# EspressoSystems/cap

Hardware: AMD Instinct MI355X
Metric: transfer-note proofs/sec (2-in/2-out) (higher is better)
Workload: dtype u32 limbs (254-bit Montgomery integers; 9 x 29-bit lazy limbs in the hot kernels)

## Files before the change

cap_amd/csrc/check_kernels.hpp:

```cpp
#pragma once
#include <hip/hip_runtime.h>

#include "gatecheck29.hpp"
#include "plonk_kernels.hpp"

namespace cap {
namespace pk {

constexpr unsigned long long kCopyKeyBase = 1ull << 40;
constexpr unsigned long long kNoFault = ~0ull;

struct CheckKey {
  const fe* sel;
  const uint32_t* perm;
  uint32_t num_inputs;
  uint32_t pad;
};
struct CheckOut {
  unsigned long long first;
  unsigned long long gates, copies;
};

__device__ __forceinline__ void check_report(unsigned long long key, unsigned long long* first,
                                             unsigned long long* count) {
  __shared__ unsigned long long s_min[kThreads / 64];
  __shared__ uint32_t s_cnt[kThreads / 64];
  const uint32_t cnt = (uint32_t)__popcll(__ballot(key != kNoFault));
  uint32_t lo = (uint32_t)key, hi = (uint32_t)(key >> 32);
#pragma unroll
  for (int d = 32; d >= 1; d >>= 1) {
    const uint32_t olo = __shfl_xor(lo, d), ohi = __shfl_xor(hi, d);
    const unsigned long long o = ((unsigned long long)ohi << 32) | olo, m = ((unsigned long long)hi << 32) | lo;
    if (o < m) {
      lo = olo;
      hi = ohi;
    }
  }
  const uint32_t wave = threadIdx.x >> 6;
  if ((threadIdx.x & 63) == 0) {
    s_min[wave] = ((unsigned long long)hi << 32) | lo;
    s_cnt[wave] = cnt;
  }
  __syncthreads();
  if (threadIdx.x == 0) {
    unsigned long long m = s_min[0];
    uint32_t c = s_cnt[0];
#pragma unroll
    for (int k = 1; k < kThreads / 64; k++) {
      m = s_min[k] < m ? s_min[k] : m;
      c += s_cnt[k];
    }
    if (c) {
      atomicMin(first, m);
      atomicAdd(count, (unsigned long long)c);
    }
  }
}

__global__ __launch_bounds__(kThreads) void k_check_gates(const fe* __restrict__ wires ,
                                                          const fe* __restrict__ pub ,
                                                          size_t pub_stride, const CheckKey* __restrict__ keys, size_t n,
                                                          CheckOut* __restrict__ out) {
  using C = wc29::Check<>;
  using F = C::F;
  const size_t j = (size_t)blockIdx.x * blockDim.x + threadIdx.x;
  const uint32_t p = blockIdx.y;
  unsigned long long key = kNoFault;
  if (j < n) {
    const CheckKey k = keys[p];
    fl w[NW];
#pragma unroll
    for (int i = 0; i < NW; i++) w[i] = F::from_ext(wires[((size_t)p * NW + i) * n + j]);
    const fl pi = j < k.num_inputs ? F::from_ext(pub[(size_t)p * pub_stride + j]) : F::zero();
    const fe* sel = k.sel + j;
    if (!C::gate_holds([&](int s) { return F::load(sel[(size_t)s * n]); }, w, pi)) key = j;
  }
  check_report(key, &out[p].first, &out[p].gates);
}

__global__ __launch_bounds__(kThreads) void k_check_copies(const fe* __restrict__ wires ,
                                                           const CheckKey* __restrict__ keys, size_t n,
                                                           CheckOut* __restrict__ out) {
  using C = wc29::Check<>;
  const size_t cells = (size_t)NW * n;
  const size_t c = (size_t)blockIdx.x * blockDim.x + threadIdx.x;
  const uint32_t p = blockIdx.y;
  unsigned long long key = kNoFault;
  if (c < cells) {
    const uint32_t to = keys[p].perm[c];
    if (to != c && to < cells) {
      const fe* w = wires + (size_t)p * cells;
      if (!C::same_value(w[c], w[to])) key = kCopyKeyBase + c;
    }
  }
  check_report(key, &out[p].first, &out[p].copies);
}

__global__ void k_check_targets(const CheckKey* __restrict__ keys, const CheckOut* __restrict__ out, uint32_t P,
                                size_t cells, uint32_t* __restrict__ to) {
  const uint32_t p = blockIdx.x * blockDim.x + threadIdx.x;
  if (p >= P) return;
  const unsigned long long first = out[p].first;
  uint32_t t = 0;
  if (first != kNoFault && first >= kCopyKeyBase && first - kCopyKeyBase < cells) t = keys[p].perm[first - kCopyKeyBase];
  to[p] = t;
}

__global__ __launch_bounds__(kThreads) void k_perm_index(const fe* __restrict__ sig_eval ,
                                                         wc29::PermConsts pc, size_t cells, uint32_t* __restrict__ perm,
                                                         uint32_t* __restrict__ bad) {
  using C = wc29::Check<>;
  const size_t c = (size_t)blockIdx.x * blockDim.x + threadIdx.x;
  if (c >= cells) return;
  const uint32_t idx = C::perm_index(C::F::from_ext(sig_eval[c]), pc);
  perm[c] = idx;
  if (idx == wc29::kNoIndex) atomicOr(bad, 1u);
}

}
}
```

cap_amd/csrc/ntt.hip:

```cpp
#include "ntt.hpp"
#include "field29.hpp"
#include "launch.hpp"

#include <stdlib.h>

#include <vector>

namespace cap {

namespace {

constexpr int kThreads = 256;
#ifndef CAP_NTT_IO_BATCH
#define CAP_NTT_IO_BATCH 2
#endif
constexpr int kIoBatch = CAP_NTT_IO_BATCH;
#ifdef CAP_NTT_WAVES4
#define CAP_NTT_ATTR __attribute__((amdgpu_waves_per_eu(4, 4)))
#else
#define CAP_NTT_ATTR
#endif
constexpr uint32_t kMaxTileLogDefault = 10;
uint32_t max_tile_log() {
  static uint32_t v = [] {
    const char* e = getenv("CAPGPU_NTT_TILE_LOG");
    int x = e ? atoi(e) : (int)kMaxTileLogDefault;
    return (uint32_t)(x >= 8 && x <= 11 ? x : (int)kMaxTileLogDefault);
  }();
  return v;
}

uint32_t tile_log_for(uint32_t log_n, uint32_t count) {
  static const bool adapt = [] {
    const char* e = getenv("CAPGPU_NTT_TILE_ADAPT");
    return !e || atoi(e) != 0;
  }();
  uint32_t tl = max_tile_log();
  if (!adapt) return tl;
  while (tl > 8 && (((uint64_t)count << log_n) >> tl) < 256) tl--;
  return tl;
}

struct PassParams {
  const fe* in;
  fe* out;
  size_t in_outer, in_inner, in_len;
  uint32_t in_group;
  uint32_t in_es;
  size_t in_inner2;
  uint32_t in_group2;
  size_t out_outer, out_inner;
  uint32_t out_group;
  size_t out_inner2;
  uint32_t out_group2;
  size_t pre_inner;
  const fl* tw_small;
  const fe* tw_full;
  const fe* pre_scale;
  const fe* post_scale;
  fe post_scalar;
  uint32_t use_post_scalar;
  uint32_t tw_scaled;
  uint32_t lazy_out;
  uint32_t log_n;
  uint32_t log_len;
  uint32_t log_c;
  uint32_t log_m;
  uint32_t log_n1, log_n2;
  uint32_t* tile_counter;
  uint32_t tiles_x, tiles_y;
};

__device__ __forceinline__ bool next_tile(const PassParams& p, uint32_t round, uint32_t& bx, uint32_t& by) {
  if (!p.tile_counter) {
    bx = blockIdx.x;
    by = blockIdx.y;
    return round == 0;
  }
  __shared__ uint32_t tile_s;
  __syncthreads();
  if (threadIdx.x == 0) tile_s = atomicAdd(p.tile_counter, 1u);
  __syncthreads();
  const uint32_t t = tile_s;
  if (t >= p.tiles_x * p.tiles_y) return false;
  bx = t % p.tiles_x;
  by = t / p.tiles_x;
  return true;
}

__device__ __forceinline__ uint32_t bitrev32(uint32_t x, uint32_t bits) { return __brev(x) >> (32 - bits); }

__device__ __forceinline__ uint32_t fl_any(const fl& a) {
  uint32_t o = 0;
#pragma unroll
  for (int k = 0; k < 9; k++) o |= a.v[k];
  return o;
}
#ifndef CAP_NTT_NO_SHOUP
constexpr int kTwStride = 2;
#define NTT_TW_MUL(x, idx) Fr29::mul_shoup((x), tw_small[2 * (idx)], tw_small[2 * (idx) + 1])
#define NTT_SUB(u, t) Fr29::sub8p((u), (t))
#define NTT_SUB_LAZY(u, t) Fr29::sub8p_lazy((u), (t))
#define NTT_SUB_FROM_LAZY(u, t) Fr29::sub8p((u), (t))
#else
constexpr int kTwStride = 1;
#define NTT_TW_MUL(x, idx) Fr29::mul((x), tw_small[(idx)])
#define NTT_SUB(u, t) Fr29::sub2p((u), (t))
#define NTT_SUB_LAZY(u, t) Fr29::sub2p_lazy((u), (t))
#define NTT_SUB_FROM_LAZY(u, t) Fr29::sub2p((u), (t))
#endif
__device__ __forceinline__ void lds_ntt(fl* sh, const fl* __restrict__ tw_small, uint32_t log_len, uint32_t log_c) {
  const uint32_t half_tile = 1u << (log_len + log_c - 1);
  const uint32_t cmask = (1u << log_c) - 1;
  const uint32_t s0 = log_len & 1;
  if (s0) {
    for (uint32_t b = threadIdx.x; b < half_tile; b += kThreads) {
      const uint32_t c = b & cmask, bb = b >> log_c;
      const uint32_t i0 = ((bb << 1) << log_c) + c, i1 = i0 + (1u << log_c);
      const fl u = sh[i0], v = sh[i1];
      if (fl_any(v) == 0) {
        sh[i1] = u;
        continue;
      }
      const fl t = Fr29::weak_reduce(v);
      sh[i0] = Fr29::normalize(Fr29::add(u, t));
      sh[i1] = Fr29::sub2p(u, t);
    }
    __syncthreads();
  }
  const uint32_t quarter_tile = half_tile >> 1;
  for (uint32_t s = s0; s + 1 < log_len; s += 2) {
    const uint32_t h = 1u << s;
    const uint32_t step = h << log_c;
    for (uint32_t g = threadIdx.x; g < quarter_tile; g += kThreads) {
      const uint32_t c = g & cmask;
      const uint32_t gg = g >> log_c;
      const uint32_t pos = gg & (h - 1);
      const uint32_t j = ((gg >> s) << (s + 2)) + pos;
      const uint32_t i0 = (j << log_c) + c, i1 = i0 + step, i2 = i1 + step, i3 = i2 + step;
      fl a = sh[i0], b = sh[i1], cc = sh[i2], d = sh[i3];
      fl a1, b1, c1, d1, t;
      if (s == 0) {
        if (fl_any(b)) {
          t = Fr29::weak_reduce(b);
          a1 = Fr29::add(a, t);
          b1 = Fr29::sub2p_lazy(a, t);
        } else {
          a1 = a;
          b1 = a;
        }
        if (fl_any(d)) {
          t = Fr29::weak_reduce(d);
          c1 = Fr29::normalize(Fr29::add(cc, t));
          d1 = Fr29::sub2p(cc, t);
        } else {
          c1 = cc;
          d1 = cc;
        }
        t = Fr29::weak_reduce(c1);
      } else {
        const uint32_t i_w1 = pos << (log_len - 1 - s);
        t = NTT_TW_MUL(b, i_w1);
        a1 = Fr29::add(a, t);
        b1 = NTT_SUB_LAZY(a, t);
        t = NTT_TW_MUL(d, i_w1);
        c1 = Fr29::add(cc, t);
        d1 = NTT_SUB(cc, t);
        t = NTT_TW_MUL(c1, pos << (log_len - 2 - s));
      }
      sh[i0] = Fr29::normalize(Fr29::add(a1, t));
      sh[i2] = NTT_SUB(a1, t);
      t = NTT_TW_MUL(d1, (pos + h) << (log_len - 2 - s));
      sh[i1] = Fr29::normalize(Fr29::add(b1, t));
      sh[i3] = NTT_SUB_FROM_LAZY(b1, t);
    }
    __syncthreads();
  }
}

__device__ __forceinline__ void col_tile(const PassParams& p, fl* sh, const uint32_t bx, const uint32_t by) {
  {
  const uint32_t log_s = p.log_m - p.log_len;
  const uint32_t tiles_per_seg_log = log_s - p.log_c;
  const uint32_t t = bx;
  const size_t seg = t >> tiles_per_seg_log;
  const uint32_t col0 = (t & ((1u << tiles_per_seg_log) - 1)) << p.log_c;
  const uint32_t q2 = by / p.in_group;
  const fe* in = p.in + (size_t)(q2 / p.in_group2) * p.in_outer + (size_t)(q2 % p.in_group2) * p.in_inner2 +
                 (size_t)(by % p.in_group) * p.in_inner;
  const uint32_t o2 = by / p.out_group;
  fe* out = p.out + (size_t)(o2 / p.out_group2) * p.out_outer + (size_t)(o2 % p.out_group2) * p.out_inner2 +
            (size_t)(by % p.out_group) * p.out_inner;
  const size_t base = (seg << p.log_m) + col0;
  const uint32_t tile = 1u << (p.log_len + p.log_c);
  const uint32_t cmask = (1u << p.log_c) - 1;
  for (uint32_t e0 = threadIdx.x; e0 < tile; e0 += kIoBatch * kThreads) {
    fe raw[kIoBatch], pre[kIoBatch];
    uint32_t any[kIoBatch];
    size_t sgs[kIoBatch];
#pragma unroll
    for (int u = 0; u < kIoBatch; u++) {
      const uint32_t e = e0 + u * kThreads;
      const uint32_t c = e & cmask, j = e >> p.log_c;
      const size_t g = base + ((size_t)j << log_s) + c;
      const size_t sg = p.in_es == 1 ? g : g * p.in_es + (size_t)(by % p.in_group) * p.in_inner;
      sgs[u] = sg;
      any[u] = 0;
      if (e < tile && sg < p.in_len) {
        raw[u] = p.in_es == 1 ? in[g] : in[g * p.in_es];
        any[u] = 1;
      } else {
#pragma unroll
        for (int k = 0; k < 8; k++) raw[u].v[k] = 0;
      }
    }
    if (p.pre_scale) {
#pragma unroll
      for (int u = 0; u < kIoBatch; u++)
        if (any[u]) pre[u] = p.pre_scale[sgs[u] + (size_t)(by % p.in_group) * p.pre_inner];
    }
#pragma unroll
    for (int u = 0; u < kIoBatch; u++) {
      const uint32_t e = e0 + u * kThreads;
      if (e >= tile) break;
      const uint32_t c = e & cmask, j = e >> p.log_c;
      uint32_t nz = 0;
#pragma unroll
      for (int k = 0; k < 8; k++) nz |= raw[u].v[k];
      fl v = Fr29::load(raw[u]);
      if (p.pre_scale && any[u] && nz) v = Fr29::mul(v, Fr29::load(pre[u]));
      sh[(bitrev32(j, p.log_len) << p.log_c) + c] = v;
    }
  }
  __syncthreads();
  lds_ntt(sh, p.tw_small, p.log_len, p.log_c);
  const uint32_t tw_shift = p.log_n - p.log_m;
  for (uint32_t e0 = threadIdx.x; e0 < tile; e0 += kIoBatch * kThreads) {
    fe tw[kIoBatch];
    size_t exs[kIoBatch];
#pragma unroll
    for (int u = 0; u < kIoBatch; u++) {
      const uint32_t e = e0 + u * kThreads;
      const uint32_t c = e & cmask, k = e >> p.log_c;
      exs[u] = e < tile ? ((size_t)(col0 + c) * k) << tw_shift : 0;
      if (exs[u] || p.tw_scaled) tw[u] = p.tw_full[exs[u]];
    }
#pragma unroll
    for (int u = 0; u < kIoBatch; u++) {
      const uint32_t e = e0 + u * kThreads;
      if (e >= tile) break;
      const uint32_t c = e & cmask, k = e >> p.log_c;
      fl v = sh[e];
      v = (exs[u] || p.tw_scaled) ? Fr29::mul(v, Fr29::load(tw[u])) : Fr29::weak_reduce(v);
      out[base + ((size_t)k << log_s) + c] = Fr29::pack(v);
    }
  }
  }
}
template <bool PERSIST>
__global__ __launch_bounds__(kThreads) CAP_NTT_ATTR void ntt_col_pass(PassParams p) {
  extern __shared__ __align__(16) unsigned char smem[];
  fl* sh = reinterpret_cast<fl*>(smem);
  if constexpr (!PERSIST) {
    col_tile(p, sh, blockIdx.x, blockIdx.y);
  } else {
    uint32_t bx, by;
    for (uint32_t round = 0; next_tile(p, round, bx, by); round++) col_tile(p, sh, bx, by);
  }
}

__device__ __forceinline__ void row_tile(const PassParams& p, fl* sh, const uint32_t bx, const uint32_t by) {
  {
  const uint32_t t = bx;
  const uint32_t k2 = t & ((1u << p.log_n2) - 1);
  const uint32_t r0 = (t >> p.log_n2) << p.log_c;
  const uint32_t q2 = by / p.in_group;
  const fe* in = p.in + (size_t)(q2 / p.in_group2) * p.in_outer + (size_t)(q2 % p.in_group2) * p.in_inner2 +
                 (size_t)(by % p.in_group) * p.in_inner;
  const uint32_t o2 = by / p.out_group;
  fe* out = p.out + (size_t)(o2 / p.out_group2) * p.out_outer + (size_t)(o2 % p.out_group2) * p.out_inner2 +
            (size_t)(by % p.out_group) * p.out_inner;
  const uint32_t tile = 1u << (p.log_len + p.log_c);
  const uint32_t lmask = (1u << p.log_len) - 1;
  const uint32_t cmask = (1u << p.log_c) - 1;
  for (uint32_t e0 = threadIdx.x; e0 < tile; e0 += kIoBatch * kThreads) {
    fe raw[kIoBatch], pre[kIoBatch];
    uint32_t any[kIoBatch];
    size_t sgs[kIoBatch];
#pragma unroll
    for (int u = 0; u < kIoBatch; u++) {
      const uint32_t e = e0 + u * kThreads;
      const uint32_t j = e & lmask, c = e >> p.log_len;
      const size_t g = ((((size_t)(r0 + c) << p.log_n2) + k2) << p.log_len) + j;
      const size_t sg = p.in_es == 1 ? g : g * p.in_es + (size_t)(by % p.in_group) * p.in_inner;
      sgs[u] = sg;
      any[u] = 0;
      if (e < tile && sg < p.in_len) {
        raw[u] = p.in_es == 1 ? in[g] : in[g * p.in_es];
        any[u] = 1;
      } else {
#pragma unroll
        for (int k = 0; k < 8; k++) raw[u].v[k] = 0;
      }
    }
    if (p.pre_scale) {
#pragma unroll
      for (int u = 0; u < kIoBatch; u++)
        if (any[u]) pre[u] = p.pre_scale[sgs[u] + (size_t)(by % p.in_group) * p.pre_inner];
    }
#pragma unroll
    for (int u = 0; u < kIoBatch; u++) {
      const uint32_t e = e0 + u * kThreads;
      if (e >= tile) break;
      const uint32_t j = e & lmask, c = e >> p.log_len;
      uint32_t nz = 0;
#pragma unroll
      for (int k = 0; k < 8; k++) nz |= raw[u].v[k];
      fl v = Fr29::load(raw[u]);
      if (p.pre_scale && any[u] && nz) v = Fr29::mul(v, Fr29::load(pre[u]));
      sh[(bitrev32(j, p.log_len) << p.log_c) + c] = v;
    }
  }
  __syncthreads();
  lds_ntt(sh, p.tw_small, p.log_len, p.log_c);
  for (uint32_t e = threadIdx.x; e < tile; e += kThreads) {
    uint32_t c = e & cmask, k = e >> p.log_c;
    fl v = sh[e];
    size_t g = (size_t)(r0 + c) + ((size_t)k2 << p.log_n1) + ((size_t)k << (p.log_n1 + p.log_n2));
    if (p.post_scale) v = Fr29::mul(v, Fr29::load(p.post_scale[g]));
    else if (p.use_post_scalar) v = Fr29::mul(v, Fr29::load(p.post_scalar));
    out[g] = p.lazy_out ? Fr29::store(v) : Fr29::pack(Fr29::canonical(v));
  }
  }
}
template <bool PERSIST>
__global__ __launch_bounds__(kThreads) CAP_NTT_ATTR void ntt_row_pass(PassParams p) {
  extern __shared__ __align__(16) unsigned char smem[];
  fl* sh = reinterpret_cast<fl*>(smem);
  if constexpr (!PERSIST) {
    row_tile(p, sh, blockIdx.x, blockIdx.y);
  } else {
    uint32_t bx, by;
    for (uint32_t round = 0; next_tile(p, round, bx, by); round++) row_tile(p, sh, bx, by);
  }
}

__global__ void table_unpack(fl* __restrict__ out, const fe* __restrict__ in, size_t n) {
  size_t e = (size_t)blockIdx.x * blockDim.x + threadIdx.x;
  if (e >= n) return;
  if constexpr (kTwStride == 1) {
    out[e] = Fr29::load(in[e]);
  } else {
    const fl t = Fr29::load(in[e]);
    out[2 * e] = Fr29::load(Fr29::from_mont(t));
    out[2 * e + 1] = Fr29::shoup_quotient(t);
  }
}

__global__ void table_to_internal(fe* __restrict__ out, const fe* __restrict__ in, size_t n) {
  size_t e = (size_t)blockIdx.x * blockDim.x + threadIdx.x;
  if (e >= n) return;
  out[e] = Fr29::pack(Fr29::canonical(Fr29::from_ext(in[e])));
}

__global__ void powers_table(fe* out, size_t n, const fe* __restrict__ pw, fe scale, int has_scale) {
  size_t e = (size_t)blockIdx.x * blockDim.x + threadIdx.x;
  if (e >= n) return;
  fe r = has_scale ? scale : Fr::one();
  bool started = has_scale;
  for (int b = 0; (e >> b) != 0; b++) {
    if ((e >> b) & 1) {
      r = started ? Fr::mul(r, pw[b]) : pw[b];
      started = true;
    }
  }
  out[e] = r;
}

__global__ __launch_bounds__(kThreads) void ntt3_combine(const fe* __restrict__ y, fe* __restrict__ out, size_t out_outer,
                                                         size_t out_inner, uint32_t out_group, size_t m_len,
                                                         const fe* __restrict__ tw, fe w3, const fe* __restrict__ post,
                                                         const fe* __restrict__ add) {
  using F = Fr29;
  const size_t k = (size_t)blockIdx.x * blockDim.x + threadIdx.x;
  if (k >= m_len) return;
  const uint32_t q = blockIdx.y;
  const fe* yq = y + (size_t)q * 3 * m_len;
  fe* o = out + (size_t)(q / out_group) * out_outer + (size_t)(q % out_group) * out_inner;
  const fl y0 = F::load(yq[k]);
  const fl t1 = F::mul(F::load(yq[m_len + k]), F::load(tw[k]));
  const fl t2 = F::mul(F::load(yq[2 * m_len + k]), F::load(tw[2 * k]));
  const fl d = F::mul(F::sub(t1, t2), F::load(w3));
  fl x0 = F::normalize(F::add(F::add(y0, t1), t2));
  fl x1 = F::normalize(F::add(F::sub(y0, t2), d));
  fl x2 = F::sub(F::sub(y0, t1), d);
  if (post) {
    const size_t half = m_len >> 1;
    const fl a = add ? F::load(add[(size_t)q * half + (k & (half - 1))]) : F::zero();
    auto finish = [&](const fl& x, const fe& ps) {
      fl v = F::mul(x, F::load(ps));
      if (add) v = F::add_norm(v, a);
      return F::pack(F::canonical(v));
    };
    o[k] = finish(x0, post[k]);
    o[m_len + k] = finish(x1, post[m_len + k]);
    o[2 * m_len + k] = finish(x2, post[2 * m_len + k]);
  } else {
    o[k] = F::store(x0);
    o[m_len + k] = F::store(x1);
    o[2 * m_len + k] = F::store(x2);
  }
}

fe host_root_of_unity(uint32_t log_n) {
  fe w;
  const uint32_t root28[8] = {0x725b19f0u, 0x9bd61b6eu, 0x41112ed4u, 0x402d111eu,
                              0x8ef62abcu, 0x00e0a7ebu, 0xa58a7e85u, 0x2a3c09f0u};
  for (int i = 0; i < 8; i++) w.v[i] = root28[i];
  w = Fr::to_mont(w);
  for (uint32_t i = log_n; i < 28; i++) w = Fr::sqr(w);
  return w;
}

fe host_from_u64(uint64_t v) {
  fe t = Fr::zero();
  t.v[0] = (uint32_t)v;
  t.v[1] = (uint32_t)(v >> 32);
  return Fr::to_mont(t);
}

int build_powers(fe* d_out, size_t n, fe base, const fe* scale, hipStream_t stream) {
  std::vector<fe> pw(40);
  fe x = base;
  for (int b = 0; b < 40; b++) {
    pw[b] = x;
    x = Fr::sqr(x);
  }
  fe* d_pw = nullptr;
  hipError_t e = hipMalloc(&d_pw, sizeof(fe) * pw.size());
  if (e != hipSuccess) return (int)e;
  e = hipMemcpyAsync(d_pw, pw.data(), sizeof(fe) * pw.size(), hipMemcpyHostToDevice, stream);
  if (e != hipSuccess) return (int)e;
  fe sc = scale ? *scale : Fr::one();
  size_t blocks = (n + 255) / 256;
  launch("powers_table", powers_table, dim3((unsigned)blocks), dim3(256), 0, stream, d_out, n, d_pw, sc, scale ? 1 : 0);
  e = hipStreamSynchronize(stream);
  hipFree(d_pw);
  return (int)e;
}

}

fe ntt_root_of_unity(uint32_t log_n) { return host_root_of_unity(log_n); }

int ntt_build_small_tables(NttSmallTables* t, hipStream_t stream) {
  if (!t->pass_counters) {
    hipError_t ec = hipMalloc(&t->pass_counters, sizeof(uint32_t) * kNttPassCounters);
    if (ec != hipSuccess) return (int)ec;
  }
  for (int s = 1; s <= kMaxLogTile; s++) {
    size_t n = (size_t)1 << (s - 1);
    hipError_t e = hipMalloc(&t->fwd[s], sizeof(fe) * n);
    if (e != hipSuccess) return (int)e;
    e = hipMalloc(&t->inv[s], sizeof(fe) * n);
    if (e != hipSuccess) return (int)e;
    fe w = host_root_of_unity(s);
    int rc = build_powers(t->fwd[s], n, w, nullptr, stream);
    if (rc) return rc;
    rc = build_powers(t->inv[s], n, Fr::inv(w), nullptr, stream);
    if (rc) return rc;
    launch("table_to_internal", table_to_internal, dim3((unsigned)((n + 255) / 256)), dim3(256), 0, stream, t->fwd[s],
           (const fe*)t->fwd[s], n);
    launch("table_to_internal", table_to_internal, dim3((unsigned)((n + 255) / 256)), dim3(256), 0, stream, t->inv[s],
           (const fe*)t->inv[s], n);
    for (int d = 0; d < 2; d++) {
      uint32_t** dst = d ? &t->inv_u[s] : &t->fwd_u[s];
      e = hipMalloc(dst, sizeof(fl) * n * kTwStride);
      if (e != hipSuccess) return (int)e;
      launch("table_unpack", table_unpack, dim3((unsigned)((n + 255) / 256)), dim3(256), 0, stream,
             reinterpret_cast<fl*>(*dst), (const fe*)(d ? t->inv[s] : t->fwd[s]), n);
    }
    hipError_t es = hipStreamSynchronize(stream);
    if (es != hipSuccess) return (int)es;
  }
  return 0;
}

void ntt_free_small_tables(NttSmallTables* t) {
  if (t->pass_counters) hipFree(t->pass_counters);
  t->pass_counters = nullptr;
  for (int s = 0; s <= kMaxLogTile; s++) {
    if (t->fwd[s]) hipFree(t->fwd[s]);
    if (t->inv[s]) hipFree(t->inv[s]);
    if (t->fwd_u[s]) hipFree(t->fwd_u[s]);
    if (t->inv_u[s]) hipFree(t->inv_u[s]);
    t->fwd[s] = t->inv[s] = nullptr;
    t->fwd_u[s] = t->inv_u[s] = nullptr;
  }
}

int ntt_build_domain(NttDomain* d, uint32_t log_n, hipStream_t stream) {
  d->log_n = log_n;
  size_t n = (size_t)1 << log_n;
  hipError_t e;
  if ((e = hipMalloc(&d->tw_fwd, sizeof(fe) * n)) != hipSuccess) return (int)e;
  if ((e = hipMalloc(&d->tw_inv, sizeof(fe) * n)) != hipSuccess) return (int)e;
  if ((e = hipMalloc(&d->coset_fwd, sizeof(fe) * n)) != hipSuccess) return (int)e;
  if ((e = hipMalloc(&d->coset_inv, sizeof(fe) * n)) != hipSuccess) return (int)e;
  fe w = host_root_of_unity(log_n);
  fe g = host_from_u64(5);
  d->n_inv = Fr::inv(host_from_u64((uint64_t)n));
  int rc;
  if ((rc = build_powers(d->tw_fwd, n, w, nullptr, stream))) return rc;
  if ((rc = build_powers(d->tw_inv, n, Fr::inv(w), nullptr, stream))) return rc;
  if ((rc = build_powers(d->coset_fwd, n, g, nullptr, stream))) return rc;
  if ((rc = build_powers(d->coset_inv, n, Fr::inv(g), &d->n_inv, stream))) return rc;
  fe* src[4] = {d->tw_fwd, d->tw_inv, d->coset_fwd, d->coset_inv};
  fe** dst[4] = {&d->tw29_fwd, &d->tw29_inv, &d->coset29_fwd, &d->coset29_inv};
#ifndef CAP_NTT_NO_INV_FOLD
  if ((e = hipMalloc(&d->tw29_inv_n, sizeof(fe) * n)) != hipSuccess) return (int)e;
  if ((rc = build_powers(d->tw29_inv_n, n, Fr::inv(w), &d->n_inv, stream))) return rc;
  launch("table_to_internal", table_to_internal, dim3((unsigned)((n + 255) / 256)), dim3(256), 0, stream, d->tw29_inv_n,
         (const fe*)d->tw29_inv_n, n);
#endif
  for (int k = 0; k < 4; k++) {
    if ((e = hipMalloc(dst[k], sizeof(fe) * n)) != hipSuccess) return (int)e;
    launch("table_to_internal", table_to_internal, dim3((unsigned)((n + 255) / 256)), dim3(256), 0, stream, *dst[k],
           (const fe*)src[k], n);
  }
  d->n_inv29 = Fr29::pack(Fr29::canonical(Fr29::from_ext(d->n_inv)));
  if ((e = hipStreamSynchronize(stream)) != hipSuccess) return (int)e;
  hipFree(d->tw_inv);
  hipFree(d->coset_fwd);
  hipFree(d->coset_inv);
  d->tw_inv = d->coset_fwd = d->coset_inv = nullptr;
  return 0;
}

void ntt_free_domain(NttDomain* d) {
  if (d->tw_fwd) hipFree(d->tw_fwd);
  if (d->tw_inv) hipFree(d->tw_inv);
  if (d->coset_fwd) hipFree(d->coset_fwd);
  if (d->coset_inv) hipFree(d->coset_inv);
  for (fe* t : {d->tw29_fwd, d->tw29_inv, d->tw29_inv_n, d->coset29_fwd, d->coset29_inv})
    if (t) hipFree(t);
  d->tw_fwd = d->tw_inv = d->coset_fwd = d->coset_inv = nullptr;
  d->tw29_fwd = d->tw29_inv = d->tw29_inv_n = d->coset29_fwd = d->coset29_inv = nullptr;
}

void ntt_table_to_internal(fe* out, const fe* in, size_t n, hipStream_t stream) {
  if (n == 0) return;
  launch("table_to_internal", table_to_internal, dim3((unsigned)((n + 255) / 256)), dim3(256), 0, stream, out, in, n);
}

namespace {
unsigned ntt_persistent() {
  static const unsigned v = [] {
    const char* e = getenv("CAPGPU_NTT_PERSISTENT");
    const long x = e ? atol(e) : 0;
    return (unsigned)(x >= 1 && x <= 16 ? x : 0);
  }();
  return v;
}
template <class K>
void launch_pass(const char* name, K kernel, K kernel_persistent, PassParams& p, const NttSmallTables& small, size_t tiles,
                 uint32_t count, size_t lds, bool persistent, hipStream_t stream) {
  p.tile_counter = nullptr;
  p.tiles_x = (uint32_t)tiles;
  p.tiles_y = count;
  if (persistent) {
    uint32_t* ctr = small.pass_counters ? small.pass_counters + (small.next_counter++ % kNttPassCounters) : nullptr;
    const hipError_t e = ctr ? hipMemsetAsync(ctr, 0, sizeof(uint32_t), stream) : hipErrorInvalidValue;
    if (e != hipSuccess) {
      (void)hipGetLastError();
      LaunchError& le = launch_error();
      if (le.code == hipSuccess) {
        le.code = e;
        le.kernel = name;
      }
      return;
    }
    p.tile_counter = ctr;
    launch(name, kernel_persistent, dim3(256u * ntt_persistent()), dim3(kThreads), lds, stream, p);
    return;
  }
  launch(name, kernel, dim3((unsigned)tiles, count), dim3(kThreads), lds, stream, p);
}
}

int ntt_plan(uint32_t log_n, uint32_t count, NttPlan* out) {
  NttPlan pl{};
  if (log_n == 0 || count == 0) {
    *out = pl;
    return 0;
  }
  pl.tile_log = tile_log_for(log_n, count);
  uint32_t lg[3] = {0, 0, 0};
  if (log_n <= 10) {
    pl.passes = 1;
    lg[2] = log_n;
  } else if (log_n <= 20) {
    pl.passes = 2;
    lg[0] = (log_n + 1) / 2;
    lg[2] = log_n / 2;
  } else {
    pl.passes = 3;
    lg[0] = (log_n + 2) / 3;
    lg[1] = (log_n - lg[0] + 1) / 2;
    lg[2] = log_n - lg[0] - lg[1];
  }
  if (lg[0] > 10 || lg[1] > 10 || lg[2] > 10) return (int)hipErrorInvalidValue;
  const unsigned per_cu = ntt_persistent();
  auto finish = [&](uint32_t i, uint32_t log_len, uint32_t log_c) {
    pl.digits[i] = log_len;
    pl.log_c[i] = log_c;
    pl.tiles[i] = (uint64_t)1 << (log_n - log_len - log_c);
    const uint64_t total = pl.tiles[i] * count;
    pl.persistent[i] = per_cu && total > 4ull * 256 * per_cu && total < (1ull << 32);
  };
  uint32_t log_m = log_n;
  for (uint32_t d = 0; d + 1 < pl.passes; d++) {
    const uint32_t log_len = lg[d];
    const uint32_t log_s = log_m - log_len;
    uint32_t log_c = pl.tile_log > log_len ? pl.tile_log - log_len : 0;
    if (log_c > log_s) log_c = log_s;
    if (log_c > 4) log_c = 4;
    finish(d, log_len, log_c);
    log_m -= log_len;
  }
  {
    const uint32_t log_len = lg[2];
    const uint32_t log_n1 = pl.passes >= 2 ? lg[0] : 0;
    uint32_t log_c = pl.tile_log > log_len ? pl.tile_log - log_len : 0;
    if (log_c > log_n1) log_c = log_n1;
    if (log_c > 4) log_c = 4;
    finish(pl.passes - 1, log_len, log_c);
  }
  *out = pl;
  return 0;
}

int ntt_run(const NttDomain& dom, const NttSmallTables& small, fe* data, fe* scratch, size_t stride_elems,
            uint32_t count, int dir, int coset, hipStream_t stream, const NttIo* io) {
  const uint32_t log_n = dom.log_n;
  if (count == 0) return 0;
  if (log_n == 0) {
    return 0;
  }
  NttPlan plan;
  if (int rc = ntt_plan(log_n, count, &plan)) return rc;
  const int passes = (int)plan.passes;
  uint32_t* const* tws = dir ? small.inv_u : small.fwd_u;
  const fe* tw_full = dir ? dom.tw29_inv : dom.tw29_fwd;

  PassParams p{};
  const size_t scratch_stride = io ? ((size_t)1 << log_n) : stride_elems;
  struct Addr {
    size_t outer, inner;
    uint32_t group;
  };
  const Addr a_src = io ? Addr{io->src_outer, io->src_inner, io->src_group ? io->src_group : 1u} : Addr{stride_elems, 0, 1};
  const Addr a_dst = io ? Addr{io->dst_outer, io->dst_inner, io->dst_group ? io->dst_group : 1u} : Addr{stride_elems, 0, 1};
  const Addr a_tmp = Addr{scratch_stride, 0, 1};
  const size_t src_len = io ? io->src_len : ~(size_t)0;
  auto set_in = [&](const Addr& a, size_t len, uint32_t es) {
    p.in_outer = a.outer;
    p.in_inner = a.inner;
    p.in_group = a.group;
    p.in_len = len;
    p.in_es = es;
    p.in_group2 = 1;
    p.in_inner2 = 0;
    if (&a == &a_src && io && io->src_group2 > 1) {
      p.in_group2 = io->src_group2;
      p.in_inner2 = io->src_inner2;
    }
  };
  const uint32_t src_es = io && io->src_elem_stride ? io->src_elem_stride : 1;
  auto set_out = [&](const Addr& a) {
    p.out_outer = a.outer;
    p.out_inner = a.inner;
    p.out_group = a.group;
    p.out_group2 = 1;
    p.out_inner2 = 0;
    if (&a == &a_dst && io && io->dst_group2 > 1) {
      p.out_group2 = io->dst_group2;
      p.out_inner2 = io->dst_inner2;
    }
  };
  p.pre_inner = io ? io->pre_inner : 0;
  p.log_n = log_n;
  p.tw_full = tw_full;
  p.use_post_scalar = 0;
#ifndef CAP_NTT_NO_INV_FOLD
  const bool inv_fold = dir && !coset && passes >= 2 && !(io && io->has_post_scalar) && dom.tw29_inv_n;
#else
  const bool inv_fold = false;
#endif

  const fe* pre = (!dir && coset) ? dom.coset29_fwd : nullptr;
  if (io && io->pre_scale) pre = io->pre_scale;
  bool first = true;
  const fe* cur_in = io ? io->src : data;
  uint32_t log_m = log_n;
  for (int d = 0; d < passes - 1; d++) {
    const uint32_t log_len = plan.digits[d], log_c = plan.log_c[d];
    p.in = cur_in;
    p.out = scratch;
    set_in(first ? a_src : a_tmp, first ? src_len : ~(size_t)0, first ? src_es : 1);
    set_out(a_tmp);
    p.tw_small = reinterpret_cast<const fl*>(tws[log_len]);
    p.pre_scale = first ? pre : nullptr;
    p.post_scale = nullptr;
    p.log_len = log_len;
    p.log_c = log_c;
    p.log_m = log_m;
    p.tw_full = (inv_fold && d == 0) ? dom.tw29_inv_n : tw_full;
    p.tw_scaled = (inv_fold && d == 0) ? 1 : 0;
    size_t lds = sizeof(fl) << (log_len + log_c);
    launch_pass("ntt_col_pass", ntt_col_pass<false>, ntt_col_pass<true>, p, small, (size_t)plan.tiles[d], count, lds,
                plan.persistent[d] != 0, stream);
    cur_in = scratch;
    first = false;
    log_m -= log_len;
  }
  {
    const int last = passes - 1;
    const uint32_t log_len = plan.digits[last], log_c = plan.log_c[last];
    const uint32_t log_n1 = passes >= 2 ? plan.digits[0] : 0;
    const uint32_t log_n2 = passes == 3 ? plan.digits[1] : 0;
    p.in = cur_in;
    p.out = data;
    set_in(first ? a_src : a_tmp, first ? src_len : ~(size_t)0, first ? src_es : 1);
    set_out(a_dst);
    p.tw_small = reinterpret_cast<const fl*>(tws[log_len]);
    p.pre_scale = first ? pre : nullptr;
    p.post_scale = (dir && coset) ? dom.coset29_inv : nullptr;
    p.use_post_scalar = (dir && !coset && !inv_fold) ? 1 : 0;
    p.post_scalar = (io && io->has_post_scalar) ? io->post_scalar : dom.n_inv29;
    p.lazy_out = (io && io->lazy_out) ? 1 : 0;
    p.log_len = log_len;
    p.log_c = log_c;
    p.log_n1 = log_n1;
    p.log_n2 = log_n2;
    size_t lds = sizeof(fl) << (log_len + log_c);
    launch_pass("ntt_row_pass", ntt_row_pass<false>, ntt_row_pass<true>, p, small, (size_t)plan.tiles[last], count, lds,
                plan.persistent[last] != 0, stream);
  }
  return 0;
}

namespace {
void exponent_third(uint32_t e[8]) {
  uint32_t t[8];
  for (int i = 0; i < 8; i++) t[i] = FrP::MOD[i];
  t[0] -= 1;
  uint64_t rem = 0;
  for (int i = 7; i >= 0; i--) {
    uint64_t cur = (rem << 32) | t[i];
    e[i] = (uint32_t)(cur / 3);
    rem = cur % 3;
  }
}
}

int ntt3_build_domain(Ntt3Domain* d, uint32_t log_m, hipStream_t stream) {
  d->log_m = log_m;
  const size_t M = (size_t)1 << log_m, N = 3 * M;
  uint32_t e3[8];
  exponent_third(e3);
  const fe g = host_from_u64(5);
  const fe w3gen = Fr::pow(g, e3);
  size_t c = (M % 3 == 2) ? (M + 1) / 3 : (2 * M + 1) / 3;
  if (M == 1) c = 1;
  uint32_t ec[8] = {(uint32_t)c, (uint32_t)((uint64_t)c >> 32), 0, 0, 0, 0, 0, 0};
  const fe wM = host_root_of_unity(log_m);
  const fe wN = Fr::mul(w3gen, Fr::pow(wM, ec));
  d->omega = wN;
  uint32_t eM[8] = {(uint32_t)M, (uint32_t)((uint64_t)M >> 32), 0, 0, 0, 0, 0, 0};
  const fe w3 = Fr::pow(wN, eM);
  auto to_internal = [](const fe& a) { return Fr29::pack(Fr29::canonical(Fr29::from_ext(a))); };
  d->w3inv_29 = to_internal(Fr::inv(w3));
  hipError_t e;
  if ((e = hipMalloc(&d->xs_ext, sizeof(fe) * N)) != hipSuccess) return (int)e;
  if ((e = hipMalloc(&d->xs29, sizeof(fe) * N)) != hipSuccess) return (int)e;
  if ((e = hipMalloc(&d->pre3, sizeof(fe) * N)) != hipSuccess) return (int)e;
  if ((e = hipMalloc(&d->tw29_inv, sizeof(fe) * 2 * M)) != hipSuccess) return (int)e;
  if ((e = hipMalloc(&d->coset_inv_ext, sizeof(fe) * N)) != hipSuccess) return (int)e;
  int rc;
  const fe k32 = host_from_u64(32);
  fe s_a = g;
  for (int a = 0; a < 3; a++) {
    if ((rc = build_powers(d->xs_ext + (size_t)a * M, M, wM, &s_a, stream))) return rc;
    if ((rc = build_powers(d->pre3 + (size_t)a * M, M, s_a, &k32, stream))) return rc;
    s_a = Fr::mul(s_a, wN);
  }
  if ((rc = build_powers(d->tw29_inv, 2 * M, Fr::inv(wN), nullptr, stream))) return rc;
  uint32_t eN[8] = {(uint32_t)N, (uint32_t)((uint64_t)N >> 32), 0, 0, 0, 0, 0, 0};
  d->kappa = Fr::inv(Fr::sub(Fr::pow(g, eN), Fr::one()));
  d->kappa_n_inv29 = to_internal(Fr::mul(Fr::add(d->kappa, d->kappa), Fr::inv(host_from_u64((uint64_t)M))));
  const fe third = Fr::inv(host_from_u64(3));
  if ((rc = build_powers(d->coset_inv_ext, N, Fr::inv(g), &third, stream))) return rc;
  const unsigned blocks = (unsigned)((N + 255) / 256);
  launch("table_to_internal", table_to_internal, dim3(blocks), dim3(256), 0, stream, d->xs29, (const fe*)d->xs_ext, N);
  launch("table_to_internal", table_to_internal, dim3(blocks), dim3(256), 0, stream, d->pre3, (const fe*)d->pre3, N);
  launch("table_to_internal", table_to_internal, dim3((unsigned)((2 * M + 255) / 256)), dim3(256), 0, stream,
         d->tw29_inv, (const fe*)d->tw29_inv, 2 * M);
  return (int)hipStreamSynchronize(stream);
}

void ntt3_free_domain(Ntt3Domain* d) {
  for (fe** t : {&d->xs_ext, &d->xs29, &d->pre3, &d->tw29_inv, &d->coset_inv_ext}) {
    if (*t) hipFree(*t);
    *t = nullptr;
  }
}

int ntt3_forward(const Ntt3Domain& d3, const NttDomain& dom_m, const NttSmallTables& small, fe* data, NttIo io,
                 uint32_t count, fe* scratch, hipStream_t stream) {
  if (dom_m.log_n != d3.log_m) return (int)hipErrorInvalidValue;
  const size_t M = (size_t)1 << d3.log_m;
  if (io.src_len > M) return (int)hipErrorInvalidValue;
  NttIo sub{};
  sub.src = io.src;
  sub.src_outer = io.src_outer;
  sub.src_inner = 0;
  sub.src_group = 3;
  sub.src_group2 = io.src_group ? io.src_group : 1;
  sub.src_inner2 = io.src_inner;
  sub.src_len = io.src_len;
  sub.pre_scale = d3.pre3;
  sub.pre_inner = M;
  sub.lazy_out = 1;
  sub.dst_outer = io.dst_outer;
  sub.dst_inner = M;
  sub.dst_group = 3;
  sub.dst_group2 = io.dst_group ? io.dst_group : 1;
  sub.dst_inner2 = io.dst_inner;
  return ntt_run(dom_m, small, data, scratch, M, count * 3, 0, 0, stream, &sub);
}

int ntt3_inverse(const Ntt3Domain& d3, const NttDomain& dom_m, const NttSmallTables& small, fe* data, uint32_t count,
                 fe* scratch, hipStream_t stream, const fe* add) {
  if (dom_m.log_n != d3.log_m) return (int)hipErrorInvalidValue;
  if (add && d3.log_m == 0) return (int)hipErrorInvalidValue;
  const size_t M = (size_t)1 << d3.log_m, N = 3 * M;
  fe* y = scratch;
  fe* sub_scratch = scratch + (size_t)count * 3 * M;
  NttIo sub{};
  sub.src = data;
  sub.src_outer = N;
  sub.src_inner = M;
  sub.src_group = 3;
  sub.src_len = M;
  sub.lazy_out = 1;
  sub.dst_outer = M;
  sub.dst_inner = 0;
  sub.dst_group = 1;
  int rc = ntt_run(dom_m, small, y, sub_scratch, M, count * 3, 1, 0, stream, &sub);
  if (rc) return rc;
  launch("ntt3_combine", ntt3_combine, dim3((unsigned)((M + kThreads - 1) / kThreads), count), dim3(kThreads), 0, stream,
         (const fe*)y, data, N, (size_t)0, 1u, M, (const fe*)d3.tw29_inv, d3.w3inv_29, (const fe*)d3.coset_inv_ext, add);
  return 0;
}

}
```

cap_amd/csrc/ntt.hpp:

```cpp
#pragma once
#include <hip/hip_runtime.h>
#include <stdint.h>

#include "field.hpp"

namespace cap {

struct NttDomain {
  uint32_t log_n = 0;
  fe* tw_fwd = nullptr;
  fe* tw_inv = nullptr;
  fe* coset_fwd = nullptr;
  fe* coset_inv = nullptr;
  fe n_inv;
  fe* tw29_fwd = nullptr;
  fe* tw29_inv = nullptr;
  fe* tw29_inv_n = nullptr;
  fe* coset29_fwd = nullptr;
  fe* coset29_inv = nullptr;
  fe n_inv29;
};

constexpr int kMaxLogTile = 11;
struct NttSmallTables {
  fe* fwd[kMaxLogTile + 1] = {nullptr};
  fe* inv[kMaxLogTile + 1] = {nullptr};
  uint32_t* fwd_u[kMaxLogTile + 1] = {nullptr};
  uint32_t* inv_u[kMaxLogTile + 1] = {nullptr};
  uint32_t* pass_counters = nullptr;
  mutable uint32_t next_counter = 0;
};
constexpr uint32_t kNttPassCounters = 256;

int ntt_build_small_tables(NttSmallTables* t, hipStream_t stream);
int ntt_build_domain(NttDomain* d, uint32_t log_n, hipStream_t stream);
void ntt_free_domain(NttDomain* d);
void ntt_free_small_tables(NttSmallTables* t);

fe ntt_root_of_unity(uint32_t log_n);

struct NttIo {
  const fe* src;
  size_t src_outer, src_inner, src_len;
  uint32_t src_group;
  size_t dst_outer, dst_inner;
  uint32_t dst_group;
  uint32_t src_elem_stride = 1;
  uint32_t src_group2 = 1;
  size_t src_inner2 = 0;
  uint32_t dst_group2 = 1;
  size_t dst_inner2 = 0;
  size_t pre_inner = 0;
  const fe* pre_scale = nullptr;
  int lazy_out = 0;
  int has_post_scalar = 0;
  fe post_scalar = {};
};
int ntt_run(const NttDomain& dom, const NttSmallTables& small, fe* data, fe* scratch, size_t stride_elems,
            uint32_t count, int dir, int coset, hipStream_t stream, const NttIo* io = nullptr);

struct NttPlan {
  uint32_t passes = 0;
  uint32_t tile_log = 0;
  uint32_t digits[3] = {0, 0, 0};
  uint32_t log_c[3] = {0, 0, 0};
  uint64_t tiles[3] = {0, 0, 0};
  uint32_t persistent[3] = {0, 0, 0};
};
int ntt_plan(uint32_t log_n, uint32_t count, NttPlan* out);

struct Ntt3Domain {
  uint32_t log_m = 0;
  fe* xs_ext = nullptr;
  fe* xs29 = nullptr;
  fe* pre3 = nullptr;
  fe* tw29_inv = nullptr;
  fe* coset_inv_ext = nullptr;
  fe w3inv_29;
  fe omega;
  fe kappa;
  fe kappa_n_inv29;
};
int ntt3_build_domain(Ntt3Domain* d, uint32_t log_m, hipStream_t stream);
void ntt3_free_domain(Ntt3Domain* d);
int ntt3_forward(const Ntt3Domain& d3, const NttDomain& dom_m, const NttSmallTables& small, fe* data, NttIo io,
                 uint32_t count, fe* scratch, hipStream_t stream);
int ntt3_inverse(const Ntt3Domain& d3, const NttDomain& dom_m, const NttSmallTables& small, fe* data, uint32_t count,
                 fe* scratch, hipStream_t stream, const fe* add = nullptr);

void ntt_table_to_internal(fe* out, const fe* in, size_t n, hipStream_t stream);

}
```

cap_amd/csrc/plonk.hip:

```cpp
#define CAP_FL_SCHED 1
#include <stdlib.h>
#include <string.h>

#include <algorithm>
#include <atomic>
#include <chrono>
#include <condition_variable>
#include <functional>
#include <map>
#include <mutex>
#include <string>
#include <thread>
#include <vector>

#include "check_kernels.hpp"
#include "coalescer.hpp"
#include "compact.hpp"
#include "compact_kernels.hpp"
#include "context.hpp"
#include "host_util.hpp"
#include "launch.hpp"
#include "params.hpp"
#include "plonk_kernels.hpp"
#include "solve.hpp"
#include "solve_defer.hpp"
#include "tickets.hpp"
#include "transcript_dev.hpp"
#include "vars_kernels.hpp"

namespace cap {

using namespace pk;

struct SolveSched {
  uint64_t uid = 0;
  sp::Plan plan;
  std::vector<fe> konst;
  capgpu_solver_info info{};
  capgpu_hint_info hint_info{};
  capgpu_solver_rules_info rules{};
  int auto_pack = 1;
  int form = CAPGPU_SOLVE_FORM_DIRECT;
  std::vector<uint32_t> table;
  std::vector<uint8_t> sel_zero;
  sd::Sched defer;
  std::vector<fe> defer_konst;
};

struct ProvingKey {
  size_t n = 0, m = 0, ps = 0;
  uint32_t log_n = 0, log_m = 0;
  size_t num_inputs = 0;
  uint64_t srs_handle = 0;
  fe* coef = nullptr;
  fe* sig_eval = nullptr;
  fe* pk_coset = nullptr;
  fe* inv_nx1 = nullptr;
  QuotConst qc;
  QuotConst qc29;
  capgpu_verifying_key vk;
  std::vector<uint8_t> vk_bytes;
  bool recompute = false;
  int device = 0;
  uint64_t uid = next_uid();
  static uint64_t next_uid() {
    static std::atomic<uint64_t> n{1};
    return n.fetch_add(1);
  }
  mutable std::mutex chk_mu;
  mutable fe* chk_sel = nullptr;
  mutable uint32_t* chk_perm = nullptr;
  mutable int chk_rc = 1;
  mutable std::string chk_err;
  mutable uint32_t* wire_vars = nullptr;
  mutable size_t num_vars = 0;
  mutable std::shared_ptr<const SolveSched> solve;
  mutable void* solve_dev = nullptr;
  mutable uint64_t solve_dev_uid = 0;
  mutable SolveTables solve_tab{};
  ProvingKey() = default;
  ProvingKey(const ProvingKey&) = delete;
  ProvingKey& operator=(const ProvingKey&) = delete;
  ~ProvingKey() {
    for (void* p : {(void*)coef, (void*)sig_eval, (void*)pk_coset, (void*)inv_nx1, (void*)chk_sel, (void*)chk_perm,
                    (void*)wire_vars, solve_dev})
      if (p) hipFree(p);
  }
};

constexpr int kGraphSegs = 8;
struct ProveGraphSig {
  uint64_t key_uid = 0, srs = 0;
  uint32_t P = 0;
  size_t num_inputs = 0;
  int form = 0;
  bool multi = false;
  const void *d_wires = nullptr, *ws = nullptr, *msm_ws = nullptr, *ntt_scratch = nullptr, *bases = nullptr;
  const void* lagrange = nullptr;
  hipStream_t stream = nullptr;
  bool overlap = false;
  int transcript = 0;
  uint32_t tr_stride = 0;
  int outcomes = 0;
  bool operator==(const ProveGraphSig& o) const {
    return key_uid == o.key_uid && srs == o.srs && P == o.P && num_inputs == o.num_inputs && form == o.form &&
           multi == o.multi && d_wires == o.d_wires && ws == o.ws && msm_ws == o.msm_ws && ntt_scratch == o.ntt_scratch &&
           bases == o.bases && lagrange == o.lagrange && stream == o.stream && overlap == o.overlap && transcript == o.transcript &&
           tr_stride == o.tr_stride && outcomes == o.outcomes;
  }
};
struct ProveGraphSet {
  ProveGraphSig sig;
  hipGraphExec_t exec[kGraphSegs] = {};
  uint32_t seen = 0;
  bool broken = false;
  uint64_t stamp = 0;
  ProveGraphSet() = default;
  ProveGraphSet(const ProveGraphSet&) = delete;
  ProveGraphSet& operator=(const ProveGraphSet&) = delete;
  ~ProveGraphSet() { drop(); }
  void drop() {
    for (auto& e : exec)
      if (e) {
        (void)hipGraphExecDestroy(e);
        e = nullptr;
      }
  }
};
struct ProveGraphCache {
  std::vector<std::unique_ptr<ProveGraphSet>> sets;
  uint64_t clock = 0;
};
static std::atomic<uint64_t> g_graph_captured{0}, g_graph_replayed{0};
static std::atomic<uint64_t> g_prove_calls{0}, g_stream_waits{0};

static_assert(sizeof(capgpu_proof) == td::kPrBytes && offsetof(capgpu_proof, prod_perm_poly_comm) == td::kPrZ &&
                  offsetof(capgpu_proof, split_quot_poly_comms) == td::kPrQuot &&
                  offsetof(capgpu_proof, opening_proof) == td::kPrOpen &&
                  offsetof(capgpu_proof, shifted_opening_proof) == td::kPrShifted &&
                  offsetof(capgpu_proof, wires_evals) == td::kPrWireEvals &&
                  offsetof(capgpu_proof, wire_sigma_evals) == td::kPrSigmaEvals &&
                  offsetof(capgpu_proof, perm_next_eval) == td::kPrNext,
              "transcript_dev.hpp writes capgpu_proof by offset");


namespace {

bool graph_runtime_ok() {
  static const bool ok = [] {
    if (env_int("CAPGPU_GRAPH_FORCE", 0) != 0) return true;
    int v = 0;
    if (hipRuntimeGetVersion(&v) != hipSuccess) {
      (void)hipGetLastError();
      return false;
    }
    return v >= HIP_VERSION;
  }();
  return ok;
}
uint32_t graph_max_batch() {
  if (!graph_runtime_ok()) return 0;
  const int x = env_int("CAPGPU_GRAPH_MAX_BATCH", 16);
  return (uint32_t)(x < 0 ? 0 : (x > 64 ? 64 : x));
}
ProveGraphSet* graph_set_for(Context& c, const ProveGraphSig& sig) {
  if (!c.prove_graphs) c.prove_graphs = std::make_shared<ProveGraphCache>();
  ProveGraphCache& gc = *c.prove_graphs;
  gc.clock++;
  for (auto& sp : gc.sets)
    if (sp->sig == sig) {
      sp->stamp = gc.clock;
      sp->seen++;
      return sp->broken ? nullptr : sp.get();
    }
  ProveGraphSet* slot = nullptr;
  for (auto& sp : gc.sets)
    if (sp->sig.key_uid == sig.key_uid && sp->sig.P == sig.P && sp->sig.form == sig.form && sp->sig.multi == sig.multi &&
        sp->sig.d_wires == sig.d_wires && sp->sig.transcript == sig.transcript && sp->sig.outcomes == sig.outcomes)
      slot = sp.get();
  if (!slot && gc.sets.size() >= 8) {
    slot = gc.sets[0].get();
    for (auto& sp : gc.sets)
      if (sp->stamp < slot->stamp) slot = sp.get();
  }
  if (!slot) {
    gc.sets.emplace_back(new ProveGraphSet);
    slot = gc.sets.back().get();
  }
  if (slot->exec[0] || slot->seen) (void)hipStreamSynchronize(c.stream);
  slot->drop();
  slot->sig = sig;
  slot->seen = 1;
  slot->broken = false;
  slot->stamp = gc.clock;
  return nullptr;
}
template <class F>
int run_segment(Context& c, ProveGraphSet* g, int id, F&& enqueue) {
  if (!g || g->broken) return enqueue();
  hipStream_t s = c.stream;
  if (g->exec[id]) {
    CAP_HIP(hipGraphLaunch(g->exec[id], s));
    g_graph_replayed++;
    return CAPGPU_OK;
  }
  if (hipStreamBeginCapture(s, hipStreamCaptureModeThreadLocal) != hipSuccess) {
    (void)hipGetLastError();
    g->broken = true;
    return enqueue();
  }
  const LaunchError before = launch_error();
  c.capturing = true;
  int rc = enqueue();
  c.capturing = false;
  hipGraph_t graph = nullptr;
  hipError_t e = hipStreamEndCapture(s, &graph);
  if (rc == CAPGPU_OK && e == hipSuccess && graph && launch_error().code == before.code) {
    hipGraphExec_t ex = nullptr;
    e = hipGraphInstantiate(&ex, graph, nullptr, nullptr, 0);
    (void)hipGraphDestroy(graph);
    if (e == hipSuccess && ex) {
      g->exec[id] = ex;
      g_graph_captured++;
      CAP_HIP(hipGraphLaunch(ex, s));
      return CAPGPU_OK;
    }
  } else if (graph) {
    (void)hipGraphDestroy(graph);
  }
  (void)hipGetLastError();
  launch_error() = before;
  g->broken = true;
  return enqueue();
}

HostPool& host_pool() {
  Context& c = ctx();
  if (!c.pool) c.pool.reset(new HostPool(HostPool::default_threads((unsigned)std::max<size_t>(num_contexts(), 1))));
  return *c.pool;
}

template <class F>
void parallel_for(uint32_t count, F&& fn) {
  HostPool& pool = host_pool();
  if (pool.size() <= 1 || count <= 1) {
    for (uint32_t i = 0; i < count; i++) fn(i);
    return;
  }
  std::function<void(uint32_t)> job = [&](uint32_t i) { fn(i); };
  pool.run(count, job);
}

}
}

#include "prove_run.hpp"

namespace cap {
namespace {


int key_check_tables(const ProvingKey& K) {
  std::lock_guard<std::mutex> lk(K.chk_mu);
  if (K.chk_rc <= 0) {
    if (K.chk_rc) set_error("%s", K.chk_err.c_str());
    return K.chk_rc;
  }
  Context& c = ctx();
  hipStream_t s = c.stream;
  const size_t n = K.n, cells = (size_t)NW * n;
  DevTmp<fe> sel;
  DevTmp<uint32_t> perm, bad;
  CAP_HIP(sel.alloc((size_t)NS * n));
  int rc = run_ntt_from(s, K.log_n, K.coef, K.ps, n, sel, n, NS, 0, 0);
  if (rc) return rc;
  ntt_table_to_internal(sel, sel, (size_t)NS * n, s);
  if (K.chk_perm) {
    CAP_HIP(hipStreamSynchronize(s));
    if ((rc = take_launch_error())) return rc;
    K.chk_sel = sel.p;
    sel.p = nullptr;
    K.chk_rc = CAPGPU_OK;
    return CAPGPU_OK;
  }
  CAP_HIP(perm.alloc(cells));
  CAP_HIP(bad.alloc(1));
  wc29::PermConsts pc;
  memset(&pc, 0, sizeof pc);
  pc.log_n = K.log_n;
  auto conv = [](const fe& a) { return Fr29::pack(Fr29::canonical(Fr29::from_ext(a))); };
  for (int i = 0; i < NW; i++) pc.kinv[i] = conv(Fr::inv(K.qc.k[i]));
  fe w = Fr::inv(ntt_root_of_unity(K.log_n));
  for (uint32_t b = 0; b < K.log_n && b < 28; b++) {
    pc.winv[b] = conv(w);
    w = Fr::sqr(w);
  }
  CAP_HIP(hipMemsetAsync(bad, 0, sizeof(uint32_t), s));
  launch("k_perm_index", k_perm_index, dim3(cdiv(cells, kThreads)), dim3(kThreads), 0, s, (const fe*)K.sig_eval, pc, cells,
         perm.p, bad.p);
  uint32_t h_bad = 0;
  CAP_HIP(hipMemcpyAsync(&h_bad, bad, sizeof(uint32_t), hipMemcpyDeviceToHost, s));
  CAP_HIP(hipStreamSynchronize(s));
  if ((rc = take_launch_error())) return rc;
  if (h_bad) {
    set_error("capgpu_plonk_check_witness: sigma is not a permutation of the extended domain (a value of sigma lies in "
              "none of the five cosets k_i H)");
    K.chk_err = last_error();
    K.chk_rc = CAPGPU_ERR_INVALID_ARG;
    return K.chk_rc;
  }
  K.chk_sel = sel.p;
  K.chk_perm = perm.p;
  sel.p = nullptr;
  perm.p = nullptr;
  K.chk_rc = CAPGPU_OK;
  return CAPGPU_OK;
}

CheckOut* check_out_at(void* d_small, uint32_t P) {
  return (CheckOut*)((char*)d_small + (sizeof(CheckKey) * P + 255) / 256 * 256);
}
size_t check_small_bytes(uint32_t P) {
  return (sizeof(CheckKey) + sizeof(CheckOut) + sizeof(uint32_t)) * (size_t)P + 768;
}

int check_batch(const ProvingKey& K, const std::vector<const ProvingKey*>* keys, uint32_t P, const fe* d_vals,
                const fe* d_pub, size_t pub_stride, void* d_small, capgpu_witness_fault* faults, bool gates_only = false) {
  Context& c = ctx();
  hipStream_t s = c.stream;
  const size_t n = K.n;
  std::vector<CheckKey> hk(P);
  int rc;
  for (uint32_t p = 0; p < P; p++) {
    const ProvingKey& Kp = keys ? *(*keys)[p] : K;
    if (Kp.n != n) {
      set_error("capgpu_plonk_check_witness_multi: the keys of one batch must share the domain size");
      return CAPGPU_ERR_INVALID_ARG;
    }
    if ((p == 0 || keys) && (rc = key_check_tables(Kp))) return rc;
    hk[p] = CheckKey{Kp.chk_sel, Kp.chk_perm, (uint32_t)Kp.num_inputs, 0};
  }
  CheckKey* dk = (CheckKey*)d_small;
  CheckOut* dout = check_out_at(d_small, P);
  uint32_t* dto = (uint32_t*)((char*)dout + (sizeof(CheckOut) * P + 255) / 256 * 256);
  std::vector<CheckOut> ho(P, CheckOut{kNoFault, 0, 0});
  std::vector<uint32_t> hto(P);
  CAP_HIP(hipMemcpyAsync(dk, hk.data(), sizeof(CheckKey) * P, hipMemcpyHostToDevice, s));
  CAP_HIP(hipMemcpyAsync(dout, ho.data(), sizeof(CheckOut) * P, hipMemcpyHostToDevice, s));
  launch("k_check_gates", k_check_gates, dim3(cdiv(n, kThreads), P), dim3(kThreads), 0, s, d_vals, d_pub, pub_stride,
         (const CheckKey*)dk, n, dout);
  if (!gates_only) {
    launch("k_check_copies", k_check_copies, dim3(cdiv((size_t)NW * n, kThreads), P), dim3(kThreads), 0, s, d_vals,
           (const CheckKey*)dk, n, dout);
    launch("k_check_targets", k_check_targets, dim3(cdiv(P, 64)), dim3(64), 0, s, (const CheckKey*)dk,
           (const CheckOut*)dout, P, (size_t)NW * n, dto);
  }
  CAP_HIP(hipMemcpyAsync(ho.data(), dout, sizeof(CheckOut) * P, hipMemcpyDeviceToHost, s));
  if (!gates_only) CAP_HIP(hipMemcpyAsync(hto.data(), dto, sizeof(uint32_t) * P, hipMemcpyDeviceToHost, s));
  CAP_HIP(hipStreamSynchronize(s));
  if ((rc = take_launch_error())) return rc;
  for (uint32_t p = 0; p < P; p++) {
    capgpu_witness_fault& f = faults[p];
    memset(&f, 0, sizeof f);
    f.gates_failed = ho[p].gates;
    f.copies_failed = ho[p].copies;
    if (ho[p].first == kNoFault) continue;
    if (ho[p].first < kCopyKeyBase) {
      f.kind = 1;
      f.row = ho[p].first;
      continue;
    }
    const uint64_t cell = ho[p].first - kCopyKeyBase;
    const uint32_t to = hto[p];
    f.kind = 2;
    f.wire = (uint32_t)(cell / n);
    f.row = cell % n;
    f.wire2 = (uint32_t)(to / n);
    f.row2 = to % n;
  }
  return CAPGPU_OK;
}

size_t check_carve(void* base, uint32_t P, size_t pub_stride, bool coeffs, size_t n, void** small, fe** pub, fe** vals) {
  Carver k(base);
  *small = k.take<char>(check_small_bytes(P));
  *pub = k.take<fe>((size_t)P * (pub_stride ? pub_stride : 1));
  *vals = coeffs ? k.take<fe>((size_t)P * NW * n) : nullptr;
  return k.off + 256;
}

int check_resident(const ProvingKey& K, const std::vector<const ProvingKey*>* keys, uint32_t P, const fe* d_wires,
                   const uint64_t* pubs, size_t pub_stride, int form, capgpu_witness_fault* faults,
                   bool gates_only = false) {
  Context& c = ctx();
  hipStream_t s = c.stream;
  const size_t n = K.n;
  const bool coeffs = form == CAPGPU_INPUT_COEFFS;
  void* d_small = nullptr;
  fe *d_pub = nullptr, *d_vals = nullptr;
  int rc = scratch_reserve(c.stage_a, check_carve(nullptr, P, pub_stride, coeffs, n, &d_small, &d_pub, &d_vals));
  if (rc) return rc;
  (void)check_carve(c.stage_a.p, P, pub_stride, coeffs, n, &d_small, &d_pub, &d_vals);
  if (pub_stride) CAP_HIP(hipMemcpyAsync(d_pub, pubs, sizeof(fe) * P * pub_stride, hipMemcpyHostToDevice, s));
  if (coeffs) {
    if ((rc = run_ntt_from(s, K.log_n, d_wires, n, n, d_vals, n, P * NW, 0, 0))) return rc;
  } else {
    d_vals = const_cast<fe*>(d_wires);
  }
  return check_batch(K, keys, P, d_vals, d_pub, pub_stride, d_small, faults, gates_only);
}

std::string fault_text(uint32_t p, const capgpu_witness_fault& f) {
  char b[160];
  oc::fault_text(p, f, b, sizeof b);
  return b;
}
int precheck_verdict(const capgpu_witness_fault* faults, uint32_t P) {
  uint32_t bad = 0, first = P;
  for (uint32_t p = 0; p < P; p++)
    if (faults[p].kind) {
      if (!bad) first = p;
      bad++;
    }
  if (!bad) return CAPGPU_OK;
  char b[320];
  oc::precheck_text(bad, P, first, faults[first], b, sizeof b);
  set_error("%s", b);
  return CAPGPU_ERR_PROOF;
}

void precheck_needs(const ProvePlan& pl, const ProvingKey& K, ProveNeeds& nd) {
  if (!pl.precheck) return;
  void* a = nullptr;
  fe *b = nullptr, *v = nullptr;
  nd.stage_a = check_carve(nullptr, pl.P, K.num_inputs, pl.coeffs, K.n, &a, &b, &v);
  if (pl.coeffs) nd.ntt(ntt_scratch_from(K.log_n, (size_t)pl.P * NW));
}
ProveNeeds prove_needs(const ProvePlan& pl, const ProvingKey& K) {
  ProveNeeds nd;
  precheck_needs(pl, K, nd);
  ProveRun::needs(pl, K, nd);
  return nd;
}

int prove_planned(Context& c, const ProvingKey& K, uint32_t P, const ProveRequest& rq, const ProvePlan& pl, ProveRun& run) {
  const size_t num_inputs = rq.num_inputs;
  int rc;
  if ((rc = scratch_reserve(c.prove_ws, carve(nullptr, K, P, num_inputs, pl.coeffs, pl.tr_stride).total))) return rc;
  run.w = carve(c.prove_ws.p, K, P, num_inputs, pl.coeffs, pl.tr_stride);
  if (run.faults && pl.dev_tr)
    CAP_HIP(hipMemcpy2DAsync(run.w.chk_first, sizeof(unsigned long long), &check_out_at(c.stage_a.p, P)->first,
                             sizeof(CheckOut), sizeof(unsigned long long), P, hipMemcpyDeviceToDevice, c.stream));
  if (pl.graphs) {
    ProveGraphSig sig;
    sig.key_uid = K.uid;
    sig.srs = K.srs_handle;
    sig.P = P;
    sig.num_inputs = num_inputs;
    sig.form = rq.form;
    sig.multi = rq.keys != nullptr;
    sig.d_wires = rq.d_wires;
    sig.ws = c.prove_ws.p;
    sig.msm_ws = c.msm_ws.p;
    sig.ntt_scratch = c.ntt_scratch.p;
    sig.bases = pl.B->ext;
    sig.lagrange = pl.Lag ? pl.Lag->ext : nullptr;
    sig.stream = c.stream;
    sig.overlap = pl.overlap;
    sig.transcript = pl.dev_tr ? CAPGPU_TRANSCRIPT_DEVICE : CAPGPU_TRANSCRIPT_HOST;
    sig.tr_stride = pl.tr_stride;
    sig.outcomes = rq.outcomes ? (run.faults ? 2 : 1) : 0;
    run.gs = graph_set_for(c, sig);
  }
  return pl.dev_tr ? run.run_device_transcript() : run.run_host_transcript();
}

std::atomic<int> g_compact{-1};
std::atomic<uint64_t> g_compact_calls{0}, g_compact_dropped{0}, g_compact_rows{0};
bool compaction_on() {
  static const int env_default = env_int("CAPGPU_COMPACT", 0) != 0 ? 1 : 0;
  const int m = g_compact.load(std::memory_order_relaxed);
  return (m < 0 ? env_default : m) != 0;
}
static_assert(sizeof(CheckKey) >= sizeof(uint2), "the move table takes the place of the check's key array");

int prove_compacted(Context& c, const ProvingKey& K, uint32_t P, const ProveRequest& rq,
                    const std::vector<capgpu_witness_fault>& faults, uint32_t bad, bool* ran) {
  *ran = false;
  const uint32_t S = P - bad;
  const size_t n = K.n, row16 = sizeof(fe) * NW * n / sizeof(uint4);
  const bool in_place = rq.d_wires == (const fe*)c.stage_b.p;
  if (!in_place && (!cp::copy_route_pays(bad, S) || ((uintptr_t)rq.d_wires & (sizeof(uint4) - 1)))) return CAPGPU_OK;
  std::vector<uint8_t> refused(P);
  for (uint32_t p = 0; p < P; p++) refused[p] = faults[p].kind != 0;
  const cp::Plan plan = cp::compact_plan(refused.data(), P);
  const std::vector<uint32_t>& orig = plan.orig;
  int rc;
  std::vector<uint2> table;
  fe* cols = const_cast<fe*>(rq.d_wires);
  if (in_place) {
    for (const cp::Move& mv : plan.moves) table.push_back(make_uint2(mv.src, mv.dst));
  } else {
    if ((rc = scratch_reserve(c.stage_b, wires_stage_bytes(S, n)))) return rc;
    cols = (fe*)c.stage_b.p;
    for (uint32_t i = 0; i < S; i++) table.push_back(make_uint2(orig[i], i));
  }
  if (!table.empty()) {
    uint2* d_table = (uint2*)c.stage_a.p;
    CAP_HIP(hipMemcpyAsync(d_table, table.data(), sizeof(uint2) * table.size(), hipMemcpyHostToDevice, c.stream));
    launch("k_move_rows", k_move_rows, dim3(cdiv(row16, kThreads), (uint32_t)std::min<size_t>(table.size(), 65535)),
           dim3(kThreads), 0, c.stream, (const uint4*)rq.d_wires, (uint4*)cols, row16, (const uint2*)d_table,
           (uint32_t)table.size());
  }
  std::vector<const ProvingKey*> keys2;
  size_t ni2 = rq.num_inputs;
  if (rq.keys) {
    ni2 = 0;
    for (uint32_t i = 0; i < S; i++) {
      keys2.push_back((*rq.keys)[orig[i]]);
      ni2 = std::max(ni2, keys2[i]->num_inputs);
    }
  }
  const ProvingKey& K2 = rq.keys ? *keys2[0] : K;
  std::vector<uint64_t> pubs2((size_t)4 * ni2 * S + 4, 0), blind2((size_t)4 * 13 * S);
  std::vector<const uint8_t*> msgs2(S, nullptr);
  std::vector<size_t> lens2(S, 0);
  size_t longest = 0;
  for (uint32_t i = 0; i < S; i++) {
    const uint32_t p = orig[i];
    if (ni2) memcpy(&pubs2[(size_t)4 * ni2 * i], rq.pub_inputs + (size_t)4 * rq.num_inputs * p, 32 * ni2);
    memcpy(&blind2[(size_t)4 * 13 * i], rq.blinders + (size_t)4 * 13 * p, 32 * 13);
    if (rq.msgs) {
      msgs2[i] = rq.msgs[p];
      lens2[i] = rq.msg_lens[p];
    }
    const ProvingKey& Kp = rq.keys ? *keys2[i] : K;
    const size_t ml = rq.msgs ? (rq.msgs[p] ? rq.msg_lens[p] : 0) : (rq.ext_msg ? rq.ext_len : 0);
    longest = std::max(longest, ml + Kp.vk_bytes.size() + 32 * Kp.num_inputs);
  }
  std::vector<capgpu_proof> proofs2(S);
  std::vector<capgpu_prove_outcome> outcomes2(S);
  ProveRequest r2 = rq;
  r2.d_wires = cols;
  r2.h_wires = nullptr;
  r2.pub_inputs = ni2 ? pubs2.data() : nullptr;
  r2.num_inputs = ni2;
  r2.blinders = blind2.data();
  r2.msgs = rq.msgs ? msgs2.data() : nullptr;
  r2.msg_lens = rq.msgs ? lens2.data() : nullptr;
  r2.keys = rq.keys ? &keys2 : nullptr;
  r2.proofs = proofs2.data();
  r2.outcomes = outcomes2.data();
  ProvePlan pl2;
  if ((rc = make_plan(c, K2, S, rq.form, false, longest, false, &pl2))) return rc;
  pl2.precheck = false;
  ProveRun run2(c, pl2, K2, r2);
  if ((rc = prove_planned(c, K2, S, r2, pl2, run2))) return rc;
  for (uint32_t i = 0; i < S; i++) {
    rq.proofs[orig[i]] = proofs2[i];
    rq.outcomes[orig[i]] = outcomes2[i];
  }
  for (uint32_t p = 0; p < P; p++)
    if (refused[p]) oc::finish_outcome(0, &faults[p], &rq.outcomes[p], &rq.proofs[p]);
  g_compact_calls.fetch_add(1, std::memory_order_relaxed);
  g_compact_dropped.fetch_add(bad, std::memory_order_relaxed);
  g_compact_rows.fetch_add(table.size(), std::memory_order_relaxed);
  *ran = true;
  return CAPGPU_OK;
}

struct KeySet {
  size_t n = 0, max_inputs = 0;
};
int key_set(const char* who, const ProvingKey* const* keys, size_t count, bool same_srs, bool no_recompute, KeySet* out) {
  *out = KeySet{};
  for (size_t i = 0; i < count; i++) {
    const ProvingKey &K = *keys[0], &Kp = *keys[i];
    if (Kp.n != K.n || (same_srs && Kp.srs_handle != K.srs_handle) || (no_recompute && (Kp.recompute || K.recompute))) {
      set_error("%s: the keys of one batch must share the domain size and the SRS", who);
      return CAPGPU_ERR_INVALID_ARG;
    }
    out->n = K.n;
    out->max_inputs = std::max(out->max_inputs, Kp.num_inputs);
  }
  return CAPGPU_OK;
}

int prove_batch(const ProvingKey& K, uint32_t P, const ProveRequest& rq) {
  Context& c = ctx();
  trace("pb_begin", c.slot, P);
  struct TraceEnd {
    int slot;
    ~TraceEnd() { trace("pb_end", slot); }
  } trace_end{c.slot};
  struct CopyDrain {
    Context& c;
    bool armed;
    ~CopyDrain() {
      if (armed && c.copy_stream) (void)hipStreamSynchronize(c.copy_stream);
    }
  } drain{c, rq.h_wires != nullptr};
  const std::vector<const ProvingKey*>* const keys = rq.keys;
  const size_t num_inputs = rq.num_inputs;
  auto key_of = [&](uint32_t p) -> const ProvingKey& { return keys ? *(*keys)[p] : K; };
  if (rq.form == CAPGPU_INPUT_VARS) {
    const VarsIn* const vin = rq.vin;
    for (uint32_t p = 0; p < P && (keys || p == 0); p++) {
      if (key_lacks_table(key_of(p))) return CAPGPU_ERR_INVALID_ARG;
      if (!vin || key_of(p).num_vars > vin->stride) {
        set_error("capgpu_plonk_prove: rows of %zu variables given, the key of proof %u has %zu", vin ? vin->stride : (size_t)0,
                  p, key_of(p).num_vars);
        return CAPGPU_ERR_INVALID_ARG;
      }
    }
  }
  if (keys) {
    KeySet ks;
    if (int rc = key_set("capgpu_plonk_prove_multi", keys->data(), P, true, true, &ks)) return rc;
    if (num_inputs != ks.max_inputs) {
      set_error("capgpu_plonk_prove_multi: rows of %zu public inputs given, the keys need %zu", num_inputs, ks.max_inputs);
      return CAPGPU_ERR_INVALID_ARG;
    }
  } else if (num_inputs != K.num_inputs) {
    set_error("capgpu_plonk_prove: %zu public inputs given, key expects %zu", num_inputs, K.num_inputs);
    return CAPGPU_ERR_INVALID_ARG;
  }
  if (const int ss = comm_shard_slot(); ss >= 0 && ss != c.slot) {
    set_error("capgpu_plonk_prove: commitment MSMs are sharded over the communicator of context %d (capgpu_plonk_shard_msm); "
              "this call runs on context %d and would prove unsharded while its peers wait", ss, c.slot);
    return CAPGPU_ERR_INVALID_ARG;
  }
  size_t longest = 0;
  for (uint32_t p = 0; p < P; p++) {
    const size_t ml = rq.msgs ? (rq.msgs[p] ? rq.msg_lens[p] : 0) : (rq.ext_msg ? rq.ext_len : 0);
    longest = std::max(longest, ml + key_of(p).vk_bytes.size() + 32 * key_of(p).num_inputs);
  }
  ProvePlan pl;
  int rc = make_plan(c, K, P, rq.form, rq.h_wires != nullptr, longest, false, &pl);
  if (rc) return rc;
  ProveRun run(c, pl, K, rq);
  if (pl.precheck && rq.h_wires && (rc = run.copy_input(0, P, c.stream))) return rc;
  if (pl.vars && !pl.r1_copies) run.gather_vars(0, P);
  std::vector<capgpu_witness_fault> faults;
  if (pl.precheck) {
    faults.resize(P);
    if ((rc = check_resident(K, keys, P, rq.d_wires, rq.pub_inputs, num_inputs, pl.vars ? CAPGPU_INPUT_EVALS : rq.form,
                             faults.data(), pl.vars)))
      return rc;
    if (!rq.outcomes) {
      if ((rc = precheck_verdict(faults.data(), P))) return rc;
    } else {
      run.faults = faults.data();
      uint32_t bad = 0;
      for (uint32_t p = 0; p < P; p++) bad += faults[p].kind != 0;
      if (bad == P) {
        for (uint32_t p = 0; p < P; p++) oc::finish_outcome(0, &faults[p], &rq.outcomes[p], &rq.proofs[p]);
        return CAPGPU_OK;
      }
      if (bad && compaction_on()) {
        bool ran = false;
        if ((rc = prove_compacted(c, K, P, rq, faults, bad, &ran)) || ran) return rc;
      }
    }
  }
  return prove_planned(c, K, P, rq, pl, run);
}

int key_init(ProvingKey& K, size_t n, size_t num_inputs, uint64_t srs_handle) {
  K.n = n;
  K.m = 6 * n;
  K.ps = n + 8;
  while (((size_t)1 << K.log_n) < n) K.log_n++;
  K.log_m = K.log_n + 1;
  if (K.log_m > 25) {
    set_error("capgpu_plonk_preprocess: domain too large");
    return CAPGPU_ERR_INVALID_ARG;
  }
  K.num_inputs = num_inputs;
  K.srs_handle = srs_handle;
  K.device = ctx().device;
  K.recompute = env_int("CAPGPU_RECOMPUTE_PK_COSET", 0) != 0;
  CAP_HIP(hipMalloc(&K.coef, sizeof(fe) * 18 * K.ps));
  CAP_HIP(hipMalloc(&K.sig_eval, sizeof(fe) * NW * n));
  CAP_HIP(hipMalloc(&K.inv_nx1, sizeof(fe) * K.m));
  return CAPGPU_OK;
}

int key_finish_tables(hipStream_t s, ProvingKey& K) {
  const size_t n = K.n, m = K.m;
  int rc;
  const uint64_t five[4] = {5, 0, 0, 0};
  K.qc.g = Fr::to_mont(fe_from_words(five));
  for (int i = 0; i < NW; i++) K.qc.k[i] = Fr::to_mont(fe_from_words(K_CANON[i]));
  {
    uint32_t e_n[8] = {(uint32_t)n, (uint32_t)((uint64_t)n >> 32), 0, 0, 0, 0, 0, 0};
    fe gn = Fr::pow(K.qc.g, e_n);
    const Ntt3Domain* dq = nullptr;
    if ((rc = get_domain3(K.log_m, &dq))) return rc;
    fe w6 = Fr::pow(dq->omega, e_n);
    fe x = gn;
    for (int i = 0; i < 8; i++) K.qc.zh_inv[i] = Fr::zero();
    for (int i = 0; i < 6; i++) {
      K.qc.zh_inv[i] = Fr::inv(Fr::sub(x, Fr::one()));
      x = Fr::mul(x, w6);
    }
  }
  const Ntt3Domain* dom_m = nullptr;
  if ((rc = get_domain3(K.log_m, &dom_m))) return rc;
  launch("k_inv_nx1", k_inv_nx1, dim3(cdiv(m, kThreads)), dim3(kThreads), 0, s, K.inv_nx1, (const fe*)dom_m->xs_ext,
         fr_from_u64((uint64_t)n), m);
  ntt_table_to_internal(K.inv_nx1, K.inv_nx1, m, s);
  {
    auto conv = [](const fe& a) { return Fr29::pack(Fr29::canonical(Fr29::from_ext(a))); };
    K.qc29.g = conv(K.qc.g);
    for (int i = 0; i < NW; i++) K.qc29.k[i] = conv(K.qc.k[i]);
    for (int i = 0; i < 8; i++) K.qc29.zh_inv[i] = conv(K.qc.zh_inv[i]);
  }
  if (!K.recompute) {
    CAP_HIP(hipMalloc(&K.pk_coset, sizeof(fe) * kPkcCols * m));
    if ((rc = compute_pk_coset(s, K, K.pk_coset))) return rc;
    if ((rc = compute_pk_kx(s, K, K.pk_coset))) return rc;
  }
  return CAPGPU_OK;
}

void key_set_vk(ProvingKey& K, const std::vector<g1_affine>& ha) {
  memset(&K.vk, 0, sizeof(K.vk));
  K.vk.domain_size = K.n;
  K.vk.num_inputs = K.num_inputs;
  for (int i = 0; i < NW; i++) fe_to_words(K.qc.k[i], K.vk.k[i]);
  for (int i = 0; i < NS; i++) affine_to_words(ha[i], K.vk.selector_comms[i]);
  for (int i = 0; i < NW; i++) affine_to_words(ha[NS + i], K.vk.sigma_comms[i]);
  SolidityTranscript t;
  t.append_u64_le(254);
  t.append_u64_le((uint64_t)K.n);
  t.append_u64_le((uint64_t)K.num_inputs);
  for (int i = 0; i < NW; i++) append_fr(t, K.qc.k[i]);
  for (int i = 0; i < 18; i++) append_g1(t, ha[i]);
  K.vk_bytes = t.buf;
}

struct ProveReq {
  uint64_t pk;
  const uint64_t* wires;
  const uint64_t* pubs;
  size_t num_inputs;
  const uint8_t* msg;
  size_t msg_len;
  const uint64_t* blinders;
  capgpu_proof* out;
  int form = CAPGPU_INPUT_EVALS;
  int rc = CAPGPU_OK;
  std::string err;
  bool done = false;
  const void* d_wires = nullptr;
  hipEvent_t staged = nullptr;
};

struct StageSlot {
  void* d = nullptr;
  hipEvent_t ev = nullptr;
  size_t bytes = 0;
  hipStream_t stream = nullptr;
};
struct StagePool {
  std::mutex mu;
  static constexpr int kStreams = 4;
  hipStream_t streams[kStreams] = {};
  int device = -1;
  std::vector<StageSlot> idle;
  size_t live = 0, made = 0;
  static constexpr size_t kMaxSlots = 320;
  static bool enabled() {
    return env_int("CAPGPU_COALESCE_PRESTAGE", 0) != 0;
// ... 2737 lines not shown
```

cap_amd/csrc/plonk_kernels.hpp:

```cpp
#pragma once
#include <hip/hip_runtime.h>

#include "field.hpp"
#include "field29.hpp"

namespace cap {
namespace pk {

constexpr int NW = 5;
constexpr int NS = 13;
constexpr int NKX = NW - 1;
constexpr int kPkcCols = NS + NW + NKX;
constexpr int kThreads = 256;
constexpr int kScanPerThread = 4;
constexpr int kScanBlock = kThreads * kScanPerThread;

struct Chal {
  fe beta, gamma, alpha, alpha2, beta_inv, alpha_beta5;
};

struct QuotConst {
  fe g;
  fe k[NW];
  fe zh_inv[8];
};

__global__ __launch_bounds__(kThreads) void k_pad_copy(fe* __restrict__ dst, size_t dst_outer, size_t dst_inner,
                                                       const fe* __restrict__ src, size_t src_outer, size_t src_inner,
                                                       uint32_t inner, size_t len, size_t total) {
  size_t k = (size_t)blockIdx.x * blockDim.x + threadIdx.x;
  if (k >= total) return;
  uint32_t q = blockIdx.y;
  size_t d = (size_t)(q / inner) * dst_outer + (size_t)(q % inner) * dst_inner + k;
  fe v = Fr::zero();
  if (k < len) v = src[(size_t)(q / inner) * src_outer + (size_t)(q % inner) * src_inner + k];
  dst[d] = v;
}

template <int SET_TAIL>
__global__ void k_blind(fe* __restrict__ polys, size_t stride, size_t n, const fe* __restrict__ blinders,
                        uint32_t inner, uint32_t bl_off, uint32_t nb, uint32_t count) {
  uint32_t t = threadIdx.x, q = blockIdx.x;
  if (q >= count) return;
  fe* p = polys + (size_t)q * stride;
  if (t >= nb) {
    if (SET_TAIL && t < 8 && n + t < stride) p[n + t] = Fr::zero();
    return;
  }
  fe b = blinders[(size_t)(q / inner) * 13 + bl_off + (size_t)(q % inner) * nb + t];
  p[t] = Fr::sub(p[t], b);
  p[n + t] = SET_TAIL ? b : Fr::add(p[n + t], b);
}

__global__ __launch_bounds__(kThreads) void k_stage_evals(const fe* __restrict__ evals, size_t src_stride, size_t n,
                                                          const fe* __restrict__ blinders, uint32_t inner,
                                                          uint32_t bl_off, uint32_t nb,
                                                          fe* __restrict__ dst ) {
  const size_t j = (size_t)blockIdx.x * blockDim.x + threadIdx.x;
  const uint32_t q = blockIdx.y;
  if (j >= n + nb) return;
  dst[(size_t)q * (n + nb) + j] =
      j < n ? evals[(size_t)q * src_stride + j]
            : blinders[(size_t)(q / inner) * 13 + bl_off + (size_t)(q % inner) * nb + (j - n)];
}

__global__ __launch_bounds__(kThreads) void k_perm_numden(const fe* __restrict__ wires ,
                                                          const fe* __restrict__ sig_eval ,
                                                          const fe* const* __restrict__ sig_of,
                                                          const fe* __restrict__ tw_n, const Chal* __restrict__ chal,
                                                          QuotConst qc29, size_t n, fe* __restrict__ num,
                                                          fe* __restrict__ den) {
  using F = Fr29;
  size_t j = (size_t)blockIdx.x * blockDim.x + threadIdx.x;
  if (j >= n) return;
  uint32_t p = blockIdx.y;
  if (sig_of) sig_eval = sig_of[p];
  const fl beta = F::from_ext(chal[p].beta);
  const fl gamma = F::load(chal[p].gamma);
  const fl bx = F::mul(beta, F::load(tw_n[j]));
  fl a, b;
#pragma unroll 1
  for (int i = 0; i < NW; i++) {
    const fl wg = F::add(F::load(wires[((size_t)p * NW + i) * n + j]), gamma);
    const fl t1 = F::normalize(F::add(wg, i == 0 ? bx : F::mul(F::load(qc29.k[i]), bx)));
    const fl t2 = F::normalize(F::add(wg, F::mul(beta, F::load(sig_eval[(size_t)i * n + j]))));
    a = i == 0 ? t1 : F::mul(a, t1);
    b = i == 0 ? t2 : F::mul(b, t2);
  }
  fl fix = F::one();
#pragma unroll 1
  for (int k = 0; k < 20; k++) fix = F::weak_reduce(F::add(fix, fix));
  num[(size_t)p * n + j] = F::pack(F::canonical(F::mul(a, fix)));
  den[(size_t)p * n + j] = F::pack(F::canonical(F::mul(b, fix)));
}

template <int OP>
__device__ __forceinline__ fe scan_op(const fe& a, const fe& b) {
  return OP == 0 ? Fr::mul(a, b) : Fr::add(a, b);
}
template <int OP>
__device__ __forceinline__ fe scan_identity() {
  return OP == 0 ? Fr::one() : Fr::zero();
}
__device__ __forceinline__ fe shfl_up_fe(const fe& a, int d) {
  fe r;
#pragma unroll
  for (int i = 0; i < 8; i++) r.v[i] = __shfl_up(a.v[i], d);
  return r;
}

template <int OP, int REV>
__global__ __launch_bounds__(kThreads) void k_scan_local(const fe* __restrict__ in, fe* __restrict__ out, size_t len,
                                                         size_t stride, fe* __restrict__ tot, uint32_t nblocks) {
  __shared__ fe wave_tot[kThreads / 64];
  const uint32_t b = blockIdx.y, blk = blockIdx.x;
  const fe* src = in + (size_t)b * stride;
  fe* dst = out + (size_t)b * stride;
  size_t k0 = (size_t)blk * kScanBlock + (size_t)threadIdx.x * kScanPerThread;
  fe v[kScanPerThread];
  fe run = scan_identity<OP>();
#pragma unroll
  for (int t = 0; t < kScanPerThread; t++) {
    size_t k = k0 + t;
    fe x = scan_identity<OP>();
    if (k < len) x = src[REV ? (len - 1 - k) : k];
    v[t] = run;
    run = t == 0 ? x : scan_op<OP>(run, x);
  }
  const uint32_t lane = threadIdx.x & 63, wave = threadIdx.x >> 6;
  fe inc = run;
  for (int d = 1; d < 64; d <<= 1) {
    fe o = shfl_up_fe(inc, d);
    if ((int)lane >= d) inc = scan_op<OP>(o, inc);
  }
  if (lane == 63) wave_tot[wave] = inc;
  fe excl = shfl_up_fe(inc, 1);
  if (lane == 0) excl = scan_identity<OP>();
  __syncthreads();
  fe wpre = scan_identity<OP>();
  for (uint32_t w = 0; w < wave; w++) wpre = scan_op<OP>(wpre, wave_tot[w]);
  fe base = scan_op<OP>(wpre, excl);
#pragma unroll
  for (int t = 0; t < kScanPerThread; t++) {
    size_t k = k0 + t;
    if (k < len) dst[REV ? (len - 1 - k) : k] = t == 0 ? base : scan_op<OP>(base, v[t]);
  }
  if (threadIdx.x == kThreads - 1) tot[(size_t)b * nblocks + blk] = scan_op<OP>(wpre, inc);
}

template <int OP>
__global__ __launch_bounds__(64) void k_scan_totals(fe* __restrict__ tot, uint32_t nblocks) {
  fe* t = tot + (size_t)blockIdx.x * nblocks;
  const uint32_t lane = threadIdx.x;
  fe carry = scan_identity<OP>();
  for (uint32_t base = 0; base < nblocks; base += 64) {
    uint32_t i = base + lane;
    fe x = i < nblocks ? t[i] : scan_identity<OP>();
    fe inc = x;
    for (int d = 1; d < 64; d <<= 1) {
      fe o = shfl_up_fe(inc, d);
      if ((int)lane >= d) inc = scan_op<OP>(o, inc);
    }
    fe excl = shfl_up_fe(inc, 1);
    if (lane == 0) excl = scan_identity<OP>();
    if (i < nblocks) t[i] = scan_op<OP>(carry, excl);
    fe last;
#pragma unroll
    for (int w = 0; w < 8; w++) last.v[w] = __shfl(inc.v[w], 63);
    carry = scan_op<OP>(carry, last);
  }
}

template <int OP, int REV>
__global__ __launch_bounds__(kThreads) void k_scan_apply(fe* __restrict__ out, size_t len, size_t stride,
                                                         const fe* __restrict__ tot, uint32_t nblocks) {
  const uint32_t b = blockIdx.y, blk = blockIdx.x;
  if (blk == 0) return;
  fe pre = tot[(size_t)b * nblocks + blk];
  fe* dst = out + (size_t)b * stride;
  for (int t = 0; t < kScanPerThread; t++) {
    size_t k = (size_t)blk * kScanBlock + (size_t)t * kThreads + threadIdx.x;
    if (k < len) {
      size_t idx = REV ? (len - 1 - k) : k;
      dst[idx] = scan_op<OP>(pre, dst[idx]);
    }
  }
}

__global__ void k_perm_total(const fe* __restrict__ sfx, const fe* __restrict__ den, size_t n, fe* __restrict__ total,
                             uint32_t count) {
  uint32_t p = blockIdx.x * blockDim.x + threadIdx.x;
  if (p >= count) return;
  total[p] = Fr::mul(sfx[(size_t)p * n], den[(size_t)p * n]);
}

__global__ void k_perm_inv_total(const fe* __restrict__ sfx, const fe* __restrict__ den, size_t n,
                                 fe* __restrict__ inv_total, uint32_t count) {
  uint32_t p = blockIdx.x * blockDim.x + threadIdx.x;
  if (p >= count) return;
  using F = Fl<FrP29, 0>;
  inv_total[p] = F::to_ext(F::inv(F::mul(F::from_ext(sfx[(size_t)p * n]), F::from_ext(den[(size_t)p * n]))));
}

__global__ __launch_bounds__(kThreads) void k_perm_finish(const fe* __restrict__ pre, const fe* __restrict__ sfx,
                                                          const fe* __restrict__ den,
                                                          const fe* __restrict__ inv_total, size_t n,
                                                          fe* __restrict__ z, size_t zstride) {
  size_t j = (size_t)blockIdx.x * blockDim.x + threadIdx.x;
  uint32_t p = blockIdx.y;
  if (j >= zstride) return;
  fe v = Fr::zero();
  if (j < n) {
    size_t o = (size_t)p * n + j;
    v = Fr::mul(Fr::mul(pre[o], sfx[o]), Fr::mul(den[o], inv_total[p]));
  }
  z[(size_t)p * zstride + j] = v;
}

struct ColAcc {
  uint64_t c[18];
  __device__ __forceinline__ void clear() {
#pragma unroll
    for (int k = 0; k < 18; k++) c[k] = 0;
  }
  __device__ __forceinline__ void mad(const fl& a, const fl& b) {
#pragma unroll
    for (int i = 0; i < 9; i++)
#pragma unroll
      for (int j = 0; j < 9; j++) c[i + j] += (uint64_t)a.v[i] * b.v[j];
  }
  __device__ __forceinline__ fl reduce() { return Fr29::reduce_cols(c); }
};

__global__ __launch_bounds__(kThreads) void k_kx_columns(fe* __restrict__ dst, const fe* __restrict__ xs, QuotConst qc,
                                                         size_t m) {
  using F = Fr29;
  size_t i = (size_t)blockIdx.x * blockDim.x + threadIdx.x;
  if (i >= m) return;
  const fl x = F::load(xs[i]);
#pragma unroll
  for (int j = 0; j < NKX; j++) dst[(size_t)j * m + i] = F::pack(F::canonical(F::mul(F::load(qc.k[j + 1]), x)));
}

__device__ __forceinline__ bool fe_nonzero(const fe& a) {
  uint32_t o = 0;
#pragma unroll
  for (int k = 0; k < 8; k++) o |= a.v[k];
  return o != 0;
}
template <bool FOLD>
__global__ __launch_bounds__(kThreads) void k_quotient(const fe* __restrict__ pkc, const fe* const* __restrict__ pkc_of,
                                                       const fe* __restrict__ cos, const fe* __restrict__ xs,
                                                       const fe* __restrict__ inv_nx1,
                                                       const Chal* __restrict__ chal, QuotConst qc, size_t m,
                                                       uint32_t only_unfoldable, fe* __restrict__ t_out) {
  using F = Fr29;
  size_t i = (size_t)blockIdx.y * blockDim.x + threadIdx.x;
  if (i >= m) return;
  const uint32_t p = blockIdx.x;
  if (FOLD ? !fe_nonzero(chal[p].beta_inv) : (only_unfoldable && fe_nonzero(chal[p].beta_inv))) return;
  if (pkc_of) pkc = pkc_of[p];
  const uint32_t mm = (uint32_t)(m / 3);
  const uint32_t blk = (i >= mm ? 1u : 0u) + (i >= 2 * (size_t)mm ? 1u : 0u);
  const fe* c = cos + (size_t)p * 6 * m;
  auto sel = [&](int s) { return F::load(pkc[(size_t)s * m + i]); };
  fl w0 = F::load(c[i]), w1 = F::load(c[m + i]), w2 = F::load(c[2 * m + i]), w3 = F::load(c[3 * m + i]),
     w4 = F::load(c[4 * m + i]);
  fl w01 = F::mul(w0, w1), w23 = F::mul(w2, w3);
  ColAcc acc;
  acc.clear();
  acc.mad(sel(0), w0);
  acc.mad(sel(1), w1);
  acc.mad(sel(2), w2);
  acc.mad(sel(3), w3);
  acc.mad(sel(4), w01);
  acc.mad(sel(5), w23);
  fl gate = acc.reduce();
  acc.clear();
  {
    fl t = F::sqr(w0);
    acc.mad(sel(6), F::mul(F::sqr(t), w0));
    t = F::sqr(w1);
    acc.mad(sel(7), F::mul(F::sqr(t), w1));
    t = F::sqr(w2);
    acc.mad(sel(8), F::mul(F::sqr(t), w2));
    t = F::sqr(w3);
    acc.mad(sel(9), F::mul(F::sqr(t), w3));
  }
  acc.mad(sel(12), F::mul(F::mul(w01, w23), w4));
  acc.mad(F::neg(sel(10)), w4);
  fl gate2 = acc.reduce();
  fl total = F::normalize(F::add(F::add(gate, gate2), sel(11)));
  const fl gamma = F::load(chal[p].gamma);
  const fl zx = F::load(c[5 * m + i]);
  const uint32_t k1 = (uint32_t)i - blk * mm;
  const size_t inext = (size_t)blk * mm + ((k1 + 2) & (mm - 1));
  if constexpr (FOLD) {
    const fl beta_inv = F::load(chal[p].beta_inv);
    fl a = zx, b = F::load(c[5 * m + inext]);
    fl u = F::mul(F::add(w0, gamma), beta_inv);
    a = F::mul(a, F::add(u, F::load(xs[i])));
    b = F::mul(b, F::add(u, sel(NS + 0)));
    u = F::mul(F::add(w1, gamma), beta_inv);
    a = F::mul(a, F::add(u, sel(NS + NW + 0)));
    b = F::mul(b, F::add(u, sel(NS + 1)));
    u = F::mul(F::add(w2, gamma), beta_inv);
    a = F::mul(a, F::add(u, sel(NS + NW + 1)));
    b = F::mul(b, F::add(u, sel(NS + 2)));
    u = F::mul(F::add(w3, gamma), beta_inv);
    a = F::mul(a, F::add(u, sel(NS + NW + 2)));
    b = F::mul(b, F::add(u, sel(NS + 3)));
    u = F::mul(F::add(w4, gamma), beta_inv);
    a = F::mul(a, F::add(u, sel(NS + NW + 3)));
    b = F::mul(b, F::add(u, sel(NS + 4)));
    total = F::normalize(F::add(total, F::mul(F::load(chal[p].alpha_beta5), F::sub(a, b))));
  } else {
    const fl beta = F::load(chal[p].beta);
    fl x = F::load(xs[i]);
    fl bx = F::mul(beta, x);
    fl a = zx, b = F::load(c[5 * m + inext]);
    fl wg = F::add(w0, gamma);
    a = F::mul(a, F::normalize(F::add(wg, bx)));
    b = F::mul(b, F::normalize(F::add(wg, F::mul(beta, sel(NS + 0)))));
    wg = F::add(w1, gamma);
    a = F::mul(a, F::normalize(F::add(wg, F::mul(F::load(qc.k[1]), bx))));
    b = F::mul(b, F::normalize(F::add(wg, F::mul(beta, sel(NS + 1)))));
    wg = F::add(w2, gamma);
    a = F::mul(a, F::normalize(F::add(wg, F::mul(F::load(qc.k[2]), bx))));
    b = F::mul(b, F::normalize(F::add(wg, F::mul(beta, sel(NS + 2)))));
    wg = F::add(w3, gamma);
    a = F::mul(a, F::normalize(F::add(wg, F::mul(F::load(qc.k[3]), bx))));
    b = F::mul(b, F::normalize(F::add(wg, F::mul(beta, sel(NS + 3)))));
    wg = F::add(w4, gamma);
    a = F::mul(a, F::normalize(F::add(wg, F::mul(F::load(qc.k[4]), bx))));
    b = F::mul(b, F::normalize(F::add(wg, F::mul(beta, sel(NS + 4)))));
    total = F::normalize(F::add(total, F::mul(F::load(chal[p].alpha), F::sub(a, b))));
  }
  fl l1a = F::mul(F::load(chal[p].alpha2), F::sub(zx, F::one()));
  const uint32_t zi = 3 * (((uint32_t)i - blk * mm) & 1) + blk;
  fl r = F::mul_add_mul(total, F::load(qc.zh_inv[zi]), l1a, F::load(inv_nx1[i]));
  t_out[(size_t)p * m + i] = F::store(r);
}

__global__ __launch_bounds__(kThreads) void k_inv_nx1(fe* __restrict__ out, const fe* __restrict__ xs, fe n_mont,
                                                      size_t m) {
  size_t i = (size_t)blockIdx.x * blockDim.x + threadIdx.x;
  if (i >= m) return;
  out[i] = Fr::inv(Fr::mul(n_mont, Fr::sub(xs[i], Fr::one())));
}

__global__ __launch_bounds__(kThreads) void k_check_degree(const fe* __restrict__ t, size_t m, size_t lo,
                                                           uint32_t* __restrict__ flags) {
  size_t k = lo - 1 + (size_t)blockIdx.x * blockDim.x + threadIdx.x;
  if (k >= m) return;
  uint32_t p = blockIdx.y;
  bool zero = Fr::is_zero(t[(size_t)p * m + k]);
  if (k == lo - 1) {
    if (zero) atomicOr(&flags[p], 2u);
  } else if (!zero) {
    atomicOr(&flags[p], 1u);
  }
}

constexpr uint32_t kPowLow = 256;
__global__ __launch_bounds__(kThreads) void k_powers_small(fe* __restrict__ small, uint32_t small_len,
                                                           const fe* __restrict__ pw) {
  uint32_t i = blockIdx.x * blockDim.x + threadIdx.x;
  if (i >= small_len) return;
  uint32_t q = blockIdx.y;
  const fe* b = pw + (size_t)q * 24;
  const uint32_t e = i < kPowLow ? i : (i - kPowLow) * kPowLow;
  fe r = Fr::one();
  bool started = false;
  for (int k = 0; (e >> k) != 0; k++) {
    if ((e >> k) & 1) {
      r = started ? Fr::mul(r, b[k]) : b[k];
      started = true;
    }
  }
  small[(size_t)q * small_len + i] = r;
}
__global__ __launch_bounds__(kThreads) void k_powers(fe* __restrict__ tables, size_t stride, size_t len,
                                                     const fe* __restrict__ small, uint32_t small_len) {
  size_t e = (size_t)blockIdx.x * blockDim.x + threadIdx.x;
  if (e >= len) return;
  uint32_t q = blockIdx.y;
  const fe* t = small + (size_t)q * small_len;
  tables[(size_t)q * stride + e] = Fr::mul(t[e & (kPowLow - 1)], t[kPowLow + (e >> 8)]);
}

struct EvalDesc {
  const fe* poly;
  const fe* pows;
  uint32_t len;
  uint32_t pad;
};

__device__ __forceinline__ fe wave_sum(fe v) {
  for (int d = 32; d >= 1; d >>= 1) {
    fe o;
#pragma unroll
    for (int i = 0; i < 8; i++) o.v[i] = __shfl_down(v.v[i], d);
    v = Fr::add(v, o);
  }
  return v;
}

__global__ __launch_bounds__(kThreads) void k_eval_partial(const EvalDesc* __restrict__ desc, fe* __restrict__ partial,
                                                           uint32_t chunks, uint32_t per_chunk) {
  __shared__ fe sh[kThreads / 64];
  const uint32_t e = blockIdx.y, chunk = blockIdx.x;
  const EvalDesc d = desc[e];
  fe acc = Fr::zero();
  uint32_t lo = chunk * per_chunk, hi = lo + per_chunk;
  if (hi > d.len) hi = d.len;
  for (uint32_t k = lo + threadIdx.x; k < hi; k += kThreads) acc = Fr::add(acc, Fr::mul(d.poly[k], d.pows[k]));
  acc = wave_sum(acc);
  if ((threadIdx.x & 63) == 0) sh[threadIdx.x >> 6] = acc;
  __syncthreads();
  if (threadIdx.x == 0) {
    fe r = sh[0];
    for (int w = 1; w < kThreads / 64; w++) r = Fr::add(r, sh[w]);
    partial[(size_t)e * chunks + chunk] = r;
  }
}
__global__ __launch_bounds__(64) void k_eval_final(const fe* __restrict__ partial, uint32_t chunks,
                                                   fe* __restrict__ out) {
  const uint32_t e = blockIdx.x;
  fe acc = Fr::zero();
  for (uint32_t k = threadIdx.x; k < chunks; k += 64) acc = Fr::add(acc, partial[(size_t)e * chunks + k]);
  acc = wave_sum(acc);
  if (threadIdx.x == 0) out[e] = acc;
}

struct LinTerm {
  const fe* poly;
  fe scalar;
  uint32_t len;
  uint32_t pad[3];
};

__global__ __launch_bounds__(kThreads) void k_lincomb(const LinTerm* __restrict__ terms, uint32_t nterms,
                                                      fe* __restrict__ out, size_t out_stride, size_t out_len) {
  using F = Fr29;
  size_t k = (size_t)blockIdx.x * blockDim.x + threadIdx.x;
  if (k >= out_len) return;
  uint32_t p = blockIdx.y;
  const LinTerm* T = terms + (size_t)p * nterms;
  fl total = F::zero();
  for (uint32_t t0 = 0; t0 < nterms; t0 += 6) {
    ColAcc acc;
    acc.clear();
#pragma unroll
    for (uint32_t u = 0; u < 6; u++) {
      const uint32_t t = t0 + u;
      if (t < nterms && k < T[t].len) acc.mad(F::load(T[t].scalar), F::load(T[t].poly[k]));
    }
    total = F::normalize(F::add(total, acc.reduce()));
  }
  out[(size_t)p * out_stride + k] = F::pack(F::canonical(total));
}

__global__ __launch_bounds__(kThreads) void k_div_prepare(const fe* __restrict__ f, const fe* __restrict__ pows,
                                                          size_t stride, size_t len, fe* __restrict__ h) {
  size_t k = (size_t)blockIdx.x * blockDim.x + threadIdx.x;
  if (k >= len) return;
  uint32_t q = blockIdx.y;
  size_t tab = (size_t)(q / 2) * 4 + (q % 2);
  h[(size_t)q * stride + k] = Fr::mul(f[(size_t)q * stride + k], pows[tab * stride + k]);
}
__global__ __launch_bounds__(kThreads) void k_div_finish(const fe* __restrict__ sfx, const fe* __restrict__ pows,
                                                         size_t stride, size_t len, fe* __restrict__ quot) {
  size_t i = (size_t)blockIdx.x * blockDim.x + threadIdx.x;
  if (i >= stride) return;
  uint32_t q = blockIdx.y;
  size_t tab = (size_t)(q / 2) * 4 + 2 + (q % 2);
  fe v = Fr::zero();
  if (i + 1 < len) v = Fr::mul(sfx[(size_t)q * stride + i], pows[tab * stride + i + 1]);
  quot[(size_t)q * stride + i] = v;
}

}
}
```

cap_amd/csrc/prove_run.hpp:

```cpp
#pragma once
#include "check_kernels.hpp"
#include "context.hpp"
#include "host_util.hpp"
#include "launch.hpp"
#include "outcome.hpp"
#include "params.hpp"
#include "plonk_kernels.hpp"
#include "transcript_dev.hpp"
#include "vars_kernels.hpp"

namespace cap {
namespace {

inline unsigned cdiv(size_t a, size_t b) { return (unsigned)((a + b - 1) / b); }

void pad_copy(hipStream_t s, fe* dst, size_t dst_outer, size_t dst_inner, const fe* src, size_t src_outer,
              size_t src_inner, uint32_t inner, uint32_t count, size_t len, size_t total) {
  if (count == 0 || total == 0) return;
  launch("k_pad_copy", k_pad_copy, dim3(cdiv(total, kThreads), count), dim3(kThreads), 0, s, dst, dst_outer, dst_inner,
         src, src_outer, src_inner, inner, len, total);
}

template <int OP, int REV>
void scan_exclusive(hipStream_t s, const fe* in, fe* out, size_t len, size_t stride, uint32_t batch, fe* tot) {
  uint32_t nblocks = cdiv(len, kScanBlock);
  launch(OP == 0 ? "k_scan_local_mul" : "k_scan_local_add", k_scan_local<OP, REV>, dim3(nblocks, batch), dim3(kThreads),
         0, s, in, out, len, stride, tot, nblocks);
  if (nblocks > 1) {
    launch("k_scan_totals", k_scan_totals<OP>, dim3(batch), dim3(64), 0, s, tot, nblocks);
    launch("k_scan_apply", k_scan_apply<OP, REV>, dim3(nblocks, batch), dim3(kThreads), 0, s, out, len, stride,
           (const fe*)tot, nblocks);
  }
}

inline size_t ntt_scratch_inplace(size_t stride, size_t count) { return sizeof(fe) * stride * count; }
inline size_t ntt_scratch_from(uint32_t log_n, size_t count) { return (sizeof(fe) << log_n) * count; }
inline size_t ntt3_scratch(uint32_t log_mm, size_t count) { return (sizeof(fe) << log_mm) * 6 * count; }
inline size_t wires_stage_bytes(size_t cnt, size_t n) { return sizeof(fe) * cnt * NW * n; }

int run_ntt(hipStream_t s, uint32_t log_n, fe* data, size_t stride, uint32_t count, int dir, int coset) {
  Context& c = ctx();
  const NttDomain* dom = nullptr;
  int rc = get_domain(log_n, &dom);
  if (rc) return rc;
  rc = scratch_reserve(c.ntt_scratch, ntt_scratch_inplace(stride, count));
  if (rc) return rc;
  rc = ntt_run(*dom, c.small, data, (fe*)c.ntt_scratch.p, stride, count, dir, coset, s);
  if (rc) return hip_fail((hipError_t)rc, "ntt_run");
  return CAPGPU_OK;
}

int run_ntt_from(hipStream_t s, uint32_t log_n, const fe* src, size_t src_stride, size_t src_len, fe* dst,
                 size_t dst_stride, uint32_t count, int dir, int coset, const fe* post_scalar = nullptr) {
  Context& c = ctx();
  const NttDomain* dom = nullptr;
  int rc = get_domain(log_n, &dom);
  if (rc) return rc;
  rc = scratch_reserve(c.ntt_scratch, ntt_scratch_from(log_n, count));
  if (rc) return rc;
  NttIo io{};
  io.src = src;
  io.src_outer = src_stride;
  io.src_inner = 0;
  io.src_group = 1;
  io.src_len = src_len;
  io.dst_outer = dst_stride;
  io.dst_inner = 0;
  io.dst_group = 1;
  if (post_scalar) {
    io.has_post_scalar = 1;
    io.post_scalar = *post_scalar;
  }
  rc = ntt_run(*dom, c.small, dst, (fe*)c.ntt_scratch.p, dst_stride, count, dir, coset, s, &io);
  if (rc) return hip_fail((hipError_t)rc, "ntt_run");
  return CAPGPU_OK;
}

int quot_domains(uint32_t log_mm, const Ntt3Domain** d3, const NttDomain** dm) {
  int rc = get_domain3(log_mm, d3);
  if (rc) return rc;
  return get_domain(log_mm, dm);
}
int run_ntt3_fwd(hipStream_t s, uint32_t log_mm, fe* data, uint32_t count, const NttIo& io) {
  Context& c = ctx();
  const Ntt3Domain* d3 = nullptr;
  const NttDomain* dm = nullptr;
  int rc = quot_domains(log_mm, &d3, &dm);
  if (rc) return rc;
  if ((rc = scratch_reserve(c.ntt_scratch, ntt3_scratch(log_mm, count)))) return rc;
  rc = ntt3_forward(*d3, *dm, c.small, data, io, count, (fe*)c.ntt_scratch.p, s);
  if (rc) return hip_fail((hipError_t)rc, "ntt3_forward");
  return CAPGPU_OK;
}
int run_ntt3_inv(hipStream_t s, uint32_t log_mm, fe* data, uint32_t count, const fe* add = nullptr) {
  Context& c = ctx();
  const Ntt3Domain* d3 = nullptr;
  const NttDomain* dm = nullptr;
  int rc = quot_domains(log_mm, &d3, &dm);
  if (rc) return rc;
  if ((rc = scratch_reserve(c.ntt_scratch, ntt3_scratch(log_mm, count)))) return rc;
  rc = ntt3_inverse(*d3, *dm, c.small, data, count, (fe*)c.ntt_scratch.p, s, add);
  if (rc) return hip_fail((hipError_t)rc, "ntt3_inverse");
  return CAPGPU_OK;
}

int run_msm(hipStream_t s, const MsmBases& B, const fe* scalars, size_t outer_stride, uint32_t inner,
            size_t inner_stride, size_t n, uint32_t batch, g1_jac* d_out) {
  Context& c = ctx();
  auto local = [&](size_t lo, size_t len) -> int {
    int rc = scratch_reserve(c.msm_ws, msm_workspace_bytes(B, len, batch));
    if (rc) return rc;
    rc = msm_run(B, lo, scalars + lo, outer_stride, inner, inner_stride, len, batch, 1, d_out, c.msm_ws.p, c.msm_ws.cap, s);
    return rc ? hip_fail((hipError_t)rc, "msm_run") : CAPGPU_OK;
  };
  if (!comm_shard_prover()) return local(0, n);
  const size_t world = (size_t)comm_world();
  const bool loop = comm_loopback();
  for (size_t rank = loop ? 0 : (size_t)comm_rank(), last = loop ? world - 1 : rank; rank <= last; rank++) {
    if (loop) comm_loopback_rank((int)rank);
    const size_t base = n / world, rem = n % world;
    const size_t lo = rank * base + std::min(rank, rem), len = base + (rank < rem ? 1 : 0);
    int rc = comm_allgather_sum(d_out, batch, s, local(lo, len));
    if (rc) return rc;
  }
  return CAPGPU_OK;
}

struct Carver {
  char* base;
  size_t off = 0;
  explicit Carver(void* b) : base((char*)b) {}
  template <class T>
  T* take(size_t count) {
    off = (off + 255) / 256 * 256;
    T* p = base ? (T*)(base + off) : nullptr;
    off += sizeof(T) * count;
    return p;
  }
};

struct BatchWs {
  fe *wpoly, *wev, *pi, *num, *den, *pre, *sfx, *scan_tot, *inv_total, *zpoly, *coset, *pkc, *t, *pows, *pows_small, *pw, *batchpoly,
      *hbuf, *quot, *evals, *eval_partial, *d_pub, *d_blind;
  Chal* chal;
  Chal* chal29;
  uint32_t* flags;
  g1_jac* comms;
  EvalDesc* edesc;
  LinTerm* terms;
  const fe** key_ptrs;
  uint8_t *d_proofs, *tr_state, *tr_pre, *tr_app;
  uint32_t* tr_pre_len;
  fe* zeta;
  unsigned long long* chk_first;
  int32_t* status;
  size_t total;
};
constexpr uint32_t kEvalChunks = 16;
constexpr uint32_t kLinTerms = 29;
static_assert(oc::kCheckNoFault == pk::kNoFault && sizeof(pk::CheckOut::first) == sizeof(unsigned long long),
              "k_prove_outcomes reads the witness check's verdicts (CheckOut::first)");
static_assert(kLinTerms == (uint32_t)td::kLinScalars, "transcript_dev.hpp derives the scalars of k_lincomb's terms");

BatchWs carve(void* base, const ProvingKey& K, uint32_t P, size_t num_inputs, bool coeffs, uint32_t tr_stride = 0) {
  Carver c(base);
  BatchWs w{};
  size_t n = K.n, m = K.m, ps = K.ps;
  w.wpoly = c.take<fe>((size_t)P * NW * ps);
  w.wev = coeffs ? c.take<fe>((size_t)P * NW * n) : nullptr;
  w.pi = num_inputs ? c.take<fe>((size_t)P * n) : nullptr;
  w.num = c.take<fe>((size_t)P * n);
  w.den = c.take<fe>((size_t)P * n);
  w.pre = c.take<fe>((size_t)P * n);
  w.sfx = c.take<fe>((size_t)P * n);
  w.scan_tot = c.take<fe>((size_t)P * 2 * (cdiv(ps, kScanBlock) + 1));
  w.inv_total = c.take<fe>(P);
  w.zpoly = c.take<fe>((size_t)P * ps);
  w.coset = c.take<fe>((size_t)P * 6 * m);
  w.pkc = K.recompute ? c.take<fe>((size_t)kPkcCols * m) : nullptr;
  w.t = c.take<fe>((size_t)P * m);
  w.pows = c.take<fe>((size_t)P * 4 * ps);
  w.pw = c.take<fe>((size_t)P * 4 * 24);
  w.pows_small = c.take<fe>((size_t)P * 4 * (kPowLow + (ps + kPowLow - 1) / kPowLow));
  w.batchpoly = c.take<fe>((size_t)P * 2 * ps);
  w.hbuf = c.take<fe>((size_t)P * 2 * ps);
  w.quot = c.take<fe>((size_t)P * 2 * ps);
  w.evals = c.take<fe>((size_t)P * 10);
  w.eval_partial = c.take<fe>((size_t)P * 10 * kEvalChunks);
  w.d_pub = c.take<fe>((size_t)P * (num_inputs ? num_inputs : 1));
  w.d_blind = c.take<fe>((size_t)P * 13);
  w.chal = c.take<Chal>(P);
  w.chal29 = c.take<Chal>(P);
  w.flags = c.take<uint32_t>(P);
  w.comms = c.take<g1_jac>((size_t)P * 5);
  w.edesc = c.take<EvalDesc>((size_t)P * 10);
  w.terms = c.take<LinTerm>((size_t)P * kLinTerms);
  w.key_ptrs = c.take<const fe*>((size_t)P * 2);
  if (tr_stride) {
    w.d_proofs = c.take<uint8_t>((size_t)P * td::kPrBytes);
    w.zeta = c.take<fe>(P);
    w.tr_state = c.take<uint8_t>((size_t)P * 64);
    w.tr_app = c.take<uint8_t>((size_t)P * td::kAppBytes);
    w.tr_pre_len = c.take<uint32_t>(P);
    w.tr_pre = c.take<uint8_t>((size_t)P * tr_stride);
    w.chk_first = c.take<unsigned long long>(P);
    w.status = c.take<int32_t>(P);
  }
  w.total = c.off + 256;
  return w;
}

int compute_pk_coset(hipStream_t s, const ProvingKey& K, fe* dst) {
  return run_ntt3_fwd(s, K.log_m, dst, 18, NttIo{K.coef, K.ps, 0, K.n, 1, K.m, 0, 1});
}
int compute_pk_kx(hipStream_t s, const ProvingKey& K, fe* dst) {
  const Ntt3Domain* dq = nullptr;
  if (int rc = get_domain3(K.log_m, &dq)) return rc;
  launch("k_kx_columns", k_kx_columns, dim3(cdiv(K.m, kThreads)), dim3(kThreads), 0, s, dst + (size_t)18 * K.m,
         (const fe*)dq->xs29, K.qc29, K.m);
  return CAPGPU_OK;
}
int quotient_fold() {
  return env_int("CAPGPU_QUOT_FOLD", 1, 0, 2);
}

std::atomic<int> g_wire_commit{-1};
bool wire_commit_from_evals() {
  static const int env_default = [] {
    const char* e = getenv("CAPGPU_WIRE_COMMIT");
    return (e && (!strcmp(e, "coeffs") || !strcmp(e, "0"))) ? 0 : 1;
  }();
  const int m = g_wire_commit.load(std::memory_order_relaxed);
  return (m < 0 ? env_default : m) != 0;
}

std::atomic<int> g_transcript{-1};
int transcript_mode() {
  static const int env_default = [] {
    const char* e = getenv("CAPGPU_TRANSCRIPT");
    return (e && (!strcmp(e, "device") || !strcmp(e, "1"))) ? CAPGPU_TRANSCRIPT_DEVICE : CAPGPU_TRANSCRIPT_HOST;
  }();
  const int m = g_transcript.load(std::memory_order_relaxed);
  return m < 0 ? env_default : m;
}
bool perm_inv_on_device() {
  static const bool on = env_int("CAPGPU_PERM_INV_ON_DEVICE", 0) != 0;
  return on;
}
std::atomic<int> g_precheck{0};
thread_local bool tl_prechecked = false;

hipStream_t h2d_stream() {
  Context& c = ctx();
  if (!c.copy_stream && hipStreamCreateWithFlags(&c.copy_stream, hipStreamNonBlocking) != hipSuccess)
    c.copy_stream = nullptr;
  return c.copy_stream;
}
uint32_t r1_overlap_max() {
  static const uint32_t v = [] {
    const int x = env_int("CAPGPU_R1_OVERLAP_MAX", 3);
    return (uint32_t)(x < 0 ? 0 : (x > 4096 ? 4096 : x));
  }();
  return v;
}
hipStream_t side_stream(Context& c) {
  if (!c.side_stream) {
    if (hipStreamCreateWithFlags(&c.side_stream, hipStreamNonBlocking) != hipSuccess) c.side_stream = nullptr;
    if (c.side_stream && (hipEventCreateWithFlags(&c.ev_fork, hipEventDisableTiming) != hipSuccess ||
                          hipEventCreateWithFlags(&c.ev_join, hipEventDisableTiming) != hipSuccess)) {
      (void)hipStreamDestroy(c.side_stream);
      c.side_stream = nullptr;
    }
    (void)hipGetLastError();
  }
  return c.side_stream;
}
struct H2dTurn {
  std::mutex mu;
  std::condition_variable cv;
  uint32_t next = 0;
  bool wait_for(uint32_t idx, uint32_t timeout_ms) {
    std::unique_lock<std::mutex> lk(mu);
    return cv.wait_for(lk, std::chrono::milliseconds(timeout_ms), [&] { return next >= idx; });
  }
  void pass(uint32_t idx) {
    std::lock_guard<std::mutex> lk(mu);
    if (next < idx + 1) next = idx + 1;
    cv.notify_all();
  }
};
thread_local H2dTurn* tl_h2d_turn = nullptr;
thread_local uint32_t tl_h2d_index = 0;
static bool h2d_in_part_order() {
  static const bool on = env_int("CAPGPU_H2D_PART_ORDER", 1) != 0;
  return on;
}

uint32_t h2d_chunks(uint32_t P) {
  static const int forced = env_int("CAPGPU_PROVE_CHUNKS", 0, 1, 16);
  if (forced) return std::min<uint32_t>((uint32_t)forced, P);
  return P >= 64 ? 4u : (P >= 32 ? 2u : 1u);
}
uint32_t h2d_chunk_start(uint32_t P, uint32_t chunks, uint32_t ck, bool short_first) {
  static const uint32_t first = (uint32_t)env_int("CAPGPU_PROVE_FIRST_CHUNK", 16, 0, 4096);
  if (ck == 0) return 0;
  if (ck >= chunks) return P;
  if (!short_first || first == 0 || chunks < 3 || first * chunks >= P) return (uint32_t)((uint64_t)P * ck / chunks);
  return first + (uint32_t)((uint64_t)(P - first) * (ck - 1) / (chunks - 1));
}

std::atomic<uint64_t> g_witness_h2d{0}, g_gather_launches{0};
inline void count_witness_h2d(size_t bytes) { g_witness_h2d.fetch_add(bytes, std::memory_order_relaxed); }

inline size_t vars_stage_bytes(size_t cnt, size_t n, size_t stride, bool host) {
  return wires_stage_bytes(cnt, n) + (host ? sizeof(fe) * cnt * stride : 0);
}
struct VarsIn {
  const fe* d_vars;
  size_t stride;
};
bool key_lacks_table(const ProvingKey& K) {
  if (K.wire_vars) return false;
  set_error("capgpu_plonk: CAPGPU_INPUT_VARS: key has no variable table (capgpu_plonk_preprocess_vars or "
            "capgpu_plonk_key_set_vars gives it one)");
  return true;
}
void gather_vars(hipStream_t s, const ProvingKey& K, const std::vector<const ProvingKey*>* keys, uint32_t p0, uint32_t cnt,
                 const VarsIn& in, fe* d_cols) {
  const size_t cells = (size_t)NW * K.n;
  for (uint32_t p = p0; p < p0 + cnt;) {
    uint32_t q = p0 + cnt;
    if (keys)
      for (q = p + 1; q < p0 + cnt && (*keys)[q] == (*keys)[p];) q++;
    const ProvingKey& Kp = keys ? *(*keys)[p] : K;
    const uint32_t rows = std::min<uint32_t>(q - p, (uint32_t)std::max<size_t>(1, ((size_t)1 << 20) / (2 * cells)));
    launch("k_gather_vars", k_gather_vars, dim3(cdiv(2 * cells, kThreads), rows), dim3(kThreads), 0, s,
           (const uint4*)(in.d_vars + (size_t)p * in.stride), in.stride, (const uint32_t*)Kp.wire_vars, cells, q - p,
           (uint4*)(d_cols + (size_t)p * cells));
    g_gather_launches.fetch_add(1, std::memory_order_relaxed);
    p = q;
  }
}

size_t prove_pinned_bytes(uint32_t P, bool dev_tr) {
  if (dev_tr) return (size_t)P * td::kPrBytes + sizeof(uint32_t) * P + sizeof(int32_t) * P + 768;
  return sizeof(g1_jac) * P * NW + sizeof(fe) * P * 11 + sizeof(uint32_t) * P + 1024;
}
uint32_t transcript_stride(size_t longest) { return (uint32_t)((longest + 256) / 256 * 256); }

struct ProvePlan {
  uint32_t P = 0;
  int form = CAPGPU_INPUT_EVALS;
  bool coeffs = false, vars = false;
  bool host = false;
  bool r1_copies = false;
  bool precheck = false;
  bool dev_tr = false;
  uint32_t tr_stride = 0;
  bool inv_on_device = false;
  uint32_t chunks = 1;
  bool overlap = false;
  hipStream_t s2 = nullptr;
  bool graphs = false;
  const MsmBases* B = nullptr;
  const MsmBases* Lag = nullptr;
  const MsmBases& wire_key() const { return Lag ? *Lag : *B; }
};

int make_plan(Context& c, const ProvingKey& K, uint32_t P, int form, bool host, size_t longest_prefix, bool sizing,
              ProvePlan* out) {
  ProvePlan pl;
  pl.P = P;
  pl.form = form;
  pl.coeffs = form == CAPGPU_INPUT_COEFFS;
  pl.vars = form == CAPGPU_INPUT_VARS;
  pl.host = host;
  int rc = find_srs(K.srs_handle, &pl.B);
  if (rc) return rc;
  pl.precheck = g_precheck.load(std::memory_order_relaxed) != 0 && (sizing || !tl_prechecked);
  pl.r1_copies = host && !pl.precheck;
  if (wire_commit_from_evals() && !comm_shard_prover() && (rc = find_lagrange(K.srs_handle, K.log_n, &pl.Lag))) {
    if (rc == CAPGPU_ERR_BAD_HANDLE) return rc;
    pl.Lag = nullptr;
    (void)hipGetLastError();
    if (!sizing) trace("pb_lagrange_fallback", c.slot, rc);
  }
  pl.dev_tr = transcript_mode() == CAPGPU_TRANSCRIPT_DEVICE && !comm_shard_prover();
  if (pl.dev_tr) {
    if (longest_prefix > (1u << 30)) {
      set_error("capgpu_plonk_prove: transcript init message of %zu bytes", longest_prefix);
      return CAPGPU_ERR_INVALID_ARG;
    }
    pl.tr_stride = transcript_stride(longest_prefix);
  }
  pl.inv_on_device = perm_inv_on_device() || pl.dev_tr;
  pl.chunks = pl.r1_copies ? h2d_chunks(P) : 1;
  const bool own = !c.prof.on && c.stream == c.own_stream;
  pl.overlap = pl.chunks == 1 && P <= r1_overlap_max() && (sizing || (own && !comm_shard_prover())) &&
               (pl.s2 = side_stream(c)) != nullptr;
  pl.graphs = P <= graph_max_batch() && pl.chunks == 1 && own && comm_shard_slot() < 0 && quotient_fold() == 1;
  *out = pl;
  return CAPGPU_OK;
}

struct ProveNeeds {
  size_t prove_ws = 0, msm_ws = 0, ntt_scratch = 0, stage_a = 0, stage_b = 0, pinned = 0;
  void ntt(size_t bytes) { ntt_scratch = std::max(ntt_scratch, bytes); }
  void msm(const MsmBases& T, size_t len, uint32_t batch) { msm_ws = std::max(msm_ws, msm_workspace_bytes(T, len, batch)); }
};

struct ProveRequest {
  const fe* d_wires = nullptr;
  const uint64_t* pub_inputs = nullptr;
  size_t num_inputs = 0;
  const uint64_t* blinders = nullptr;
  capgpu_proof* proofs = nullptr;
  const uint8_t* ext_msg = nullptr;
  size_t ext_len = 0;
  const uint8_t* const* msgs = nullptr;
  const size_t* msg_lens = nullptr;
  const std::vector<const ProvingKey*>* keys = nullptr;
  const uint64_t* const* h_wires = nullptr;
  int form = CAPGPU_INPUT_EVALS;
  const VarsIn* vin = nullptr;
  capgpu_prove_outcome* outcomes = nullptr;
};

struct ProveRun {
  struct SideDrain {
    Context& c;
    bool armed;
    ~SideDrain() {
      if (armed && c.side_stream) (void)hipStreamSynchronize(c.side_stream);
    }
  } side_drain;
  Context& c;
  const hipStream_t s;
  const ProvePlan& pl;
  const ProvingKey& K;
  const ProveRequest& rq;
  BatchWs w{};
  ProveGraphSet* gs = nullptr;
  const uint32_t P;
  const size_t n, m, ps, num_inputs;
  const fe* const d_wires;
  const uint64_t* pub_inputs;
  const uint64_t* const* h_wires;
  const NttDomain* dom_n = nullptr;
  const Ntt3Domain* dom_q = nullptr;
  const fe omega;
  std::vector<uint64_t> pub_rows;
  std::vector<const fe*> key_ptrs;
  const fe* const* sig_of = nullptr;
  const fe* const* pkc_of = nullptr;
  std::vector<SolidityTranscript> tr;
  g1_jac* hj = nullptr;
  fe* h_tot = nullptr;
  bool beta_zero_possible = true;
  fe* h_evals = nullptr;
  uint32_t* h_flags = nullptr;
  uint8_t* h_proofs = nullptr;
  int32_t* h_status = nullptr;
  const capgpu_witness_fault* faults = nullptr;
  const size_t proofs_bytes;
  std::vector<g1_affine> ha;

  ProveRun(Context& c_, const ProvePlan& pl_, const ProvingKey& K_, const ProveRequest& rq_)
      : side_drain{c_, false}, c(c_), s(c_.stream), pl(pl_), K(K_), rq(rq_), P(pl_.P), n(K_.n), m(K_.m), ps(K_.ps),
        num_inputs(rq_.num_inputs), d_wires(rq_.d_wires), pub_inputs(rq_.pub_inputs),
        h_wires(pl_.r1_copies ? rq_.h_wires : nullptr), omega(ntt_root_of_unity(K_.log_n)),
        proofs_bytes((size_t)pl_.P * td::kPrBytes) {}
  ProveRun(const ProveRun&) = delete;
  ProveRun& operator=(const ProveRun&) = delete;

  const ProvingKey& key_of(uint32_t p) const { return rq.keys ? *(*rq.keys)[p] : K; }
  template <class F>
  int seg(int id, F&& enqueue) {
    return run_segment(c, gs, id, enqueue);
  }
  hipError_t wait_stream() {
    g_stream_waits++;
    return hipStreamSynchronize(s);
  }
  static void needs(const ProvePlan& pl, const ProvingKey& K, ProveNeeds& nd) {
    input_needs(pl, K, nd);
    begin_needs(pl, K, nd);
    if (pl.chunks > 1) {
      for (int short_first = 0; short_first < 2; short_first++)
        for (uint32_t ck = 0; ck < pl.chunks; ck++) {
          const uint32_t cnt = h2d_chunk_start(pl.P, pl.chunks, ck + 1, short_first != 0) -
                               h2d_chunk_start(pl.P, pl.chunks, ck, short_first != 0);
          if (cnt) r1_chunk_needs(pl, K, cnt, nd);
        }
    } else {
      r1_chunk_needs(pl, K, pl.P, nd);
      r1_overlapped_needs(pl, K, pl.P, nd);
    }
    r1_tail_needs(pl, K, pl.P, nd);
    cosets_needs(pl, K, pl.P, nd);
    commit_z_needs(pl, K, pl.P, nd);
    r3_needs(pl, K, pl.P, nd);
    r5_needs(pl, K, pl.P, nd);
  }

  size_t in_elems() const { return pl.vars ? rq.vin->stride : (size_t)NW * n; }
  size_t in_len(uint32_t p) const { return pl.vars ? key_of(p).num_vars : in_elems(); }
  int copy_input(uint32_t p0, uint32_t p1, hipStream_t st) {
    const size_t elems = in_elems();
    fe* const in_dst = const_cast<fe*>(pl.vars ? rq.vin->d_vars : d_wires);
    for (uint32_t p = p0; p < p1;) {
      uint32_t q = p + 1;
      while (q < p1 && in_len(q - 1) == elems && rq.h_wires[q] == rq.h_wires[q - 1] + (size_t)4 * elems) q++;
      const size_t bytes = sizeof(fe) * ((size_t)(q - 1 - p) * elems + in_len(q - 1));
      CAP_HIP(hipMemcpyAsync(in_dst + (size_t)p * elems, rq.h_wires[p], bytes, hipMemcpyHostToDevice, st));
      count_witness_h2d(bytes);
      p = q;
    }
    return CAPGPU_OK;
  }
  void gather_vars(uint32_t p0, uint32_t cnt) { cap::gather_vars(s, K, rq.keys, p0, cnt, *rq.vin, const_cast<fe*>(d_wires)); }
  static void input_needs(const ProvePlan& pl, const ProvingKey& K, ProveNeeds& nd) {
    if (pl.host) nd.stage_b = wires_stage_bytes(pl.P, K.n);
    if (pl.vars) nd.stage_b = vars_stage_bytes(pl.P, K.n, K.num_vars, pl.host);
  }
  int copy_chunks() {
    int rc;
    H2dTurn* const turn = h_wires ? tl_h2d_turn : nullptr;
    const uint32_t turn_idx = tl_h2d_index;
    if (turn) {
      const bool in_time = turn->wait_for(turn_idx, 100);
      trace("pb_h2d_turn", c.slot, in_time ? (int64_t)turn_idx : -1);
    }
    const bool short_first = h_wires && (!turn || turn_idx == 0);
    for (uint32_t ck = 0; ck < pl.chunks; ck++) {
      const uint32_t p0 = h2d_chunk_start(P, pl.chunks, ck, short_first), p1 = h2d_chunk_start(P, pl.chunks, ck + 1, short_first);
      if (h_wires) {
        hipStream_t cs = pl.chunks > 1 ? h2d_stream() : nullptr;
        if (!cs) cs = s;
        if (cs != s && ck == 0) {
          hipEvent_t ev;
          CAP_HIP(hipEventCreateWithFlags(&ev, hipEventDisableTiming));
          hipError_t e1 = hipEventRecord(ev, s), e2 = e1 == hipSuccess ? hipStreamWaitEvent(cs, ev, 0) : e1;
          (void)hipEventDestroy(ev);
          CAP_HIP(e2);
        }
        trace("pb_h2d_issue", c.slot, ck);
        if ((rc = copy_input(p0, p1, cs))) return rc;
        trace("pb_h2d_issued", c.slot, ck);
        if (cs != s) {
          hipEvent_t ev;
          CAP_HIP(hipEventCreateWithFlags(&ev, hipEventDisableTiming));
          hipError_t e1 = hipEventRecord(ev, cs), e2 = e1 == hipSuccess ? hipStreamWaitEvent(s, ev, 0) : e1;
          (void)hipEventDestroy(ev);
          CAP_HIP(e2);
        }
        if (pl.vars) gather_vars(p0, p1 - p0);
      }
      if (pl.chunks > 1 && (rc = r1_chunk_kernels(p0, p1 - p0, true))) return rc;
    }
    if (turn) {
      if (pl.chunks > 1 && c.copy_stream) CAP_HIP(hipStreamSynchronize(c.copy_stream));
      turn->pass(turn_idx);
    }
    return CAPGPU_OK;
  }

  int begin() {
    int rc;
    side_drain.armed = pl.overlap;
    if ((rc = get_domain(K.log_n, &dom_n))) return rc;
    if ((rc = get_domain3(K.log_m, &dom_q))) return rc;
    g_prove_calls++;
    if (!pl.dev_tr) {
      tr.resize(P);
      parallel_for(P, [&](uint32_t p) {
        if (rq.msgs) {
          if (rq.msgs[p] && rq.msg_lens[p]) tr[p].append(rq.msgs[p], rq.msg_lens[p]);
        } else if (rq.ext_msg && rq.ext_len) {
          tr[p].append(rq.ext_msg, rq.ext_len);
        }
        const ProvingKey& Kp = key_of(p);
        tr[p].append(Kp.vk_bytes.data(), Kp.vk_bytes.size());
        for (size_t i = 0; i < Kp.num_inputs; i++) append_fr(tr[p], fe_from_words(pub_inputs + 4 * (p * num_inputs + i)));
      });
    }
    if (rq.keys && num_inputs) {
      pub_rows.assign(pub_inputs, pub_inputs + (size_t)4 * P * num_inputs);
      for (uint32_t p = 0; p < P; p++)
        for (size_t i = key_of(p).num_inputs; i < num_inputs; i++)
          for (int k = 0; k < 4; k++) pub_rows[4 * (p * num_inputs + i) + k] = 0;
      pub_inputs = pub_rows.data();
    }
    if (num_inputs)
      CAP_HIP(hipMemcpyAsync(w.d_pub, pub_inputs, sizeof(fe) * P * num_inputs, hipMemcpyHostToDevice, s));
    if (rq.keys) {
      key_ptrs.resize((size_t)2 * P);
      for (uint32_t p = 0; p < P; p++) {
        key_ptrs[p] = key_of(p).sig_eval;
        key_ptrs[P + p] = key_of(p).pk_coset;
      }
      CAP_HIP(hipMemcpyAsync(w.key_ptrs, key_ptrs.data(), sizeof(const fe*) * key_ptrs.size(), hipMemcpyHostToDevice, s));
      sig_of = w.key_ptrs;
      pkc_of = w.key_ptrs + P;
    }
    CAP_HIP(hipMemcpyAsync(w.d_blind, rq.blinders, sizeof(fe) * P * 13, hipMemcpyHostToDevice, s));
    CAP_HIP(hipMemsetAsync(w.flags, 0, sizeof(uint32_t) * P, s));
    if ((rc = pinned_reserve(c, prove_pinned_bytes(P, pl.dev_tr)))) return rc;
    if (pl.dev_tr) {
      h_proofs = (uint8_t*)c.pin_host;
      h_flags = (uint32_t*)(h_proofs + (proofs_bytes + 255) / 256 * 256);
      h_status = (int32_t*)((char*)h_flags + (sizeof(uint32_t) * P + 255) / 256 * 256);
    } else {
      char* b = (char*)c.pin_host;
      hj = (g1_jac*)b;
      b += (sizeof(g1_jac) * P * NW + 255) / 256 * 256;
      h_tot = (fe*)b;
      b += (sizeof(fe) * P + 255) / 256 * 256;
      h_evals = (fe*)b;
      b += (sizeof(fe) * P * 10 + 255) / 256 * 256;
      h_flags = (uint32_t*)b;
    }
    return copy_chunks();
  }
  static void begin_needs(const ProvePlan& pl, const ProvingKey& K, ProveNeeds& nd) {
    nd.prove_ws = carve(nullptr, K, pl.P, K.num_inputs, pl.coeffs, pl.tr_stride).total;
    nd.pinned = prove_pinned_bytes(pl.P, pl.dev_tr);
  }

  int fetch_comms(uint32_t count, const std::function<int()>& keep_busy = nullptr) {
    CAP_HIP(hipMemcpyAsync(hj, w.comms, sizeof(g1_jac) * count, hipMemcpyDeviceToHost, s));
    CAP_HIP(wait_stream());
    if (keep_busy) {
      int brc = keep_busy();
      if (brc) return brc;
    }
    ha.resize(count);
    const uint32_t chunk = 64, nchunks = (count + chunk - 1) / chunk;
    parallel_for(nchunks, [&](uint32_t ci) {
      const uint32_t lo = ci * chunk, hi = std::min(count, lo + chunk);
      std::vector<g1_jac> in(hj + lo, hj + hi);
      std::vector<g1_affine> out;
      batch_to_affine(in, out);
      std::copy(out.begin(), out.end(), ha.begin() + lo);
    });
    return CAPGPU_OK;
  }
  int degree_verdict(const uint32_t* flags) const {
    for (uint32_t p = 0; p < P; p++) {
      if (flags[p]) {
        char b[256];
        oc::degree_text(p, flags[p], b, sizeof b);
        set_error("%s", b);
        return CAPGPU_ERR_PROOF;
      }
    }
    return CAPGPU_OK;
  }
  void host_outcomes(const uint32_t* flags) const {
    for (uint32_t p = 0; p < P; p++) oc::finish_outcome(flags[p], faults ? &faults[p] : nullptr, &rq.outcomes[p], &rq.proofs[p]);
  }

  int commit_wires(uint32_t p0, uint32_t cnt) {
    g1_jac* out = w.comms + (size_t)p0 * NW;
    if (!pl.Lag) return run_msm(s, *pl.B, w.wpoly + (size_t)p0 * NW * ps, ps, 1, 0, n + 2, cnt * NW, out);
    fe* stage = w.t + (size_t)p0 * NW * (n + 2);
    const fe* ev = (pl.coeffs ? (const fe*)w.wev : d_wires) + (size_t)p0 * NW * n;
    launch("k_stage_evals", k_stage_evals, dim3(cdiv(n + 2, kThreads), cnt * NW), dim3(kThreads), 0, s, ev, n, n,
           (const fe*)(w.d_blind + (size_t)p0 * 13), (uint32_t)NW, 0u, 2u, stage);
    return run_msm(s, *pl.Lag, stage, n + 2, 1, 0, n + 2, cnt * NW, out);
  }
  int r1_chunk_kernels(uint32_t p0, uint32_t cnt, bool commit) {
    const size_t wo = (size_t)p0 * NW * n;
    fe* wp = w.wpoly + (size_t)p0 * NW * ps;
    int r;
    if (pl.coeffs) {
      pad_copy(s, wp, ps, 0, d_wires + wo, n, 0, 1, cnt * NW, n, n);
      if ((r = run_ntt_from(s, K.log_n, d_wires + wo, n, n, w.wev + wo, n, cnt * NW, 0, 0))) return r;
    } else if ((r = run_ntt_from(s, K.log_n, d_wires + wo, n, n, wp, ps, cnt * NW, 1, 0))) {
      return r;
    }
    launch("k_blind", k_blind<1>, dim3(cnt * NW), dim3(64), 0, s, wp, ps, n, (const fe*)(w.d_blind + (size_t)p0 * 13),
           (uint32_t)NW, 0u, 2u, cnt * NW);
    if (commit && (r = commit_wires(p0, cnt))) return r;
    return CAPGPU_OK;
  }
  static void r1_chunk_needs(const ProvePlan& pl, const ProvingKey& K, uint32_t cnt, ProveNeeds& nd) {
    nd.ntt(ntt_scratch_from(K.log_n, (size_t)cnt * NW));
    nd.msm(pl.wire_key(), K.n + 2, cnt * NW);
  }
  int pi_fold(hipStream_t st) {
    if (!num_inputs) return CAPGPU_OK;
    return run_ntt_from(st, K.log_n, w.d_pub, num_inputs, num_inputs, w.pi, n, P, 1, 0, &dom_q->kappa_n_inv29);
  }
  int r1_tail_kernels() {
    int r;
    if ((r = pi_fold(s))) return r;
    if (pl.chunks == 1 && (r = commit_wires(0, P))) return r;
    return CAPGPU_OK;
  }
  static void r1_tail_needs(const ProvePlan&, const ProvingKey& K, uint32_t cnt, ProveNeeds& nd) {
    if (K.num_inputs) nd.ntt(ntt_scratch_from(K.log_n, cnt));
  }
  int r3_wire_cosets(hipStream_t st) {
    return run_ntt3_fwd(st, K.log_m, w.coset, P * NW, NttIo{w.wpoly, NW * ps, ps, n + 2, NW, 6 * m, m, NW});
  }
  int z_cosets(hipStream_t st) {
    return run_ntt3_fwd(st, K.log_m, w.coset + 5 * m, P, NttIo{w.zpoly, ps, 0, n + 3, 1, 6 * m, 0, 1});
  }
  static void cosets_needs(const ProvePlan&, const ProvingKey& K, uint32_t cnt, ProveNeeds& nd) {
    nd.ntt(ntt3_scratch(K.log_m, (size_t)cnt * NW));
    nd.ntt(ntt3_scratch(K.log_m, cnt));
  }
  int r1_overlapped() {
    int r;
    const hipStream_t s2 = pl.s2;
    if ((r = scratch_reserve(c.ntt_scratch, ntt3_scratch(K.log_m, (size_t)P * NW)))) return r;
    auto interpolate_and_blind = [&](hipStream_t st) -> int {
      int q = CAPGPU_OK;
      if (pl.coeffs) pad_copy(st, w.wpoly, ps, 0, d_wires, n, 0, 1, P * NW, n, n);
      else q = run_ntt_from(st, K.log_n, d_wires, n, n, w.wpoly, ps, P * NW, 1, 0);
      if (q) return q;
      launch("k_blind", k_blind<1>, dim3(P * NW), dim3(64), 0, st, w.wpoly, ps, n, (const fe*)w.d_blind, (uint32_t)NW, 0u,
             2u, P * NW);
      return CAPGPU_OK;
    };
    if (pl.coeffs && (r = run_ntt_from(s, K.log_n, d_wires, n, n, w.wev, n, P * NW, 0, 0))) return r;
    if (!pl.Lag && (r = interpolate_and_blind(s))) return r;
    CAP_HIP(hipEventRecord(c.ev_fork, s));
    CAP_HIP(hipStreamWaitEvent(s2, c.ev_fork, 0));
    if (pl.Lag && (r = interpolate_and_blind(s2))) return r;
    if ((r = pi_fold(s2))) return r;
    if ((r = r3_wire_cosets(s2))) return r;
    if ((r = commit_wires(0, P))) return r;
    CAP_HIP(hipEventRecord(c.ev_join, s2));
    CAP_HIP(hipStreamWaitEvent(s, c.ev_join, 0));
    return CAPGPU_OK;
  }
  static void r1_overlapped_needs(const ProvePlan& pl, const ProvingKey& K, uint32_t cnt, ProveNeeds& nd) {
    if (pl.overlap) nd.ntt(ntt3_scratch(K.log_m, (size_t)cnt * NW));
  }
  int r1_body() {
    if (pl.overlap) return r1_overlapped();
    int r = pl.chunks == 1 ? r1_chunk_kernels(0, P, false) : CAPGPU_OK;
    return r ? r : r1_tail_kernels();
  }

  int finish_and_commit_z() {
    int r;
    const hipStream_t s2 = pl.s2;
    const MsmBases* const Lag = pl.Lag;
    launch("k_perm_finish", k_perm_finish, dim3(cdiv(ps, kThreads), P), dim3(kThreads), 0, s, (const fe*)w.pre,
           (const fe*)w.sfx, (const fe*)w.den, (const fe*)w.inv_total, n, w.zpoly, ps);
    auto interpolate_and_blind = [&](hipStream_t st) -> int {
      int q = run_ntt(st, K.log_n, w.zpoly, ps, P, 1, 0);
      if (q) return q;
      launch("k_blind", k_blind<0>, dim3(P), dim3(64), 0, st, w.zpoly, ps, n, (const fe*)w.d_blind, 1u, 10u, 3u, P);
      return CAPGPU_OK;
    };
    if (Lag) {
      launch("k_stage_evals", k_stage_evals, dim3(cdiv(n + 3, kThreads), P), dim3(kThreads), 0, s, (const fe*)w.zpoly, ps, n,
             (const fe*)w.d_blind, 1u, 10u, 3u, w.t);
    }
    if (!pl.overlap) {
      if ((r = interpolate_and_blind(s))) return r;
      return Lag ? run_msm(s, *Lag, w.t, n + 3, 1, 0, n + 3, P, w.comms) : run_msm(s, *pl.B, w.zpoly, ps, 1, 0, n + 3, P, w.comms);
    }
    if (!Lag && (r = interpolate_and_blind(s))) return r;
    CAP_HIP(hipEventRecord(c.ev_fork, s));
    CAP_HIP(hipStreamWaitEvent(s2, c.ev_fork, 0));
    if (Lag && (r = interpolate_and_blind(s2))) return r;
    if ((r = z_cosets(s2))) return r;
    r = Lag ? run_msm(s, *Lag, w.t, n + 3, 1, 0, n + 3, P, w.comms) : run_msm(s, *pl.B, w.zpoly, ps, 1, 0, n + 3, P, w.comms);
    CAP_HIP(hipEventRecord(c.ev_join, s2));
    CAP_HIP(hipStreamWaitEvent(s, c.ev_join, 0));
    return r;
  }
  static void commit_z_needs(const ProvePlan& pl, const ProvingKey& K, uint32_t cnt, ProveNeeds& nd) {
    nd.ntt(ntt_scratch_inplace(K.ps, cnt));
    nd.msm(pl.wire_key(), K.n + 3, cnt);
  }
  int r2_body() {
    launch("k_perm_numden", k_perm_numden, dim3(cdiv(n, kThreads), P), dim3(kThreads), 0, s,
           pl.coeffs ? (const fe*)w.wev : d_wires, (const fe*)K.sig_eval, sig_of, (const fe*)dom_n->tw_fwd,
           (const Chal*)w.chal, K.qc29, n, w.num, w.den);
    {
      uint32_t nb = cdiv(n, kScanBlock);
      scan_exclusive<0, 0>(s, w.num, w.pre, n, n, P, w.scan_tot);
      scan_exclusive<0, 1>(s, w.den, w.sfx, n, n, P, w.scan_tot + (size_t)P * nb);
    }
    if (pl.inv_on_device) {
      launch("k_perm_inv_total", k_perm_inv_total, dim3(cdiv(P, 64)), dim3(64), 0, s, (const fe*)w.sfx,
             (const fe*)w.den, n, w.inv_total, P);
    } else {
      launch("k_perm_total", k_perm_total, dim3(cdiv(P, 64)), dim3(64), 0, s, (const fe*)w.sfx, (const fe*)w.den, n,
             w.inv_total, P);
      return CAPGPU_OK;
    }
    return finish_and_commit_z();
  }

  int r3_body() {
    int r;
    const fe* pkc = K.pk_coset;
    if (K.recompute) {
      for (uint32_t p = 0; p < P; p++)
        if ((r = compute_pk_coset(s, K, w.pkc))) return r;
      if ((r = compute_pk_kx(s, K, w.pkc))) return r;
      pkc = w.pkc;
    }
    const int fold = quotient_fold();
    if (fold == 2)
      CAP_HIP(hipMemset2DAsync(&w.chal29[0].beta_inv, sizeof(Chal), 0, sizeof(fe), P, s));
    if (fold)
      launch("k_quotient", k_quotient<true>, dim3(P, cdiv(m, kThreads)), dim3(kThreads), 0, s, pkc, pkc_of,
             (const fe*)w.coset, (const fe*)dom_q->xs29, (const fe*)K.inv_nx1, (const Chal*)w.chal29, K.qc29, m, 1u, w.t);
    if (!fold || fold == 2 || beta_zero_possible)
      launch("k_quotient_direct", k_quotient<false>, dim3(P, cdiv(m, kThreads)), dim3(kThreads), 0, s,
             pkc, pkc_of, (const fe*)w.coset, (const fe*)dom_q->xs29, (const fe*)K.inv_nx1, (const Chal*)w.chal29, K.qc29, m,
             fold ? 1u : 0u, w.t);
    if ((r = run_ntt3_inv(s, K.log_m, w.t, P, w.pi))) return r;
    {
      size_t lo = NW * (n + 1) + 3;
      launch("k_check_degree", k_check_degree, dim3(cdiv(m - (lo - 1), kThreads), P), dim3(kThreads), 0, s,
             (const fe*)w.t, m, lo, w.flags);
    }
    return run_msm(s, *pl.B, w.t, m, NW, n + 2, n + 2, P * NW, w.comms);
  }
  static void r3_needs(const ProvePlan& pl, const ProvingKey& K, uint32_t cnt, ProveNeeds& nd) {
    if (K.recompute) nd.ntt(ntt3_scratch(K.log_m, 18));
    nd.ntt(ntt3_scratch(K.log_m, cnt));
    nd.msm(*pl.B, K.n + 2, cnt * NW);
  }

  std::vector<EvalDesc> make_edesc() const {
    std::vector<EvalDesc> ed((size_t)P * 10);
    for (uint32_t p = 0; p < P; p++) {
      const fe* pz = w.pows + ((size_t)p * 4 + 0) * ps;
      const fe* pzw = w.pows + ((size_t)p * 4 + 1) * ps;
      for (int i = 0; i < NW; i++) ed[p * 10 + i] = EvalDesc{w.wpoly + ((size_t)p * NW + i) * ps, pz, (uint32_t)(n + 2), 0};
      for (int i = 0; i < NW - 1; i++)
        ed[p * 10 + NW + i] = EvalDesc{key_of(p).coef + (size_t)(NS + i) * ps, pz, (uint32_t)n, 0};
      ed[p * 10 + 9] = EvalDesc{w.zpoly + (size_t)p * ps, pzw, (uint32_t)(n + 3), 0};
    }
    return ed;
  }
  int r4_body() {
    const uint32_t small_len = kPowLow + cdiv(ps, kPowLow);
    launch("k_powers_small", k_powers_small, dim3(cdiv(small_len, kThreads), P * 4), dim3(kThreads), 0, s,
           w.pows_small, small_len, (const fe*)w.pw);
    launch("k_powers", k_powers, dim3(cdiv(ps, kThreads), P * 4), dim3(kThreads), 0, s, w.pows, ps, ps,
           (const fe*)w.pows_small, small_len);
    uint32_t per_chunk = cdiv(n + 3, kEvalChunks);
    launch("k_eval_partial", k_eval_partial, dim3(kEvalChunks, P * 10), dim3(kThreads), 0, s,
           (const EvalDesc*)w.edesc, w.eval_partial, kEvalChunks, per_chunk);
    launch("k_eval_final", k_eval_final, dim3(P * 10), dim3(64), 0, s, (const fe*)w.eval_partial, kEvalChunks,
           w.evals);
    return CAPGPU_OK;
  }

  void term_polys(uint32_t p, LinTerm* T) const {
    int t = 0;
    auto add = [&](const fe* poly, size_t len) {
      T[t].poly = poly;
      T[t].len = (uint32_t)len;
      t++;
    };
    const fe* const coef = key_of(p).coef;
    for (int j = 0; j < NS; j++) add(coef + (size_t)j * ps, n);
    add(w.zpoly + (size_t)p * ps, n + 3);
    add(coef + (size_t)(NS + NW - 1) * ps, n);
    for (int j = 0; j < NW; j++) add(w.t + (size_t)p * m + (size_t)j * (n + 2), n + 2);
    for (int j = 0; j < NW; j++) add(w.wpoly + ((size_t)p * NW + j) * ps, n + 2);
    for (int j = 0; j < NW - 1; j++) add(coef + (size_t)(NS + j) * ps, n);
  }
  int r5_body() {
    launch("k_lincomb", k_lincomb, dim3(cdiv(ps, kThreads), P), dim3(kThreads), 0, s, (const LinTerm*)w.terms,
           kLinTerms, w.batchpoly, 2 * ps, ps);
    pad_copy(s, w.batchpoly + ps, 2 * ps, 0, w.zpoly, ps, 0, 1, P, n + 3, ps);
    launch("k_div_prepare", k_div_prepare, dim3(cdiv(n + 3, kThreads), P * 2), dim3(kThreads), 0, s,
           (const fe*)w.batchpoly, (const fe*)w.pows, ps, n + 3, w.hbuf);
    scan_exclusive<1, 1>(s, w.hbuf, w.batchpoly, n + 3, ps, P * 2, w.scan_tot);
    launch("k_div_finish", k_div_finish, dim3(cdiv(ps, kThreads), P * 2), dim3(kThreads), 0, s,
           (const fe*)w.batchpoly, (const fe*)w.pows, ps, n + 3, w.quot);
    return run_msm(s, *pl.B, w.quot, ps, 1, 0, n + 2, P * 2, w.comms);
  }
  static void r5_needs(const ProvePlan& pl, const ProvingKey& K, uint32_t cnt, ProveNeeds& nd) {
    nd.msm(*pl.B, K.n + 2, cnt * 2);
  }

  int run_device_transcript() {
    int rc;
    if ((rc = begin())) return rc;
    const uint32_t tr_stride = pl.tr_stride;
    std::vector<uint8_t> h_pre((size_t)P * tr_stride, 0);
    std::vector<uint32_t> h_pre_len(P);
    parallel_for(P, [&](uint32_t p) {
      uint8_t* b = &h_pre[(size_t)p * tr_stride];
      size_t o = 0;
      auto put = [&](const void* src, size_t len) {
        memcpy(b + o, src, len);
        o += len;
      };
      if (rq.msgs) {
        if (rq.msgs[p] && rq.msg_lens[p]) put(rq.msgs[p], rq.msg_lens[p]);
      } else if (rq.ext_msg && rq.ext_len) {
        put(rq.ext_msg, rq.ext_len);
      }
      const ProvingKey& Kp = key_of(p);
      put(Kp.vk_bytes.data(), Kp.vk_bytes.size());
      for (size_t i = 0; i < Kp.num_inputs; i++) {
        uint8_t e[32];
        serialize_fr(fe_from_words(pub_inputs + 4 * (p * num_inputs + i)), e);
        put(e, 32);
      }
      h_pre_len[p] = (uint32_t)o;
    });
    CAP_HIP(hipMemcpyAsync(w.tr_pre, h_pre.data(), h_pre.size(), hipMemcpyHostToDevice, s));
    CAP_HIP(hipMemcpyAsync(w.tr_pre_len, h_pre_len.data(), sizeof(uint32_t) * P, hipMemcpyHostToDevice, s));
    CAP_HIP(hipMemsetAsync(w.tr_state, 0, (size_t)P * 64, s));
    const std::vector<EvalDesc> ed = make_edesc();
    CAP_HIP(hipMemcpyAsync(w.edesc, ed.data(), sizeof(EvalDesc) * ed.size(), hipMemcpyHostToDevice, s));
    std::vector<LinTerm> terms((size_t)P * kLinTerms);
    memset((void*)terms.data(), 0, sizeof(LinTerm) * terms.size());
    for (uint32_t p = 0; p < P; p++) term_polys(p, &terms[(size_t)p * kLinTerms]);
    CAP_HIP(hipMemcpyAsync(w.terms, terms.data(), sizeof(LinTerm) * terms.size(), hipMemcpyHostToDevice, s));
    const td::TrBufs tb{w.tr_state, w.tr_pre, w.tr_pre_len, w.tr_app, tr_stride};
    td::LinIn lin_base;
    memset((void*)&lin_base, 0, sizeof lin_base);
    for (int i = 0; i < NW; i++) lin_base.k[i] = K.qc.k[i];
    lin_base.n = n;
    if ((rc = seg(0, [&]() -> int {
           int r;
           if ((r = r1_body())) return r;
           launch("k_tr_comms_r1", td::k_tr_comms<1>, dim3(P), dim3(64), 0, s, tb, (const g1_jac*)w.comms, w.d_proofs, w.chal,
                  w.chal29, w.zeta, w.pw, omega, P);
           if (!pl.overlap && (r = r3_wire_cosets(s))) return r;
           if ((r = r2_body())) return r;
           launch("k_tr_comms_r2", td::k_tr_comms<2>, dim3(P), dim3(64), 0, s, tb, (const g1_jac*)w.comms, w.d_proofs, w.chal,
                  w.chal29, w.zeta, w.pw, omega, P);
           if (!pl.overlap && (r = z_cosets(s))) return r;
           if ((r = r3_body())) return r;
           launch("k_tr_comms_r3", td::k_tr_comms<3>, dim3(P), dim3(64), 0, s, tb, (const g1_jac*)w.comms, w.d_proofs, w.chal,
                  w.chal29, w.zeta, w.pw, omega, P);
           if ((r = r4_body())) return r;
           launch("k_tr_evals", td::k_tr_evals, dim3(P), dim3(64), 0, s, tb, (const fe*)w.evals, w.d_proofs,
                  (const Chal*)w.chal, (const fe*)w.zeta, w.terms, lin_base, P);
           if ((r = r5_body())) return r;
           launch("k_tr_open", td::k_tr_open, dim3(cdiv(P, 64)), dim3(64), 0, s, (const g1_jac*)w.comms, w.d_proofs, P);
           if (rq.outcomes)
             launch("k_prove_outcomes", oc::k_prove_outcomes, dim3(P), dim3(64), 0, s, P, (const uint32_t*)w.flags,
                    faults ? (const unsigned long long*)w.chk_first : nullptr, w.status, w.d_proofs);
           return CAPGPU_OK;
         })))
      return rc;
    uint32_t* flags = h_flags;
    CAP_HIP(hipMemcpyAsync(h_proofs, w.d_proofs, proofs_bytes, hipMemcpyDeviceToHost, s));
    CAP_HIP(hipMemcpyAsync(flags, w.flags, sizeof(uint32_t) * P, hipMemcpyDeviceToHost, s));
    if (rq.outcomes) CAP_HIP(hipMemcpyAsync(h_status, w.status, sizeof(int32_t) * P, hipMemcpyDeviceToHost, s));
    CAP_HIP(wait_stream());
    trace("pb_r5_done", c.slot);
    if ((rc = take_launch_error())) return rc;
    if (rq.outcomes) {
      for (uint32_t p = 0; p < P; p++) {
        capgpu_prove_outcome& o = rq.outcomes[p];
        memset(&o, 0, sizeof o);
        o.status = h_status[p];
        o.degree_flags = flags[p];
        if (faults) o.fault = faults[p];
      }
    } else if ((rc = degree_verdict(flags))) {
      return rc;
    }
    memcpy(rq.proofs, h_proofs, proofs_bytes);
    side_drain.armed = false;
    return CAPGPU_OK;
  }

  int run_host_transcript() {
    int rc;
    if ((rc = begin())) return rc;
    capgpu_proof* const proofs = rq.proofs;
    if ((rc = seg(0, [&]() -> int { return r1_body(); }))) return rc;
    if ((rc = fetch_comms(P * NW, [&]() -> int {
           if (pl.overlap) return CAPGPU_OK;
           return seg(1, [&]() -> int { return r3_wire_cosets(s); });
         })))
      return rc;
    trace("pb_r1_done", c.slot);
    std::vector<Chal> chal(P);
    parallel_for(P, [&](uint32_t p) {
      for (int i = 0; i < NW; i++) {
        append_g1(tr[p], ha[p * NW + i]);
        affine_to_words(ha[p * NW + i], proofs[p].wires_poly_comms[i]);
      }
      (void)get_challenge(tr[p]);
      chal[p].beta = get_challenge(tr[p]);
      chal[p].gamma = get_challenge(tr[p]);
      chal[p].alpha = Fr::zero();
      chal[p].alpha2 = Fr::zero();
      chal[p].beta_inv = Fr::is_zero(chal[p].beta) ? Fr::zero() : Fr::inv(chal[p].beta);
      chal[p].alpha_beta5 = Fr::zero();
    });
    beta_zero_possible = pl.graphs;
    for (uint32_t p = 0; p < P; p++) beta_zero_possible = beta_zero_possible || Fr::is_zero(chal[p].beta);
    CAP_HIP(hipMemcpyAsync(w.chal, chal.data(), sizeof(Chal) * P, hipMemcpyHostToDevice, s));

    if ((rc = seg(2, [&]() -> int { return r2_body(); }))) return rc;
    if (!pl.inv_on_device) {
      std::vector<fe> pref(P);
      fe* tot = h_tot;
      CAP_HIP(hipMemcpyAsync(tot, w.inv_total, sizeof(fe) * P, hipMemcpyDeviceToHost, s));
      CAP_HIP(wait_stream());
      fe acc = Fr::one();
      for (uint32_t p = 0; p < P; p++) {
        pref[p] = acc;
        if (!Fr::is_zero(tot[p])) acc = Fr::mul(acc, tot[p]);
      }
      acc = Fr::inv_fermat(acc);
      for (uint32_t p = P; p-- > 0;) {
        if (Fr::is_zero(tot[p])) continue;
        const fe inv_p = Fr::mul(acc, pref[p]);
        acc = Fr::mul(acc, tot[p]);
        tot[p] = inv_p;
      }
      CAP_HIP(hipMemcpyAsync(w.inv_total, tot, sizeof(fe) * P, hipMemcpyHostToDevice, s));
      if ((rc = seg(7, [&]() -> int { return finish_and_commit_z(); }))) return rc;
    }
    if ((rc = fetch_comms(P, [&]() -> int {
           if (pl.overlap) return CAPGPU_OK;
           return seg(3, [&]() -> int { return z_cosets(s); });
         })))
      return rc;
    trace("pb_r2_done", c.slot);
    parallel_for(P, [&](uint32_t p) {
      append_g1(tr[p], ha[p]);
      affine_to_words(ha[p], proofs[p].prod_perm_poly_comm);
      chal[p].alpha = get_challenge(tr[p]);
      chal[p].alpha2 = Fr::sqr(chal[p].alpha);
      const fe b2 = Fr::sqr(chal[p].beta);
      chal[p].alpha_beta5 = Fr::mul(chal[p].alpha, Fr::mul(Fr::sqr(b2), chal[p].beta));
    });
    CAP_HIP(hipMemcpyAsync(w.chal, chal.data(), sizeof(Chal) * P, hipMemcpyHostToDevice, s));
    std::vector<Chal> chal29(P);
    parallel_for(P, [&](uint32_t p) {
      auto conv = [](const fe& a) { return Fr29::pack(Fr29::canonical(Fr29::from_ext(a))); };
      chal29[p].beta = conv(chal[p].beta);
      chal29[p].gamma = conv(chal[p].gamma);
      chal29[p].alpha = conv(chal[p].alpha);
      chal29[p].alpha2 = conv(chal[p].alpha2);
      chal29[p].beta_inv = conv(chal[p].beta_inv);
      chal29[p].alpha_beta5 = conv(chal[p].alpha_beta5);
    });
    CAP_HIP(hipMemcpyAsync(w.chal29, chal29.data(), sizeof(Chal) * P, hipMemcpyHostToDevice, s));

    if ((rc = seg(4, [&]() -> int { return r3_body(); }))) return rc;
    uint32_t* flags = h_flags;
    CAP_HIP(hipMemcpyAsync(flags, w.flags, sizeof(uint32_t) * P, hipMemcpyDeviceToHost, s));
    if ((rc = fetch_comms(P * NW))) return rc;
    trace("pb_r3_done", c.slot);
    if (!rq.outcomes && (rc = degree_verdict(flags))) return rc;
    std::vector<fe> zeta(P);
    std::vector<fe> pw((size_t)P * 4 * 24);
    parallel_for(P, [&](uint32_t p) {
      for (int i = 0; i < NW; i++) {
        append_g1(tr[p], ha[p * NW + i]);
        affine_to_words(ha[p * NW + i], proofs[p].split_quot_poly_comms[i]);
      }
      zeta[p] = get_challenge(tr[p]);
      fe bases4[4];
      td::zeta_bases(zeta[p], omega, bases4);
      for (int q = 0; q < 4; q++) {
        fe x = bases4[q];
        for (int b = 0; b < 24; b++) {
          pw[((size_t)p * 4 + q) * 24 + b] = x;
          x = Fr::sqr(x);
        }
      }
    });

    CAP_HIP(hipMemcpyAsync(w.pw, pw.data(), sizeof(fe) * pw.size(), hipMemcpyHostToDevice, s));
    const std::vector<EvalDesc> ed = make_edesc();
    CAP_HIP(hipMemcpyAsync(w.edesc, ed.data(), sizeof(EvalDesc) * ed.size(), hipMemcpyHostToDevice, s));
    if ((rc = seg(5, [&]() -> int { return r4_body(); }))) return rc;
    fe* evals = h_evals;
    CAP_HIP(hipMemcpyAsync(evals, w.evals, sizeof(fe) * (size_t)P * 10, hipMemcpyDeviceToHost, s));
    CAP_HIP(wait_stream());
    trace("pb_r4_done", c.slot);

    std::vector<LinTerm> terms((size_t)P * kLinTerms);
    parallel_for(P, [&](uint32_t p) {
      const fe* ev = &evals[(size_t)p * 10];
      const fe *we = ev, *se = ev + NW;
      for (int i = 0; i < 10; i++) append_fr(tr[p], ev[i]);
      for (int i = 0; i < NW; i++) fe_to_words(we[i], proofs[p].wires_evals[i]);
      for (int i = 0; i < NW - 1; i++) fe_to_words(se[i], proofs[p].wire_sigma_evals[i]);
      fe_to_words(ev[9], proofs[p].perm_next_eval);
      td::LinIn in;
      for (int i = 0; i < 10; i++) in.ev[i] = ev[i];
      in.beta = chal[p].beta;
      in.gamma = chal[p].gamma;
      in.alpha = chal[p].alpha;
      in.alpha2 = chal[p].alpha2;
      in.zeta = zeta[p];
      in.v = get_challenge(tr[p]);
      for (int i = 0; i < NW; i++) in.k[i] = K.qc.k[i];
      in.n = n;
      fe sc[td::kLinScalars];
      td::lin_scalars(in, sc);
      LinTerm* T = &terms[(size_t)p * kLinTerms];
      term_polys(p, T);
      for (uint32_t t = 0; t < kLinTerms; t++) T[t].scalar = td::to_internal(sc[t]);
    });
    CAP_HIP(hipMemcpyAsync(w.terms, terms.data(), sizeof(LinTerm) * terms.size(), hipMemcpyHostToDevice, s));
    if ((rc = seg(6, [&]() -> int { return r5_body(); }))) return rc;
    if ((rc = fetch_comms(P * 2))) return rc;
    trace("pb_r5_done", c.slot);
    for (uint32_t p = 0; p < P; p++) {
      affine_to_words(ha[p * 2], proofs[p].opening_proof);
      affine_to_words(ha[p * 2 + 1], proofs[p].shifted_opening_proof);
    }
    if (rq.outcomes) host_outcomes(flags);
    side_drain.armed = false;
    return take_launch_error();
  }
};

}
}
```

Before: 1447.

## Evaluate quotient on five cosets plus top coefficients instead of six

Adds a five-coset quotient path. Wire and z polynomials are transformed onto fewer extended-domain points (two full-size sub-NTTs plus one half-size folded NTT). The high-degree top coefficients of the quotient are computed separately, and a custom combine kernel interpolates back using a precomputed 5x5 inverse system. Because the quotient is no longer evaluated at every point, gate and permutation correctness is checked directly on rows with new verdict kernels. It is enabled by default for non-recompute keys. It aims to cut about a sixth of quotient evaluation and NTT work, at the cost of extra kernels, a per-key selector table, and added complexity.

```diff
diff --git a/cap_amd/csrc/check_kernels.hpp b/cap_amd/csrc/check_kernels.hpp
--- a/cap_amd/csrc/check_kernels.hpp
+++ b/cap_amd/csrc/check_kernels.hpp
@@ -96,6 +96,16 @@
   check_report(key, &out[p].first, &out[p].copies);
 }
 
+__global__ void k_rows_verdict(const CheckOut* __restrict__ out, const fe* __restrict__ pre, const fe* __restrict__ num,
+                               const fe* __restrict__ sfx, const fe* __restrict__ den, size_t n,
+                               uint32_t* __restrict__ flags, uint32_t count) {
+  const uint32_t p = blockIdx.x * blockDim.x + threadIdx.x;
+  if (p >= count) return;
+  const size_t o = (size_t)p * n;
+  const fe total_num = Fr::mul(pre[o + n - 1], num[o + n - 1]), total_den = Fr::mul(sfx[o], den[o]);
+  if (out[p].first != kNoFault || !Fr::eq(total_num, total_den)) atomicOr(&flags[p], 1u);
+}
+
 __global__ void k_check_targets(const CheckKey* __restrict__ keys, const CheckOut* __restrict__ out, uint32_t P,
                                 size_t cells, uint32_t* __restrict__ to) {
   const uint32_t p = blockIdx.x * blockDim.x + threadIdx.x;
diff --git a/cap_amd/csrc/ntt.hip b/cap_amd/csrc/ntt.hip
--- a/cap_amd/csrc/ntt.hip
+++ b/cap_amd/csrc/ntt.hip
@@ -47,6 +47,7 @@
   size_t in_outer, in_inner, in_len;
   uint32_t in_group;
   uint32_t in_es;
+  size_t in_fold;
   size_t in_inner2;
   uint32_t in_group2;
   size_t out_outer, out_inner;
@@ -229,6 +230,9 @@
       for (int k = 0; k < 8; k++) nz |= raw[u].v[k];
       fl v = Fr29::load(raw[u]);
       if (p.pre_scale && any[u] && nz) v = Fr29::mul(v, Fr29::load(pre[u]));
+      if (p.in_fold && sgs[u] + p.in_fold < p.in_len)
+        v = Fr29::add_norm(v, Fr29::mul(Fr29::load(in[sgs[u] + p.in_fold]),
+                                        Fr29::load(p.pre_scale[sgs[u] + p.in_fold + (size_t)(by % p.in_group) * p.pre_inner])));
       sh[(bitrev32(j, p.log_len) << p.log_c) + c] = v;
     }
   }
@@ -318,6 +322,9 @@
       for (int k = 0; k < 8; k++) nz |= raw[u].v[k];
       fl v = Fr29::load(raw[u]);
       if (p.pre_scale && any[u] && nz) v = Fr29::mul(v, Fr29::load(pre[u]));
+      if (p.in_fold && sgs[u] + p.in_fold < p.in_len)
+        v = Fr29::add_norm(v, Fr29::mul(Fr29::load(in[sgs[u] + p.in_fold]),
+                                        Fr29::load(p.pre_scale[sgs[u] + p.in_fold + (size_t)(by % p.in_group) * p.pre_inner])));
       sh[(bitrev32(j, p.log_len) << p.log_c) + c] = v;
     }
   }
@@ -412,6 +419,44 @@
   }
 }
 
+__global__ __launch_bounds__(kThreads) void ntt3_combine5(const fe* __restrict__ y01, const fe* __restrict__ y2,
+                                                          fe* __restrict__ out, size_t n_len,
+                                                          const fe* __restrict__ unscale, Quot5Const qc,
+                                                          const fe* __restrict__ top, const fe* __restrict__ add) {
+  using F = Fr29;
+  const size_t i = (size_t)blockIdx.x * blockDim.x + threadIdx.x;
+  if (i >= n_len) return;
+  const uint32_t q = blockIdx.y;
+  const size_t m_len = 2 * n_len;
+  const fe* ya = y01 + (size_t)q * 2 * m_len;
+  fe* o = out + (size_t)q * 3 * m_len;
+  const fl e0 = F::mul(F::load(ya[i]), F::load(unscale[i]));
+  const fl o0 = F::mul(F::load(ya[n_len + i]), F::load(unscale[n_len + i]));
+  const fl e1 = F::mul(F::load(ya[m_len + i]), F::load(unscale[m_len + i]));
+  const fl o1 = F::mul(F::load(ya[m_len + n_len + i]), F::load(unscale[m_len + n_len + i]));
+  const fl r = F::mul(F::load(y2[(size_t)q * n_len + i]), F::load(unscale[2 * m_len + i]));
+  const bool has_top = i < 8;
+  fl pi = F::zero(), h = F::zero();
+  if (add) pi = F::load(add[(size_t)q * n_len + i]);
+  if (has_top) h = F::load(top[(size_t)q * 8 + i]);
+  auto finish = [&](fl v, int j) {
+    if (add) v = F::add(v, F::mul(pi, F::load(qc.d[j])));
+    if (has_top) v = F::add(v, F::mul(h, F::load(qc.mt[j])));
+    return F::pack(F::canonical(F::normalize(v)));
+  };
+  for (int jj = 0; jj < 2; jj++)
+    o[(size_t)(2 * jj + 1) * n_len + i] =
+        finish(F::mul_add_mul(o0, F::load(qc.odd[jj][0]), o1, F::load(qc.odd[jj][1])), 2 * jj + 1);
+  for (int jj = 0; jj < 3; jj++) {
+    const fl a = F::mul_add_mul(e0, F::load(qc.even[jj][0]), o0, F::load(qc.even[jj][1]));
+    const fl b = F::mul_add_mul(e1, F::load(qc.even[jj][2]), o1, F::load(qc.even[jj][3]));
+    o[(size_t)(2 * jj) * n_len + i] = finish(F::add(F::add(a, b), F::mul(r, F::load(qc.even[jj][4]))), 2 * jj);
+  }
+  fe t5 = Fr::zero();
+  if (has_top) t5 = top[(size_t)q * 8 + i];
+  o[5 * n_len + i] = t5;
+}
+
 fe host_root_of_unity(uint32_t log_n) {
   fe w;
   const uint32_t root28[8] = {0x725b19f0u, 0x9bd61b6eu, 0x41112ed4u, 0x402d111eu,
@@ -663,7 +708,11 @@
   const Addr a_dst = io ? Addr{io->dst_outer, io->dst_inner, io->dst_group ? io->dst_group : 1u} : Addr{stride_elems, 0, 1};
   const Addr a_tmp = Addr{scratch_stride, 0, 1};
   const size_t src_len = io ? io->src_len : ~(size_t)0;
+  const size_t src_fold = io ? io->src_fold : 0;
+  if (src_fold && (!io->pre_scale || (io->src_elem_stride > 1) || src_fold + ((size_t)1 << log_n) < io->src_len))
+    return (int)hipErrorInvalidValue;
   auto set_in = [&](const Addr& a, size_t len, uint32_t es) {
+    p.in_fold = &a == &a_src ? src_fold : 0;
     p.in_outer = a.outer;
     p.in_inner = a.inner;
     p.in_group = a.group;
@@ -761,6 +810,67 @@
     e[i] = (uint32_t)(cur / 3);
     rem = cur % 3;
   }
+}
+
+template <class ToInternal>
+int build_quot5(Ntt3Domain* d, const fe& g, const fe& wN, ToInternal to_internal, hipStream_t stream) {
+  const size_t M = (size_t)1 << d->log_m, nh = M / 2;
+  hipError_t e;
+  if ((e = hipMalloc(&d->unscale5, sizeof(fe) * (2 * M + nh))) != hipSuccess) return (int)e;
+  const uint32_t en[8] = {(uint32_t)nh, (uint32_t)((uint64_t)nh >> 32), 0, 0, 0, 0, 0, 0};
+  fe c[5];
+  fe s_a = g;
+  int rc;
+  for (int a = 0; a < 3; a++) {
+    c[a] = Fr::pow(s_a, en);
+    if ((rc = build_powers(d->unscale5 + (size_t)a * M, a < 2 ? M : nh, Fr::inv(s_a), nullptr, stream))) return rc;
+    s_a = Fr::mul(s_a, wN);
+  }
+  c[3] = Fr::neg(c[0]);
+  c[4] = Fr::neg(c[1]);
+  fe A[5][10];
+  for (int r = 0; r < 5; r++)
+    for (int j = 0; j < 10; j++) A[r][j] = j == 5 + r ? Fr::one() : Fr::zero();
+  for (int a = 0; a < 2; a++) {
+    const fe c2 = Fr::sqr(c[a]);
+    A[2 * a][0] = Fr::one();
+    A[2 * a][2] = c2;
+    A[2 * a][4] = Fr::sqr(c2);
+    A[2 * a + 1][1] = Fr::one();
+    A[2 * a + 1][3] = c2;
+  }
+  A[4][0] = Fr::one();
+  for (int j = 1; j < 5; j++) A[4][j] = Fr::mul(A[4][j - 1], c[2]);
+  for (int col = 0; col < 5; col++) {
+    int piv = col;
+    while (piv < 5 && Fr::is_zero(A[piv][col])) piv++;
+    if (piv == 5) return (int)hipErrorInvalidValue;
+    for (int j = 0; j < 10; j++) std::swap(A[piv][j], A[col][j]);
+    const fe inv = Fr::inv(A[col][col]);
+    for (int j = 0; j < 10; j++) A[col][j] = Fr::mul(A[col][j], inv);
+    for (int r = 0; r < 5; r++) {
+      if (r == col) continue;
+      const fe f = A[r][col];
+      for (int j = 0; j < 10; j++) A[r][j] = Fr::sub(A[r][j], Fr::mul(f, A[col][j]));
+    }
+  }
+  Quot5Const& q = d->q5;
+  for (int jj = 0; jj < 2; jj++)
+    for (int a = 0; a < 2; a++) q.odd[jj][a] = to_internal(A[2 * jj + 1][5 + 2 * a + 1]);
+  for (int jj = 0; jj < 3; jj++)
+    for (int r = 0; r < 5; r++) q.even[jj][r] = to_internal(A[2 * jj][5 + r]);
+  fe mt[6];
+  mt[0] = Fr::one();
+  for (int k = 0; k < 5; k++) {
+    mt[k + 1] = mt[k];
+    for (int j = k; j >= 1; j--) mt[j] = Fr::sub(mt[j - 1], Fr::mul(mt[j], c[k]));
+    mt[0] = Fr::neg(Fr::mul(mt[0], c[k]));
+  }
+  for (int j = 0; j < 5; j++) {
+    q.mt[j] = to_internal(mt[j]);
+    q.d[j] = to_internal(Fr::sub(Fr::one(), mt[j]));
+  }
+  return 0;
 }
 }
 
@@ -806,11 +916,12 @@
   launch("table_to_internal", table_to_internal, dim3(blocks), dim3(256), 0, stream, d->pre3, (const fe*)d->pre3, N);
   launch("table_to_internal", table_to_internal, dim3((unsigned)((2 * M + 255) / 256)), dim3(256), 0, stream,
          d->tw29_inv, (const fe*)d->tw29_inv, 2 * M);
+  if (log_m >= 1 && (rc = build_quot5(d, g, wN, to_internal, stream))) return rc;
   return (int)hipStreamSynchronize(stream);
 }
 
 void ntt3_free_domain(Ntt3Domain* d) {
-  for (fe** t : {&d->xs_ext, &d->xs29, &d->pre3, &d->tw29_inv, &d->coset_inv_ext}) {
+  for (fe** t : {&d->xs_ext, &d->xs29, &d->pre3, &d->tw29_inv, &d->coset_inv_ext, &d->unscale5}) {
     if (*t) hipFree(*t);
     *t = nullptr;
   }
@@ -864,4 +975,78 @@
   return 0;
 }
 
-}
+int ntt3_forward5(const Ntt3Domain& d3, const NttDomain& dom_m, const NttDomain& dom_h, const NttSmallTables& small,
+                  fe* data, NttIo io, uint32_t count, fe* scratch, hipStream_t stream) {
+  if (dom_m.log_n != d3.log_m || d3.log_m < 5 || dom_h.log_n + 1 != d3.log_m) return (int)hipErrorInvalidValue;
+  const size_t M = (size_t)1 << d3.log_m, nh = M / 2;
+  if (io.src_len > M || io.src_len < nh) return (int)hipErrorInvalidValue;
+  NttIo sub{};
+  sub.src = io.src;
+  sub.src_outer = io.src_outer;
+  sub.src_inner = 0;
+  sub.src_group = 2;
+  sub.src_group2 = io.src_group ? io.src_group : 1;
+  sub.src_inner2 = io.src_inner;
+  sub.src_len = io.src_len;
+  sub.pre_scale = d3.pre3;
+  sub.pre_inner = M;
+  sub.lazy_out = 1;
+  sub.dst_outer = io.dst_outer;
+  sub.dst_inner = M;
+  sub.dst_group = 2;
+  sub.dst_group2 = io.dst_group ? io.dst_group : 1;
+  sub.dst_inner2 = io.dst_inner;
+  int rc = ntt_run(dom_m, small, data, scratch, M, count * 2, 0, 0, stream, &sub);
+  if (rc) return rc;
+  NttIo h{};
+  h.src = io.src;
+  h.src_outer = io.src_outer;
+  h.src_inner = io.src_inner;
+  h.src_group = io.src_group ? io.src_group : 1;
+  h.src_len = io.src_len;
+  h.src_fold = io.src_len > nh ? nh : 0;
+  h.pre_scale = d3.pre3 + 2 * M;
+  h.lazy_out = 1;
+  h.dst_outer = io.dst_outer;
+  h.dst_inner = io.dst_inner;
+  h.dst_group = io.dst_group ? io.dst_group : 1;
+  return ntt_run(dom_h, small, data + 2 * M, scratch, nh, count, 0, 0, stream, &h);
+}
+
+int ntt3_inverse5(const Ntt3Domain& d3, const NttDomain& dom_m, const NttDomain& dom_h, const NttSmallTables& small,
+                  fe* data, uint32_t count, fe* scratch, hipStream_t stream, const fe* top, const fe* add) {
+  if (dom_m.log_n != d3.log_m || d3.log_m < 5 || dom_h.log_n + 1 != d3.log_m || !d3.unscale5 || !top)
+    return (int)hipErrorInvalidValue;
+  const size_t M = (size_t)1 << d3.log_m, N = 3 * M, nh = M / 2;
+  fe* y01 = scratch;
+  fe* y2 = y01 + (size_t)count * 2 * M;
+  fe* sub_scratch = y2 + (size_t)count * nh;
+  NttIo sub{};
+  sub.src = data;
+  sub.src_outer = N;
+  sub.src_inner = M;
+  sub.src_group = 2;
+  sub.src_len = M;
+  sub.lazy_out = 1;
+  sub.dst_outer = M;
+  sub.dst_inner = 0;
+  sub.dst_group = 1;
+  int rc = ntt_run(dom_m, small, y01, sub_scratch, M, count * 2, 1, 0, stream, &sub);
+  if (rc) return rc;
+  NttIo h{};
+  h.src = data + 2 * M;
+  h.src_outer = N;
+  h.src_inner = 0;
+  h.src_group = 1;
+  h.src_len = nh;
+  h.lazy_out = 1;
+  h.dst_outer = nh;
+  h.dst_inner = 0;
+  h.dst_group = 1;
+  if ((rc = ntt_run(dom_h, small, y2, sub_scratch, nh, count, 1, 0, stream, &h))) return rc;
+  launch("ntt3_combine5", ntt3_combine5, dim3((unsigned)((nh + kThreads - 1) / kThreads), count), dim3(kThreads), 0, stream,
+         (const fe*)y01, (const fe*)y2, data, nh, (const fe*)d3.unscale5, d3.q5, top, add);
+  return 0;
+}
+
+}
diff --git a/cap_amd/csrc/ntt.hpp b/cap_amd/csrc/ntt.hpp
--- a/cap_amd/csrc/ntt.hpp
+++ b/cap_amd/csrc/ntt.hpp
@@ -55,6 +55,7 @@
   int lazy_out = 0;
   int has_post_scalar = 0;
   fe post_scalar = {};
+  size_t src_fold = 0;
 };
 int ntt_run(const NttDomain& dom, const NttSmallTables& small, fe* data, fe* scratch, size_t stride_elems,
             uint32_t count, int dir, int coset, hipStream_t stream, const NttIo* io = nullptr);
@@ -69,6 +70,12 @@
 };
 int ntt_plan(uint32_t log_n, uint32_t count, NttPlan* out);
 
+struct Quot5Const {
+  fe odd[2][2];
+  fe even[3][5];
+  fe mt[5];
+  fe d[5];
+};
 struct Ntt3Domain {
   uint32_t log_m = 0;
   fe* xs_ext = nullptr;
@@ -80,6 +87,8 @@
   fe omega;
   fe kappa;
   fe kappa_n_inv29;
+  fe* unscale5 = nullptr;
+  Quot5Const q5;
 };
 int ntt3_build_domain(Ntt3Domain* d, uint32_t log_m, hipStream_t stream);
 void ntt3_free_domain(Ntt3Domain* d);
@@ -88,6 +97,11 @@
 int ntt3_inverse(const Ntt3Domain& d3, const NttDomain& dom_m, const NttSmallTables& small, fe* data, uint32_t count,
                  fe* scratch, hipStream_t stream, const fe* add = nullptr);
 
+int ntt3_forward5(const Ntt3Domain& d3, const NttDomain& dom_m, const NttDomain& dom_h, const NttSmallTables& small,
+                  fe* data, NttIo io, uint32_t count, fe* scratch, hipStream_t stream);
+int ntt3_inverse5(const Ntt3Domain& d3, const NttDomain& dom_m, const NttDomain& dom_h, const NttSmallTables& small,
+                  fe* data, uint32_t count, fe* scratch, hipStream_t stream, const fe* top, const fe* add = nullptr);
+
 void ntt_table_to_internal(fe* out, const fe* in, size_t n, hipStream_t stream);
 
 }
diff --git a/cap_amd/csrc/plonk.hip b/cap_amd/csrc/plonk.hip
--- a/cap_amd/csrc/plonk.hip
+++ b/cap_amd/csrc/plonk.hip
@@ -102,11 +102,12 @@
   int transcript = 0;
   uint32_t tr_stride = 0;
   int outcomes = 0;
+  bool five = false;
   bool operator==(const ProveGraphSig& o) const {
     return key_uid == o.key_uid && srs == o.srs && P == o.P && num_inputs == o.num_inputs && form == o.form &&
            multi == o.multi && d_wires == o.d_wires && ws == o.ws && msm_ws == o.msm_ws && ntt_scratch == o.ntt_scratch &&
            bases == o.bases && lagrange == o.lagrange && stream == o.stream && overlap == o.overlap && transcript == o.transcript &&
-           tr_stride == o.tr_stride && outcomes == o.outcomes;
+           tr_stride == o.tr_stride && outcomes == o.outcomes && five == o.five;
   }
 };
 struct ProveGraphSet {
@@ -260,6 +261,26 @@
 namespace {
 
 
+int key_gate_table_locked(const ProvingKey& K) {
+  if (K.chk_sel) return CAPGPU_OK;
+  hipStream_t s = ctx().stream;
+  const size_t n = K.n;
+  DevTmp<fe> sel;
+  CAP_HIP(sel.alloc((size_t)NS * n));
+  int rc = run_ntt_from(s, K.log_n, K.coef, K.ps, n, sel, n, NS, 0, 0);
+  if (rc) return rc;
+  ntt_table_to_internal(sel, sel, (size_t)NS * n, s);
+  CAP_HIP(hipStreamSynchronize(s));
+  if ((rc = take_launch_error())) return rc;
+  K.chk_sel = sel.p;
+  sel.p = nullptr;
+  return CAPGPU_OK;
+}
+int key_gate_table(const ProvingKey& K) {
+  std::lock_guard<std::mutex> lk(K.chk_mu);
+  return key_gate_table_locked(K);
+}
+
 int key_check_tables(const ProvingKey& K) {
   std::lock_guard<std::mutex> lk(K.chk_mu);
   if (K.chk_rc <= 0) {
@@ -268,18 +289,11 @@
   }
   Context& c = ctx();
   hipStream_t s = c.stream;
-  const size_t n = K.n, cells = (size_t)NW * n;
-  DevTmp<fe> sel;
+  const size_t cells = (size_t)NW * K.n;
   DevTmp<uint32_t> perm, bad;
-  CAP_HIP(sel.alloc((size_t)NS * n));
-  int rc = run_ntt_from(s, K.log_n, K.coef, K.ps, n, sel, n, NS, 0, 0);
+  int rc = key_gate_table_locked(K);
   if (rc) return rc;
-  ntt_table_to_internal(sel, sel, (size_t)NS * n, s);
   if (K.chk_perm) {
-    CAP_HIP(hipStreamSynchronize(s));
-    if ((rc = take_launch_error())) return rc;
-    K.chk_sel = sel.p;
-    sel.p = nullptr;
     K.chk_rc = CAPGPU_OK;
     return CAPGPU_OK;
   }
@@ -309,9 +323,7 @@
     K.chk_rc = CAPGPU_ERR_INVALID_ARG;
     return K.chk_rc;
   }
-  K.chk_sel = sel.p;
   K.chk_perm = perm.p;
-  sel.p = nullptr;
   perm.p = nullptr;
   K.chk_rc = CAPGPU_OK;
   return CAPGPU_OK;
@@ -446,6 +458,9 @@
 int prove_planned(Context& c, const ProvingKey& K, uint32_t P, const ProveRequest& rq, const ProvePlan& pl, ProveRun& run) {
   const size_t num_inputs = rq.num_inputs;
   int rc;
+  if (pl.five)
+    for (uint32_t p = 0; p < P && (rq.keys || p == 0); p++)
+      if ((rc = key_gate_table(rq.keys ? *(*rq.keys)[p] : K))) return rc;
   if ((rc = scratch_reserve(c.prove_ws, carve(nullptr, K, P, num_inputs, pl.coeffs, pl.tr_stride).total))) return rc;
   run.w = carve(c.prove_ws.p, K, P, num_inputs, pl.coeffs, pl.tr_stride);
   if (run.faults && pl.dev_tr)
@@ -470,6 +485,7 @@
     sig.transcript = pl.dev_tr ? CAPGPU_TRANSCRIPT_DEVICE : CAPGPU_TRANSCRIPT_HOST;
     sig.tr_stride = pl.tr_stride;
     sig.outcomes = rq.outcomes ? (run.faults ? 2 : 1) : 0;
+    sig.five = pl.five;
     run.gs = graph_set_for(c, sig);
   }
   return pl.dev_tr ? run.run_device_transcript() : run.run_host_transcript();
diff --git a/cap_amd/csrc/plonk_kernels.hpp b/cap_amd/csrc/plonk_kernels.hpp
--- a/cap_amd/csrc/plonk_kernels.hpp
+++ b/cap_amd/csrc/plonk_kernels.hpp
@@ -253,17 +253,20 @@
                                                        const fe* __restrict__ cos, const fe* __restrict__ xs,
                                                        const fe* __restrict__ inv_nx1,
                                                        const Chal* __restrict__ chal, QuotConst qc, size_t m,
-                                                       uint32_t only_unfoldable, fe* __restrict__ t_out) {
+                                                       uint32_t only_unfoldable, uint32_t five,
+                                                       fe* __restrict__ t_out) {
   using F = Fr29;
   size_t i = (size_t)blockIdx.y * blockDim.x + threadIdx.x;
-  if (i >= m) return;
+  if (i >= (five ? m - m / 6 : m)) return;
   const uint32_t p = blockIdx.x;
   if (FOLD ? !fe_nonzero(chal[p].beta_inv) : (only_unfoldable && fe_nonzero(chal[p].beta_inv))) return;
   if (pkc_of) pkc = pkc_of[p];
   const uint32_t mm = (uint32_t)(m / 3);
   const uint32_t blk = (i >= mm ? 1u : 0u) + (i >= 2 * (size_t)mm ? 1u : 0u);
   const fe* c = cos + (size_t)p * 6 * m;
-  auto sel = [&](int s) { return F::load(pkc[(size_t)s * m + i]); };
+  const bool half = five && blk == 2;
+  const size_t it = half ? 2 * i - 2 * (size_t)mm : i;
+  auto sel = [&](int s) { return F::load(pkc[(size_t)s * m + it]); };
   fl w0 = F::load(c[i]), w1 = F::load(c[m + i]), w2 = F::load(c[2 * m + i]), w3 = F::load(c[3 * m + i]),
      w4 = F::load(c[4 * m + i]);
   fl w01 = F::mul(w0, w1), w23 = F::mul(w2, w3);
@@ -294,12 +297,12 @@
   const fl gamma = F::load(chal[p].gamma);
   const fl zx = F::load(c[5 * m + i]);
   const uint32_t k1 = (uint32_t)i - blk * mm;
-  const size_t inext = (size_t)blk * mm + ((k1 + 2) & (mm - 1));
+  const size_t inext = (size_t)blk * mm + (half ? (k1 + 1) & (mm / 2 - 1) : (k1 + 2) & (mm - 1));
   if constexpr (FOLD) {
     const fl beta_inv = F::load(chal[p].beta_inv);
     fl a = zx, b = F::load(c[5 * m + inext]);
     fl u = F::mul(F::add(w0, gamma), beta_inv);
-    a = F::mul(a, F::add(u, F::load(xs[i])));
+    a = F::mul(a, F::add(u, F::load(xs[it])));
     b = F::mul(b, F::add(u, sel(NS + 0)));
     u = F::mul(F::add(w1, gamma), beta_inv);
     a = F::mul(a, F::add(u, sel(NS + NW + 0)));
@@ -316,7 +319,7 @@
     total = F::normalize(F::add(total, F::mul(F::load(chal[p].alpha_beta5), F::sub(a, b))));
   } else {
     const fl beta = F::load(chal[p].beta);
-    fl x = F::load(xs[i]);
+    fl x = F::load(xs[it]);
     fl bx = F::mul(beta, x);
     fl a = zx, b = F::load(c[5 * m + inext]);
     fl wg = F::add(w0, gamma);
@@ -337,8 +340,8 @@
     total = F::normalize(F::add(total, F::mul(F::load(chal[p].alpha), F::sub(a, b))));
   }
   fl l1a = F::mul(F::load(chal[p].alpha2), F::sub(zx, F::one()));
-  const uint32_t zi = 3 * (((uint32_t)i - blk * mm) & 1) + blk;
-  fl r = F::mul_add_mul(total, F::load(qc.zh_inv[zi]), l1a, F::load(inv_nx1[i]));
+  const uint32_t zi = 3 * (half ? 0u : ((uint32_t)i - blk * mm) & 1) + blk;
+  fl r = F::mul_add_mul(total, F::load(qc.zh_inv[zi]), l1a, F::load(inv_nx1[it]));
   t_out[(size_t)p * m + i] = F::store(r);
 }
 
@@ -359,6 +362,70 @@
     if (zero) atomicOr(&flags[p], 2u);
   } else if (!zero) {
     atomicOr(&flags[p], 1u);
+  }
+}
+
+__device__ __noinline__ void series_mul8(fe* dst, const fe* x, const fe* y, fe* prod) {
+  const uint32_t t = threadIdx.x, a = t >> 3, b = t & 7;
+  __syncthreads();
+  if (a + b < 8) prod[t] = Fr::mul(x[a], y[b]);
+  __syncthreads();
+  fe s = Fr::zero();
+  if (t < 8) {
+    s = prod[t];
+    for (uint32_t k = 1; k <= t; k++) s = Fr::add(s, prod[k * 8 + t - k]);
+  }
+  __syncthreads();
+  if (t < 8) dst[t] = s;
+  __syncthreads();
+}
+__global__ __launch_bounds__(64) void k_quotient_top(const fe* __restrict__ wpoly ,
+                                                     const fe* __restrict__ zpoly ,
+                                                     const fe* __restrict__ coef, const fe* const* __restrict__ coef_of,
+                                                     const fe* __restrict__ tw_n, const Chal* __restrict__ chal, size_t n,
+                                                     size_t ps, fe* __restrict__ top) {
+  __shared__ fe W[NW][8], B[NW][8], sa[8], sb[8], sc[8], prod[64];
+  const uint32_t p = blockIdx.x, t = threadIdx.x;
+  if (coef_of) coef = coef_of[p];
+  const fe* wp = wpoly + (size_t)p * NW * ps;
+  const fe* zp = zpoly + (size_t)p * ps;
+  if (t < NW * 8) {
+    const uint32_t j = t >> 3, k = t & 7;
+    const fe w = wp[(size_t)j * ps + n + 1 - k];
+    W[j][k] = w;
+    B[j][k] = k >= 2 ? Fr::add(w, Fr::mul(chal[p].beta, coef[(size_t)(NS + j) * ps + n + 1 - k])) : w;
+  }
+  fe h = Fr::zero();
+  auto take_gate = [&](const fe* s) {
+    if (t < 5) h = Fr::add(h, s[4 - t]);
+  };
+  for (int i = 0; i < 4; i++) {
+    series_mul8(sa, W[i], W[i], prod);
+    series_mul8(sa, sa, sa, prod);
+    series_mul8(sa, sa, W[i], prod);
+    if (t < 8) sb[t] = coef[(size_t)(6 + i) * ps + n - 1 - t];
+    series_mul8(sc, sa, sb, prod);
+    take_gate(sc);
+  }
+  series_mul8(sa, W[0], W[1], prod);
+  for (int j = 2; j < NW; j++) series_mul8(sa, sa, W[j], prod);
+  if (t < 8) sb[t] = coef[(size_t)12 * ps + n - 1 - t];
+  series_mul8(sc, sa, sb, prod);
+  take_gate(sc);
+  if (t < 8) sb[t] = zp[n + 2 - t];
+  series_mul8(sc, sa, sb, prod);
+  fe perm = Fr::zero();
+  if (t < 8) perm = sc[7 - t];
+  series_mul8(sa, B[0], B[1], prod);
+  for (int j = 2; j < NW; j++) series_mul8(sa, sa, B[j], prod);
+  if (t < 8) {
+    const size_t c = n + 2 - t;
+    sb[t] = Fr::mul(zp[c], tw_n[c >= n ? c - n : c]);
+  }
+  series_mul8(sc, sa, sb, prod);
+  if (t < 8) {
+    perm = Fr::sub(perm, sc[7 - t]);
+    top[(size_t)p * 8 + t] = Fr::add(h, Fr::mul(chal[p].alpha, perm));
   }
 }
 
diff --git a/cap_amd/csrc/prove_run.hpp b/cap_amd/csrc/prove_run.hpp
--- a/cap_amd/csrc/prove_run.hpp
+++ b/cap_amd/csrc/prove_run.hpp
@@ -35,7 +35,9 @@
 
 inline size_t ntt_scratch_inplace(size_t stride, size_t count) { return sizeof(fe) * stride * count; }
 inline size_t ntt_scratch_from(uint32_t log_n, size_t count) { return (sizeof(fe) << log_n) * count; }
-inline size_t ntt3_scratch(uint32_t log_mm, size_t count) { return (sizeof(fe) << log_mm) * 6 * count; }
+inline size_t ntt3_scratch(uint32_t log_mm, size_t count, bool five = false) {
+  return five ? (sizeof(fe) << log_mm) / 2 * 9 * count : (sizeof(fe) << log_mm) * 6 * count;
+}
 inline size_t wires_stage_bytes(size_t cnt, size_t n) { return sizeof(fe) * cnt * NW * n; }
 
 int run_ntt(hipStream_t s, uint32_t log_n, fe* data, size_t stride, uint32_t count, int dir, int coset) {
@@ -92,6 +94,28 @@
   if (rc) return hip_fail((hipError_t)rc, "ntt3_forward");
   return CAPGPU_OK;
 }
+int run_ntt3_fwd5(hipStream_t s, uint32_t log_mm, fe* data, uint32_t count, const NttIo& io) {
+  Context& c = ctx();
+  const Ntt3Domain* d3 = nullptr;
+  const NttDomain *dm = nullptr, *dh = nullptr;
+  int rc = quot_domains(log_mm, &d3, &dm);
+  if (rc || (rc = get_domain(log_mm - 1, &dh))) return rc;
+  if ((rc = scratch_reserve(c.ntt_scratch, ntt3_scratch(log_mm, count, true)))) return rc;
+  rc = ntt3_forward5(*d3, *dm, *dh, c.small, data, io, count, (fe*)c.ntt_scratch.p, s);
+  if (rc) return hip_fail((hipError_t)rc, "ntt3_forward5");
+  return CAPGPU_OK;
+}
+int run_ntt3_inv5(hipStream_t s, uint32_t log_mm, fe* data, uint32_t count, const fe* top, const fe* add) {
+  Context& c = ctx();
+  const Ntt3Domain* d3 = nullptr;
+  const NttDomain *dm = nullptr, *dh = nullptr;
+  int rc = quot_domains(log_mm, &d3, &dm);
+  if (rc || (rc = get_domain(log_mm - 1, &dh))) return rc;
+  if ((rc = scratch_reserve(c.ntt_scratch, ntt3_scratch(log_mm, count, true)))) return rc;
+  rc = ntt3_inverse5(*d3, *dm, *dh, c.small, data, count, (fe*)c.ntt_scratch.p, s, top, add);
+  if (rc) return hip_fail((hipError_t)rc, "ntt3_inverse5");
+  return CAPGPU_OK;
+}
 int run_ntt3_inv(hipStream_t s, uint32_t log_mm, fe* data, uint32_t count, const fe* add = nullptr) {
   Context& c = ctx();
   const Ntt3Domain* d3 = nullptr;
@@ -149,6 +173,9 @@
   EvalDesc* edesc;
   LinTerm* terms;
   const fe** key_ptrs;
+  fe* top;
+  CheckKey* chk_keys;
+  CheckOut* chk_out;
   uint8_t *d_proofs, *tr_state, *tr_pre, *tr_app;
   uint32_t* tr_pre_len;
   fe* zeta;
@@ -195,7 +222,10 @@
   w.comms = c.take<g1_jac>((size_t)P * 5);
   w.edesc = c.take<EvalDesc>((size_t)P * 10);
   w.terms = c.take<LinTerm>((size_t)P * kLinTerms);
-  w.key_ptrs = c.take<const fe*>((size_t)P * 2);
+  w.key_ptrs = c.take<const fe*>((size_t)P * 3);
+  w.top = c.take<fe>((size_t)P * 8);
+  w.chk_keys = c.take<CheckKey>(P);
+  w.chk_out = c.take<CheckOut>(P);
   if (tr_stride) {
     w.d_proofs = c.take<uint8_t>((size_t)P * td::kPrBytes);
     w.zeta = c.take<fe>(P);
@@ -222,6 +252,9 @@
 }
 int quotient_fold() {
   return env_int("CAPGPU_QUOT_FOLD", 1, 0, 2);
+}
+int quotient_cosets() {
+  return env_int("CAPGPU_QUOT_COSETS", 5, 5, 6);
 }
 
 std::atomic<int> g_wire_commit{-1};
@@ -362,6 +395,7 @@
   bool overlap = false;
   hipStream_t s2 = nullptr;
   bool graphs = false;
+  bool five = false;
   const MsmBases* B = nullptr;
   const MsmBases* Lag = nullptr;
   const MsmBases& wire_key() const { return Lag ? *Lag : *B; }
@@ -386,6 +420,7 @@
     if (!sizing) trace("pb_lagrange_fallback", c.slot, rc);
   }
   pl.dev_tr = transcript_mode() == CAPGPU_TRANSCRIPT_DEVICE && !comm_shard_prover();
+  pl.five = quotient_cosets() == 5 && K.log_n >= 4 && !K.recompute;
   if (pl.dev_tr) {
     if (longest_prefix > (1u << 30)) {
       set_error("capgpu_plonk_prove: transcript init message of %zu bytes", longest_prefix);
@@ -453,6 +488,8 @@
   std::vector<const fe*> key_ptrs;
   const fe* const* sig_of = nullptr;
   const fe* const* pkc_of = nullptr;
+  const fe* const* coef_of = nullptr;
+  std::vector<CheckKey> chk_keys;
   std::vector<SolidityTranscript> tr;
   g1_jac* hj = nullptr;
   fe* h_tot = nullptr;
@@ -594,14 +631,22 @@
     if (num_inputs)
       CAP_HIP(hipMemcpyAsync(w.d_pub, pub_inputs, sizeof(fe) * P * num_inputs, hipMemcpyHostToDevice, s));
     if (rq.keys) {
-      key_ptrs.resize((size_t)2 * P);
+      key_ptrs.resize((size_t)3 * P);
       for (uint32_t p = 0; p < P; p++) {
         key_ptrs[p] = key_of(p).sig_eval;
         key_ptrs[P + p] = key_of(p).pk_coset;
+        key_ptrs[2 * P + p] = key_of(p).coef;
       }
       CAP_HIP(hipMemcpyAsync(w.key_ptrs, key_ptrs.data(), sizeof(const fe*) * key_ptrs.size(), hipMemcpyHostToDevice, s));
       sig_of = w.key_ptrs;
       pkc_of = w.key_ptrs + P;
+      coef_of = w.key_ptrs + 2 * P;
+    }
+    if (pl.five) {
+      chk_keys.resize(P);
+      for (uint32_t p = 0; p < P; p++) chk_keys[p] = CheckKey{key_of(p).chk_sel, nullptr, (uint32_t)key_of(p).num_inputs, 0};
+      CAP_HIP(hipMemcpyAsync(w.chk_keys, chk_keys.data(), sizeof(CheckKey) * P, hipMemcpyHostToDevice, s));
+      CAP_HIP(hipMemsetAsync(w.chk_out, 0xff, sizeof(CheckOut) * P, s));
     }
     CAP_HIP(hipMemcpyAsync(w.d_blind, rq.blinders, sizeof(fe) * P * 13, hipMemcpyHostToDevice, s));
     CAP_HIP(hipMemsetAsync(w.flags, 0, sizeof(uint32_t) * P, s));
@@ -702,19 +747,21 @@
     if (K.num_inputs) nd.ntt(ntt_scratch_from(K.log_n, cnt));
   }
   int r3_wire_cosets(hipStream_t st) {
-    return run_ntt3_fwd(st, K.log_m, w.coset, P * NW, NttIo{w.wpoly, NW * ps, ps, n + 2, NW, 6 * m, m, NW});
+    const NttIo io{w.wpoly, NW * ps, ps, n + 2, NW, 6 * m, m, NW};
+    return pl.five ? run_ntt3_fwd5(st, K.log_m, w.coset, P * NW, io) : run_ntt3_fwd(st, K.log_m, w.coset, P * NW, io);
   }
   int z_cosets(hipStream_t st) {
-    return run_ntt3_fwd(st, K.log_m, w.coset + 5 * m, P, NttIo{w.zpoly, ps, 0, n + 3, 1, 6 * m, 0, 1});
-  }
-  static void cosets_needs(const ProvePlan&, const ProvingKey& K, uint32_t cnt, ProveNeeds& nd) {
-    nd.ntt(ntt3_scratch(K.log_m, (size_t)cnt * NW));
-    nd.ntt(ntt3_scratch(K.log_m, cnt));
+    const NttIo io{w.zpoly, ps, 0, n + 3, 1, 6 * m, 0, 1};
+    return pl.five ? run_ntt3_fwd5(st, K.log_m, w.coset + 5 * m, P, io) : run_ntt3_fwd(st, K.log_m, w.coset + 5 * m, P, io);
+  }
+  static void cosets_needs(const ProvePlan& pl, const ProvingKey& K, uint32_t cnt, ProveNeeds& nd) {
+    nd.ntt(ntt3_scratch(K.log_m, (size_t)cnt * NW, pl.five));
+    nd.ntt(ntt3_scratch(K.log_m, cnt, pl.five));
   }
   int r1_overlapped() {
     int r;
     const hipStream_t s2 = pl.s2;
-    if ((r = scratch_reserve(c.ntt_scratch, ntt3_scratch(K.log_m, (size_t)P * NW)))) return r;
+    if ((r = scratch_reserve(c.ntt_scratch, ntt3_scratch(K.log_m, (size_t)P * NW, pl.five)))) return r;
     auto interpolate_and_blind = [&](hipStream_t st) -> int {
       int q = CAPGPU_OK;
       if (pl.coeffs) pad_copy(st, w.wpoly, ps, 0, d_wires, n, 0, 1, P * NW, n, n);
@@ -737,7 +784,7 @@
     return CAPGPU_OK;
   }
   static void r1_overlapped_needs(const ProvePlan& pl, const ProvingKey& K, uint32_t cnt, ProveNeeds& nd) {
-    if (pl.overlap) nd.ntt(ntt3_scratch(K.log_m, (size_t)cnt * NW));
+    if (pl.overlap) nd.ntt(ntt3_scratch(K.log_m, (size_t)cnt * NW, pl.five));
   }
   int r1_body() {
     if (pl.overlap) return r1_overlapped();
@@ -811,14 +858,27 @@
     const int fold = quotient_fold();
     if (fold == 2)
       CAP_HIP(hipMemset2DAsync(&w.chal29[0].beta_inv, sizeof(Chal), 0, sizeof(fe), P, s));
+    const uint32_t five = pl.five ? 1u : 0u;
+    const size_t pts = pl.five ? 5 * n : m;
     if (fold)
-      launch("k_quotient", k_quotient<true>, dim3(P, cdiv(m, kThreads)), dim3(kThreads), 0, s, pkc, pkc_of,
-             (const fe*)w.coset, (const fe*)dom_q->xs29, (const fe*)K.inv_nx1, (const Chal*)w.chal29, K.qc29, m, 1u, w.t);
+      launch("k_quotient", k_quotient<true>, dim3(P, cdiv(pts, kThreads)), dim3(kThreads), 0, s, pkc, pkc_of,
+             (const fe*)w.coset, (const fe*)dom_q->xs29, (const fe*)K.inv_nx1, (const Chal*)w.chal29, K.qc29, m, 1u, five,
+             w.t);
     if (!fold || fold == 2 || beta_zero_possible)
-      launch("k_quotient_direct", k_quotient<false>, dim3(P, cdiv(m, kThreads)), dim3(kThreads), 0, s,
+      launch("k_quotient_direct", k_quotient<false>, dim3(P, cdiv(pts, kThreads)), dim3(kThreads), 0, s,
              pkc, pkc_of, (const fe*)w.coset, (const fe*)dom_q->xs29, (const fe*)K.inv_nx1, (const Chal*)w.chal29, K.qc29, m,
-             fold ? 1u : 0u, w.t);
-    if ((r = run_ntt3_inv(s, K.log_m, w.t, P, w.pi))) return r;
+             fold ? 1u : 0u, five, w.t);
+    if (pl.five) {
+      launch("k_quotient_top", k_quotient_top, dim3(P), dim3(64), 0, s, (const fe*)w.wpoly, (const fe*)w.zpoly,
+             (const fe*)K.coef, coef_of, (const fe*)dom_n->tw_fwd, (const Chal*)w.chal, n, ps, w.top);
+      launch("k_check_gates", k_check_gates, dim3(cdiv(n, kThreads), P), dim3(kThreads), 0, s,
+             pl.coeffs ? (const fe*)w.wev : d_wires, (const fe*)w.d_pub, num_inputs, (const CheckKey*)w.chk_keys, n, w.chk_out);
+      launch("k_rows_verdict", k_rows_verdict, dim3(cdiv(P, 64)), dim3(64), 0, s, (const CheckOut*)w.chk_out,
+             (const fe*)w.pre, (const fe*)w.num, (const fe*)w.sfx, (const fe*)w.den, n, w.flags, P);
+      if ((r = run_ntt3_inv5(s, K.log_m, w.t, P, w.top, w.pi))) return r;
+    } else if ((r = run_ntt3_inv(s, K.log_m, w.t, P, w.pi))) {
+      return r;
+    }
     {
       size_t lo = NW * (n + 1) + 3;
       launch("k_check_degree", k_check_degree, dim3(cdiv(m - (lo - 1), kThreads), P), dim3(kThreads), 0, s,
@@ -828,7 +888,7 @@
   }
   static void r3_needs(const ProvePlan& pl, const ProvingKey& K, uint32_t cnt, ProveNeeds& nd) {
     if (K.recompute) nd.ntt(ntt3_scratch(K.log_m, 18));
-    nd.ntt(ntt3_scratch(K.log_m, cnt));
+    nd.ntt(ntt3_scratch(K.log_m, cnt, pl.five));
     nd.msm(*pl.B, K.n + 2, cnt * NW);
   }
 
```

Measured after the change: 1494, median of 6. +3.3%, better.
